# skyhehe123/SA-SSD

Hardware: AMD Instinct MI355X
Metric: KITTI-Car inference frames/sec (whole job) (higher is better)
Workload: dtype f32; 1 GPU; configs/car_cfg.py inference, fp32, synthetic lidar64 K21 frames (21500 pts -> ~16k voxels), batch=1, random-init SA-SSD weights, points resident in HBM; frames_in_flight=3, spconv_cfg=0, rulebook_pyramid=levels, launch=one hipGraph replay per frame, parallelism=frame-sharded x1, no collective

## Files before the change

### include/sassd.h

```cpp
#ifndef SASSD_H
#define SASSD_H

#include <stddef.h>
#include <stdint.h>

#ifdef __cplusplus
extern "C" {
#endif

#define SASSD_OK       0
#define SASSD_EINVAL  -1
#define SASSD_ENOSPC  -2
#define SASSD_EHIP    -3

#define SASSD_ST_VOXEL_OVERFLOW   1
#define SASSD_ST_HASH_FULL        2
#define SASSD_ST_BOX_OVERFLOW     4
#define SASSD_ST_GRID_SYNC        8
#define SASSD_ST_POINT_OVERFLOW  16

#define SASSD_MAX_POINTS_PER_VOXEL 64

const char *sassd_version(void);
int sassd_last_hip_error(void);
const char *sassd_last_hip_error_string(void);


int sassd_graph_begin(void *stream);
int sassd_graph_end(void *stream, void **graph_exec);
int sassd_graph_launch(void *graph_exec, void *stream);
int sassd_graph_destroy(void *graph_exec);

size_t sassd_voxelize_workspace_bytes(int n_points, int max_points);
int sassd_voxelize(const float *points, int n_points, int ndim, const float *voxel_size,
                   const float *coors_range, int max_points, int max_voxels, int batch_idx,
                   float *voxels, int32_t *coors, int coors_cols, int32_t *num_points, float *mean,
                   int nfeat, int32_t *row_offset, int32_t *voxel_num, int cap, int32_t *status,
                   void *workspace, size_t workspace_bytes, void *stream);

int sassd_voxelize_dev(const float *points, int points_cap, const int32_t *n_points_dev, int ndim,
                       const float *voxel_size, const float *coors_range, int max_points, int max_voxels,
                       int batch_idx, float *voxels, int32_t *coors, int coors_cols, int32_t *num_points,
                       float *mean, int nfeat, int32_t *row_offset, int32_t *voxel_num, int cap, int32_t *status,
                       void *workspace, size_t workspace_bytes, void *stream);

int sassd_voxel_mean(const float *voxels, const int32_t *num_points, int m, int max_points, int ndim,
                     int nfeat, float *mean, void *stream);

size_t sassd_crop_polytope_workspace_bytes(int cap_in);
int sassd_crop_polytope_dev(const float *points, int cap_in, const int32_t *n_in_dev, int ndim,
                            const double *planes, int f32_math, float *out, int cap_out, int32_t *n_out_dev,
                            int32_t *status, void *workspace, size_t workspace_bytes, void *stream);

size_t sassd_hash_bytes(int cap_rows);
int sassd_hash_build(const int32_t *indices, const int32_t *n_ptr, int cap, int D, int H, int W,
                     int batch_size, void *table, size_t table_bytes, int32_t *status, void *stream);
int sassd_rulebook_subm(const int32_t *indices, const int32_t *n_ptr, int cap, int D, int H, int W,
                        int batch_size, const void *table, size_t table_bytes, int32_t *nbr,
                        void *stream);
size_t sassd_rulebook_conv_workspace_bytes(int D, int H, int W, int batch_size);
int sassd_rulebook_conv(const int32_t *in_indices, const int32_t *n_in_ptr, int cap_in, int D, int H,
                        int W, int batch_size, const void *in_table, size_t in_table_bytes,
                        int32_t *out_indices, int32_t *n_out_ptr, int cap_out, int32_t *nbr,
                        int32_t *status, void *workspace, size_t workspace_bytes, void *stream);
int sassd_rulebook_pairs(const int32_t *nbr, const int32_t *n_out_ptr, int cap_out, int K,
                         int32_t *pairs , int32_t *pair_num , void *stream);

#define SASSD_PYRAMID_PERSISTENT 1
size_t sassd_rulebook_pyramid_workspace_bytes(int levels, const int *caps, int D, int H, int W, int batch_size);
int sassd_rulebook_pyramid(int levels, int32_t *const *indices, int32_t *const *n_ptrs, const int *caps,
                           int D, int H, int W, int batch_size, int32_t *const *nbr_subm,
                           int32_t *const *nbr_down, int level_begin, int level_end, int flags, int32_t *status,
                           void *workspace, size_t workspace_bytes, void *stream);

size_t sassd_spconv_packed_floats(int K, int Cin, int Cout);
int sassd_spconv_pack_weight(const float *w, int K, int Cin, int Cout, float *packed, void *stream);
int sassd_spconv_fwd(const float *x, const int32_t *nbr, const int32_t *n_out_ptr, int cap_out,
                     const float *w_packed, int K, int Cin, int Cout, const float *scale,
                     const float *shift, int relu, float *y, int cfg, void *stream);

int sassd_rulebook_transpose(const int32_t *nbr, const int32_t *n_out_ptr, int cap_out, int32_t *nbrT,
                             int cap_in, void *stream);
int sassd_spconv_pack_weight_t(const float *w, int K, int Cin, int Cout, float *packed, void *stream);
int sassd_spconv_bwd_data(const float *dy, const int32_t *nbrT, const int32_t *n_in_ptr, int cap_in,
                          const float *wT_packed, int K, int Cin, int Cout, float *dx, int cfg, void *stream);
size_t sassd_spconv_bwd_weight_workspace_bytes(int cap_out, int K, int Cin, int Cout);
int sassd_spconv_bwd_weight(const float *x, const float *dy, const int32_t *nbr, const int32_t *n_out_ptr,
                            int cap_out, int K, int Cin, int Cout, float *dw, int accumulate, int cfg,
                            void *workspace, size_t workspace_bytes, void *stream);

int sassd_densify(const float *feats, const int32_t *indices, const int32_t *n_ptr, int cap, int C,
                  int D, int H, int W, int batch_size, int channel_order, float *out, void *stream);
int sassd_densify_bf16_supported(int C, int D, int H, int W);
int sassd_densify_bf16(const float *feats, const int32_t *indices, const int32_t *n_ptr, int cap, int C, int D, int H, int W,
                       int batch_size, int channel_order, void *out, void *stream);

int sassd_spconv_bf16_supported(int K, int Cin, int Cout, int cap);
size_t sassd_spconv_bf16_packed_bytes(int K, int Cin, int Cout);
int sassd_spconv_bf16_pack_weight(const float *w, int K, int Cin, int Cout, void *packed, void *stream);
int sassd_spconv_fwd_bf16(const void *x, int x_is_f32, const int32_t *nbr, const int32_t *n_out_ptr, int cap_out,
                          const void *w_packed, int K, int Cin, int Cout, const float *scale, const float *shift, int relu,
                          void *y_bf16, int cfg, void *stream);
int sassd_densify_from_bf16(const void *feats, const int32_t *indices, const int32_t *n_ptr, int cap, int C, int D, int H, int W,
                            int batch_size, int channel_order, void *out, int out_is_bf16, void *stream);

int sassd_spconv_train_bf16_supported(int K, int Cin, int Cout, int cap);
size_t sassd_spconv_train_bf16_packed_bytes(int K, int Cin, int Cout);
int sassd_spconv_train_bf16_pack_weight(const float *w, int K, int Cin, int Cout, void *packed, void *stream);
int sassd_spconv_fwd_bf16_raw(const void *x_bf16, const int32_t *nbr, const int32_t *n_out_ptr, int cap_out, const void *w_packed,
                              int K, int Cin, int Cout, float *y, int cfg, void *stream);
size_t sassd_spconv_bwd_weight_bf16_workspace_bytes(int cap_out, int K, int Cin, int Cout);
int sassd_spconv_bwd_weight_bf16(const void *x_bf16, const void *dy_bf16, const int32_t *nbr, const int32_t *n_out_ptr, int cap_out,
                                 int K, int Cin, int Cout, float *dw, int accumulate, int cfg, void *workspace,
                                 size_t workspace_bytes, void *stream);
int sassd_bn_relu_fwd_bf16out(const float *x, int n, int C, const float *gamma, const float *beta, float *running_mean,
                              float *running_var, float momentum, float eps, void *y_bf16, float *save_mean, float *save_invstd,
                              void *workspace, size_t workspace_bytes, void *stream);
int sassd_bn_relu_bwd_bf16out(const float *x, const float *dy, int n, int C, const float *gamma, const float *beta,
                              const float *save_mean, const float *save_invstd, void *dx_bf16, float *dgamma, float *dbeta,
                              void *workspace, size_t workspace_bytes, void *stream);

size_t sassd_conv2d_packed_floats(int Cin, int Cout, int ksize);
int sassd_conv2d_pack_weight(const float *w, int Cout, int Cin, int ksize, float *packed, void *stream);
int sassd_conv2d_fwd(const float *x, const float *w_packed, const float *scale, const float *shift,
                     int relu, float *y, int batch, int Cin, int Cout, int H, int W, int ksize,
                     void *stream);
int sassd_conv2d_fwd_cfg(const float *x, const float *w_packed, const float *scale, const float *shift, int relu, float *y,
                         int batch, int Cin, int Cout, int H, int W, int ksize, int cfg, void *stream);

int sassd_conv1x1_narrow_supported(int Cin, int Cout);
int sassd_conv1x1_narrow_pad(int Cout);
int sassd_conv1x1_narrow_fwd(const float *x, const float *wT, const float *scale, const float *shift, int relu,
                             float *y, int batch, int Cin, int Cout, int H, int W, void *stream);

int sassd_conv2d_wino_supported(int Cin, int Cout, int H, int W);
size_t sassd_conv2d_wino_packed_floats(int Cin, int Cout);
int sassd_conv2d_wino_pack_weight(const float *w, int Cout, int Cin, float *packed, void *stream);
int sassd_conv2d_wino_fwd(const float *x, const float *w_packed, const float *scale, const float *shift, int relu,
                          float *y, int batch, int Cin, int Cout, int H, int W, void *stream);

int sassd_conv2d_wino4_supported(int Cin, int Cout, int H, int W);
size_t sassd_conv2d_wino4_packed_floats(int Cin, int Cout);
int sassd_conv2d_wino4_pack_weight(const float *w , int Cout, int Cin, float *packed, void *stream);
size_t sassd_conv2d_wino4_workspace_bytes(int batch, int Cin, int Cout, int H, int W);
int sassd_conv2d_wino4_fwd(const float *x, const float *w_packed, const float *scale, const float *shift, int relu,
                           float *y, int batch, int Cin, int Cout, int H, int W, int cfg, void *workspace,
                           size_t workspace_bytes, void *stream);

int sassd_conv2d_wino4_chain_supported(int Cin, int Cout, int H, int W);
size_t sassd_conv2d_wino4_chain_workspace_bytes(int batch, int cmax, int H, int W);
int sassd_conv2d_wino4_chain(const float *x, int src_products, const float *prev_scale, const float *prev_shift,
                             int prev_relu, const float *w_packed, const float *scale, const float *shift, int relu,
                             float *y, int batch, int Cin, int Cout, int cmax, int H, int W, const int32_t *tile_map,
                             const int32_t *prev_tile_map, int cfg, void *workspace, size_t workspace_bytes,
                             void *stream);
size_t sassd_conv2d_wino4_narrow_packed_floats(int Cin);
int sassd_conv2d_wino4_pack_weight_narrow(const float *w , int Cout, int Cin, float *packed, void *stream);
int sassd_conv2d_wino4_chain_tail(const float *prev_scale, const float *prev_shift, int prev_relu, float *y_prev,
                                  const float *w_packed64, const float *scale, const float *shift, int relu, float *y,
                                  int batch, int Cin, int Cout, int cmax, int H, int W, const int32_t *prev_tile_map, int cfg,
                                  void *workspace, size_t workspace_bytes, void *stream);

size_t sassd_wino4_tile_map_ints(int batch, int H, int W);
int sassd_wino4_tile_map(const int32_t *indices, const int32_t *n_ptr, int cap, int batch, int H, int W,
                         int32_t *tile_map, void *stream);

size_t sassd_wino4_sparse_grid_ints(int batch, int D, int H, int W);
int sassd_wino4_sparse_prepare(const int32_t *indices, const int32_t *n_ptr, int cap, int batch, int D, int H, int W,
                               int32_t *grid, int32_t *tile_map, void *stream);
int sassd_conv2d_wino4_chain_sparse(const float *feats, int C, int D, const int32_t *grid, const float *w_packed,
                                    const float *scale, const float *shift, int relu, float *y, int batch, int Cin, int Cout,
                                    int cmax, int H, int W, const int32_t *tile_map, int cfg, void *workspace,
                                    size_t workspace_bytes, void *stream);

int sassd_conv1x1_gemm_supported(int Cin, int Cout, int H, int W);
int sassd_conv1x1_gemm_pack_weight(const float *w , int Cout, int Cin, float *packed, void *stream);
int sassd_conv1x1_gemm_fwd(const float *x, const float *w_packed, const float *scale, const float *shift, int relu,
                           float *y, int batch, int Cin, int Cout, int H, int W, int cfg, void *stream);

int sassd_conv2d_bf16_supported(int Cin, int Cout, int H, int W);
size_t sassd_conv2d_bf16_packed_elems(int Cin, int Cout);
int sassd_conv2d_bf16_pack_weight(const float *w, int Cout, int Cin, void *packed, void *stream);
int sassd_conv2d_bf16_fwd(const float *x, const void *w_packed, const float *shift, float *y, int batch, int Cin,
                          int Cout, int H, int W, void *stream);
int sassd_conv2d_bf16_fwd_cfg(const float *x, const void *w_packed, const float *shift, float *y, int batch, int Cin,
                              int Cout, int H, int W, int cfg, void *stream);
int sassd_conv2d_bf16_bnrelu_fwd(const float *x, const float *in_affine, const void *w_packed, const float *shift, float *y,
                                 int batch, int Cin, int Cout, int H, int W, void *stream);

int sassd_conv1x1_bf16_supported(int Cin, int Cout, int HW);
size_t sassd_conv1x1_bf16_packed_elems(int Cin, int Cout);
int sassd_conv1x1_bf16_pack_weight(const float *w, int Cout, int Cin, int transposed, void *packed, void *stream);
int sassd_conv1x1_bf16_fwd(const float *x, const void *w_packed, const float *shift, float *y, int batch, int Cin, int Cout,
                           int HW, void *stream);

int sassd_conv2d_bf16_infer_supported(int Cin, int Cout, int H, int W);
size_t sassd_conv2d_bf16_infer_packed_elems(int Cin, int Cout);
int sassd_conv2d_bf16_infer_pack_weight(const float *w, int Cout, int Cin, void *packed, void *stream);
int sassd_conv2d_bf16_infer_fwd(const void *x, const void *w_packed, const float *scale, const float *shift, int relu, void *y,
                                int y_bf16, int batch, int Cin, int Cout, int H, int W, void *stream);
int sassd_conv1x1_bf16_infer_supported(int Cin, int Cout, int HW);
int sassd_conv1x1_bf16_infer_fwd(const void *x, const void *w_packed, const float *scale, const float *shift, int relu, void *y,
                                 int y_bf16, int batch, int Cin, int Cout, int HW, void *stream);

size_t sassd_conv2d_wgrad_workspace_bytes(int batch, int Cin, int Cout, int H, int W, int ksize);
int sassd_conv2d_bwd_weight(const float *x, const float *dy, float *dw, int batch, int Cin, int Cout, int H, int W,
                            int ksize, int accumulate, void *workspace, size_t workspace_bytes, void *stream);
int sassd_conv2d_bwd_weight_bf16(const float *x, const float *dy, float *dw, int batch, int Cin, int Cout, int H, int W,
                                 int ksize, int accumulate, void *workspace, size_t workspace_bytes, void *stream);
int sassd_conv2d_bwd_weight_bf16_bnrelu(const float *x, const float *x_affine, const float *dy, float *dw, int batch, int Cin,
                                        int Cout, int H, int W, int ksize, int accumulate, void *workspace,
                                        size_t workspace_bytes, void *stream);

size_t sassd_assign_targets_workspace_bytes(int batch, int n_anchors, int total_gt);
int sassd_assign_targets(const float *anchors, int anchors_per_sample, const uint8_t *anchor_mask, int n_anchors,
                         int batch, const float *gt_boxes, const int64_t *gt_classes, const uint8_t *gt_ok,
                         const int32_t *gt_offsets, int total_gt, const float *overlaps, const int64_t *overlap_offsets,
                         float matched_threshold, float unmatched_threshold, int64_t *labels, float *targets,
                         float *best_overlap, size_t out_sample_stride, int32_t *num_pos, int zero_num_pos,
                         void *workspace, size_t workspace_bytes, void *stream);
size_t sassd_guided_select_workspace_bytes(int batch, int n_anchors);
int sassd_guided_select(const float *cls_preds, const uint8_t *anchor_mask, int n_anchors, int batch, int num_class,
                        float score_thr, int cap, int64_t *sel, int32_t *counts, int32_t *overflow, void *workspace,
                        size_t workspace_bytes, void *stream);
size_t sassd_rpn_loss_workspace_bytes(int batch, int n_anchors);
int sassd_rpn_loss(const float *box_preds, const float *cls_preds, const float *dir_preds, int num_class,
                   const int64_t *labels, const float *targets, const float *anchors, int anchors_per_sample,
                   const int32_t *num_pos, int n_anchors, int batch, float *grad_box, float *grad_cls, float *grad_dir,
                   float *loss_sums, void *workspace, size_t workspace_bytes, void *stream);

size_t sassd_anchor_mask_workspace_bytes(int H0, int W0);
int sassd_anchor_mask(const int32_t *coors, const int32_t *row_begin_ptr, const int32_t *row_end_ptr,
                      int H0, int W0, const float *anchors_bv, int n_anchors, const float *voxel_size,
                      const float *coors_range, float area_threshold, uint8_t *mask, void *workspace,
                      size_t workspace_bytes, void *stream);
int sassd_anchor_mask_batch(const int32_t *coors, const int32_t *row_offsets, int batch, int H0, int W0,
                            const float *anchors_bv, int n_anchors, const float *voxel_size,
                            const float *coors_range, float area_threshold, uint8_t *mask, void *workspace,
                            size_t workspace_bytes, void *stream);

size_t sassd_decode_filter_workspace_bytes(int batch, int n_anchors_total);
int sassd_decode_filter(const float *box, const float *cls, const float *dir, size_t batch_stride,
                        int batch, int num_class, int anchors_per_loc, int H, int W,
                        const float *anchors, const uint8_t *mask, float thr, float *guided,
                        int32_t *labels, float *scores, int32_t *counts, int capK, int32_t *status,
                        void *workspace, size_t workspace_bytes, void *stream);

int sassd_pswarp_sample(const float *feat, int batch, int H, int W, const float *guided,
                        const int32_t *counts, int capK, float grid_off_x, float grid_off_y,
                        float spatial_scale, float *logits, void *stream);

int sassd_pswarp_sample_bwd(const float *feat, int batch, int H, int W, const float *guided,
                            const int32_t *counts, int capK, float grid_off_x, float grid_off_y,
                            float spatial_scale, const float *dlogits, float *dfeat, float *dguided,
                            void *stream);

size_t sassd_rescore_nms_workspace_bytes(int batch, int capK);
int sassd_rescore_nms(const float *guided, const float *logits, const int32_t *labels,
                      const int32_t *counts, int batch, int capK, float score_thr, float iou_thr,
                      float *out_boxes, float *out_scores, int32_t *out_labels, int32_t *out_counts,
                      int capD, int32_t *status, void *workspace, size_t workspace_bytes, void *stream);

#define SASSD_FRAME_MAGIC 0x53460001
#define SASSD_FRAME_HEADER_WORDS(B) ((5 + (B) + 3) / 4 * 4)
size_t sassd_frame_record_bytes(int batch, int capD);
int sassd_frame_seal(const float *boxes, const float *scores, const int32_t *labels, const int32_t *counts,
                     int batch, int capD, const int32_t *seq, const int32_t *status, void *record,
                     size_t record_bytes, void *stream);

#define SASSD_FRAME_MAGIC_KITTI 0x53460002
size_t sassd_frame_annos_bytes(int batch, int capD);
int sassd_frame_annos(const float *boxes, const int32_t *counts, int batch, int capD, const double *calib,
                      void *annos, size_t annos_bytes, void *stream);
size_t sassd_frame_record_kitti_bytes(int batch, int capD);
int sassd_frame_seal_kitti(const float *boxes, const float *scores, const int32_t *labels, const int32_t *counts,
                           int batch, int capD, const int32_t *seq, const int32_t *status, const double *calib,
                           void *record, size_t record_bytes, void *stream);

int sassd_boxes_overlap_bev(const float *boxes_a, int num_a, const float *boxes_b, int num_b,
                            float *ans_overlap, void *stream);
int sassd_boxes_iou_bev(const float *boxes_a, int num_a, const float *boxes_b, int num_b,
                        float *ans_iou, void *stream);
size_t sassd_nms_workspace_bytes(int n);
int sassd_nms_gpu(const float *boxes, int n, float thresh, int64_t *keep, int32_t *num_keep,
                  void *workspace, size_t workspace_bytes, void *stream);
int sassd_nms_normal_gpu(const float *boxes_sorted, int n, float thresh, int64_t *keep, int32_t *num_keep,
                         void *workspace, size_t workspace_bytes, void *stream);

int sassd_three_nn(int n, int m, const float *unknown, const float *known, float *dist2, int32_t *idx,
                   void *stream);
size_t sassd_three_nn_binned_workspace_bytes(int m, int nx, int ny, int batch_size);
int sassd_three_nn_binned(int n, int m, const float *unknown, const float *known, float x0, float y0, float cell,
                          int nx, int ny, int batch_size, float *dist2, int32_t *idx, void *workspace,
                          size_t workspace_bytes, void *stream);
int sassd_three_interpolate(int c, int m, int n, const float *points, const int32_t *idx, const float *weight,
                            float *out, void *stream);
int sassd_three_interpolate_grad(int c, int n, int m, const float *grad_out, const int32_t *idx,
                                 const float *weight, float *grad_points, void *stream);
int sassd_pts_in_boxes3d(const float *pts, int n, const float *boxes3d, int m, int32_t *pts_flag,
                         float *reg_target, void *stream);

int sassd_rotate_iou_eval(const float *boxes, int n, const float *query_boxes, int k, int criterion, float *iou,
                          void *stream);

int sassd_kitti_eval_statistics(const double *overlaps, int64_t ld, int n_img, const int64_t *gt_nums,
                                const int64_t *dt_nums, const int64_t *dc_nums, const double *gt_datas,
                                const double *dt_datas, const double *dontcares, const int64_t *ignored_gts,
                                const int64_t *ignored_dets, int metric, double min_overlap, const double *thresholds,
                                int n_thr, int compute_aos, double *pr, double *tp_scores, int64_t *n_tp_scores);


int sassd_points_in_polytopes(const float *points, int n, int stride, const double *planes, int m, int f32_math,
                              uint8_t *mask, void *stream);

int sassd_points_transform(float *points, int n, int stride, const uint8_t *mask, int m, const uint8_t *valid,
                           const float *centers, const float *rot_sin, const float *rot_cos, const double *loc,
                           void *stream);

int sassd_points_global_transform(float *points, int n, int stride, int flip, float rot_sin, float rot_cos, float scale,
                                  void *stream);

int sassd_paste_objects(const float *db_points, const int64_t *src_start, const int64_t *out_start, int n_obj,
                        int64_t n_out, const double *shift, const double *lower, float *out, void *stream);

int sassd_box_collision_test(const void *boxes, int n, const void *qboxes, int k, int is_f64, uint8_t *out);
int sassd_noise_per_box(const float *boxes, const uint8_t *valid, const double *loc_noises, const double *rot_noises,
                        int n, int num_try, int64_t *success);

size_t sassd_bn_relu_workspace_bytes(int C);
int sassd_bn_relu_fwd(const float *x, int n, int C, const float *gamma, const float *beta, float *running_mean,
                      float *running_var, float momentum, float eps, float *y, float *save_mean, float *save_invstd,
                      void *workspace, size_t workspace_bytes, void *stream);
int sassd_bn_relu_bwd(const float *x, const float *dy, int n, int C, const float *gamma, const float *beta,
                      const float *save_mean, const float *save_invstd, float *dx, float *dgamma, float *dbeta,
                      void *workspace, size_t workspace_bytes, void *stream);

size_t sassd_bn2d_relu_workspace_bytes(int C);
int sassd_bn2d_relu_fwd(const float *x, int B, int C, int HW, const float *gamma, const float *beta, float *running_mean,
                        float *running_var, float momentum, float eps, float *y, float *save_mean, float *save_invstd,
                        void *workspace, size_t workspace_bytes, void *stream);
int sassd_bn2d_stats(const float *x, int B, int C, int HW, const float *gamma, const float *beta, float *running_mean,
                     float *running_var, float momentum, float eps, float *save_mean, float *save_invstd, float *affine,
                     void *workspace, size_t workspace_bytes, void *stream);
int sassd_bn2d_relu_bwd(const float *x, const float *dy, int B, int C, int HW, const float *gamma, const float *beta,
                        const float *save_mean, const float *save_invstd, float *dx, float *dgamma, float *dbeta,
                        void *workspace, size_t workspace_bytes, void *stream);

int sassd_guided_decode_fwd(const float *box_preds, const float *dir_preds, const float *anchors, int anchors_per_sample,
                            const int64_t *sel, const int32_t *sel_count, const float *gt_boxes, const int32_t *gt_off,
                            int A, int B, int cap, int gmax, float *guided, int32_t *counts, void *stream);
int sassd_guided_decode_bwd(const float *box_preds, const float *anchors, int anchors_per_sample, const int64_t *sel,
                            const int32_t *sel_count, const int32_t *gt_off, int A, int B, int cap, int gmax,
                            const float *dguided, float *dbox, void *stream);
int sassd_boxes_iou3d_batch(const float *boxes, const int32_t *counts, int B, int rows, const float *gt_boxes,
                            const int32_t *gt_off, int gmax, const int64_t *ov_off, float *overlaps, void *stream);
size_t sassd_focal_loss_workspace_bytes(int n);
int sassd_focal_loss(const float *logits, const int64_t *labels, int n, const int32_t *num_pos, int nb, float *loss_sum,
                     float *grad, void *workspace, size_t workspace_bytes, void *stream);

size_t sassd_aux_head_workspace_bytes(int N);
int sassd_aux_prepare(const float *voxel_feats, int vstride, const int32_t *coors, int N, const int32_t *const *indices,
                      const int *M, const float *voxel_size, const float *offset, const float *gt_boxes,
                      const int32_t *gt_off, int B, float *points, float *const *known, uint8_t *label, float *target,
                      int *npos, void *stream);
int sassd_aux_head_fwd(int N, const float *const *feats, const int32_t *const *nn_idx, const float *const *nn_d2,
                       const float *w1, const float *w2, const uint8_t *label, const float *target, const int *npos,
                       float *wgt, float *h, float *out, float *gout, float *loss_sums, void *workspace,
                       size_t workspace_bytes, void *stream);
int sassd_aux_head_bwd(int N, const float *const *feats, const int *M, const int32_t *const *nn_idx, const float *w1,
                       const float *w2, const float *wgt, const float *h, const float *gout, const float *grad_sums,
                       float *const *grad_feats, float *dw1, float *dw2, void *workspace, size_t workspace_bytes,
                       void *stream);

int sassd_gather_pack(const float *src, const int32_t *map, void *dst, long n, int bf16, void *stream);
int sassd_grad_sumsq(const float *grad, long n, float *out, void *stream);
int sassd_adam_step(float *param, const float *grad, float *exp_avg, float *exp_avg_sq, long n,
                    const float *grad_sumsq, float lr, float beta1, float beta2, float eps, float weight_decay,
                    int step, float max_norm, float grad_scale, void *stream);

size_t sassd_three_interpolate_grad_det_workspace_bytes(int n, int m);
int sassd_three_interpolate_grad_det(int c, int n, int m, const float *grad_out, const int32_t *idx,
                                     const float *weight, float *grad_points, void *ws, size_t ws_bytes, void *stream);
size_t sassd_aux_head_bwd_det_workspace_bytes(int N, const int *M);
int sassd_aux_head_bwd_det(int N, const float *const *feats, const int *M, const int32_t *const *nn_idx,
                           const float *w1, const float *w2, const float *wgt, const float *h, const float *gout,
                           const float *grad_sums, float *const *grad_feats, float *dw1, float *dw2, void *workspace,
                           size_t workspace_bytes, void *stream);
size_t sassd_pswarp_sample_bwd_det_workspace_bytes(int batch, int capK);
int sassd_pswarp_sample_bwd_det(const float *feat, int batch, int H, int W, const float *guided,
                                const int32_t *counts, int capK, float grid_off_x, float grid_off_y,
                                float spatial_scale, const float *dlogits, float *dfeat, float *dguided, void *ws,
                                size_t ws_bytes, void *stream);
size_t sassd_grad_sumsq_det_workspace_bytes(long n);
int sassd_grad_sumsq_det(const float *grad, long n, float *out, void *ws, size_t ws_bytes, void *stream);

int sassd_mfma_probe(const float *a32, const float *b32, float *d32, const float *a16, const float *b16,
                     float *d16, int ksteps, void *stream);

#ifdef __cplusplus
}
#endif
#endif
```

### sa-ssd_amd/_C.py

```python
import ctypes as C
import os
import subprocess

_HERE = os.path.dirname(os.path.abspath(__file__))
LIB_PATH = os.path.join(_HERE, "lib", "libsassd.so")
_lib = None

OK, EINVAL, ENOSPC, EHIP = 0, -1, -2, -3
ST_VOXEL_OVERFLOW, ST_HASH_FULL, ST_BOX_OVERFLOW = 1, 2, 4
ST_POINT_OVERFLOW = 16


def build(force=False, verbose=False):
    cmd = ["make", "-C", os.path.join(_HERE, "csrc"), "-j8"]
    if force:
        subprocess.check_call(cmd + ["clean"], stdout=subprocess.DEVNULL)
    out = subprocess.run(cmd, stdout=subprocess.PIPE, stderr=subprocess.STDOUT, text=True)
    if verbose or out.returncode != 0:
        print(out.stdout)
    if out.returncode != 0:
        raise RuntimeError("building libsassd.so failed")
    return LIB_PATH


_SZ = C.c_size_t
_P = C.c_void_p
_I = C.c_int
_F = C.c_float

_SIGS = {
    "sassd_version": (C.c_char_p, []),
    "sassd_last_hip_error": (_I, []),
    "sassd_last_hip_error_string": (C.c_char_p, []),
    "sassd_voxelize_workspace_bytes": (_SZ, [_I, _I]),
    "sassd_voxelize": (_I, [_P, _I, _I, _P, _P, _I, _I, _I, _P, _P, _I, _P, _P, _I, _P, _P, _I, _P, _P, _SZ, _P]),
    "sassd_voxelize_dev": (_I, [_P, _I, _P, _I, _P, _P, _I, _I, _I, _P, _P, _I, _P, _P, _I, _P, _P, _I, _P, _P, _SZ, _P]),
    "sassd_voxel_mean": (_I, [_P, _P, _I, _I, _I, _I, _P, _P]),
    "sassd_crop_polytope_workspace_bytes": (_SZ, [_I]),
    "sassd_crop_polytope_dev": (_I, [_P, _I, _P, _I, _P, _I, _P, _I, _P, _P, _P, _SZ, _P]),
    "sassd_hash_bytes": (_SZ, [_I]),
    "sassd_hash_build": (_I, [_P, _P, _I, _I, _I, _I, _I, _P, _SZ, _P, _P]),
    "sassd_rulebook_subm": (_I, [_P, _P, _I, _I, _I, _I, _I, _P, _SZ, _P, _P]),
    "sassd_rulebook_conv_workspace_bytes": (_SZ, [_I, _I, _I, _I]),
    "sassd_rulebook_conv": (_I, [_P, _P, _I, _I, _I, _I, _I, _P, _SZ, _P, _P, _I, _P, _P, _P, _SZ, _P]),
    "sassd_rulebook_pairs": (_I, [_P, _P, _I, _I, _P, _P, _P]),
    "sassd_rulebook_pyramid_workspace_bytes": (_SZ, [_I, _P, _I, _I, _I, _I]),
    "sassd_rulebook_pyramid": (_I, [_I, _P, _P, _P, _I, _I, _I, _I, _P, _P, _I, _I, _I, _P, _P, _SZ, _P]),
    "sassd_graph_begin": (_I, [_P]),
    "sassd_graph_end": (_I, [_P, _P]),
    "sassd_graph_launch": (_I, [_P, _P]),
    "sassd_graph_destroy": (_I, [_P]),
    "sassd_spconv_packed_floats": (_SZ, [_I, _I, _I]),
    "sassd_spconv_pack_weight": (_I, [_P, _I, _I, _I, _P, _P]),
    "sassd_spconv_fwd": (_I, [_P, _P, _P, _I, _P, _I, _I, _I, _P, _P, _I, _P, _I, _P]),
    "sassd_rulebook_transpose": (_I, [_P, _P, _I, _P, _I, _P]),
    "sassd_spconv_pack_weight_t": (_I, [_P, _I, _I, _I, _P, _P]),
    "sassd_spconv_bwd_data": (_I, [_P, _P, _P, _I, _P, _I, _I, _I, _P, _I, _P]),
    "sassd_spconv_bwd_weight_workspace_bytes": (_SZ, [_I, _I, _I, _I]),
    "sassd_spconv_bwd_weight": (_I, [_P, _P, _P, _P, _I, _I, _I, _I, _P, _I, _I, _P, _SZ, _P]),
    "sassd_densify": (_I, [_P, _P, _P, _I, _I, _I, _I, _I, _I, _I, _P, _P]),
    "sassd_densify_bf16_supported": (_I, [_I, _I, _I, _I]),
    "sassd_densify_bf16": (_I, [_P, _P, _P, _I, _I, _I, _I, _I, _I, _I, _P, _P]),
    "sassd_spconv_bf16_supported": (_I, [_I, _I, _I, _I]),
    "sassd_spconv_bf16_packed_bytes": (_SZ, [_I, _I, _I]),
    "sassd_spconv_bf16_pack_weight": (_I, [_P, _I, _I, _I, _P, _P]),
    "sassd_spconv_fwd_bf16": (_I, [_P, _I, _P, _P, _I, _P, _I, _I, _I, _P, _P, _I, _P, _I, _P]),
    "sassd_densify_from_bf16": (_I, [_P, _P, _P, _I, _I, _I, _I, _I, _I, _I, _P, _I, _P]),
    "sassd_spconv_train_bf16_supported": (_I, [_I, _I, _I, _I]),
    "sassd_spconv_train_bf16_packed_bytes": (_SZ, [_I, _I, _I]),
    "sassd_spconv_train_bf16_pack_weight": (_I, [_P, _I, _I, _I, _P, _P]),
    "sassd_spconv_fwd_bf16_raw": (_I, [_P, _P, _P, _I, _P, _I, _I, _I, _P, _I, _P]),
    "sassd_spconv_bwd_weight_bf16_workspace_bytes": (_SZ, [_I, _I, _I, _I]),
    "sassd_spconv_bwd_weight_bf16": (_I, [_P, _P, _P, _P, _I, _I, _I, _I, _P, _I, _I, _P, _SZ, _P]),
    "sassd_bn_relu_fwd_bf16out": (_I, [_P, _I, _I, _P, _P, _P, _P, _F, _F, _P, _P, _P, _P, _SZ, _P]),
    "sassd_bn_relu_bwd_bf16out": (_I, [_P, _P, _I, _I, _P, _P, _P, _P, _P, _P, _P, _P, _SZ, _P]),
    "sassd_conv2d_packed_floats": (_SZ, [_I, _I, _I]),
    "sassd_conv2d_pack_weight": (_I, [_P, _I, _I, _I, _P, _P]),
    "sassd_conv2d_fwd": (_I, [_P, _P, _P, _P, _I, _P, _I, _I, _I, _I, _I, _I, _P]),
    "sassd_conv2d_fwd_cfg": (_I, [_P, _P, _P, _P, _I, _P, _I, _I, _I, _I, _I, _I, _I, _P]),
    "sassd_anchor_mask_workspace_bytes": (_SZ, [_I, _I]),
    "sassd_anchor_mask": (_I, [_P, _P, _P, _I, _I, _P, _I, _P, _P, _F, _P, _P, _SZ, _P]),
    "sassd_anchor_mask_batch": (_I, [_P, _P, _I, _I, _I, _P, _I, _P, _P, _F, _P, _P, _SZ, _P]),
    "sassd_decode_filter_workspace_bytes": (_SZ, [_I, _I]),
    "sassd_decode_filter": (_I, [_P, _P, _P, _SZ, _I, _I, _I, _I, _I, _P, _P, _F, _P, _P, _P, _P, _I, _P, _P, _SZ, _P]),
    "sassd_pswarp_sample": (_I, [_P, _I, _I, _I, _P, _P, _I, _F, _F, _F, _P, _P]),
    "sassd_pswarp_sample_bwd": (_I, [_P, _I, _I, _I, _P, _P, _I, _F, _F, _F, _P, _P, _P, _P]),
    "sassd_rescore_nms_workspace_bytes": (_SZ, [_I, _I]),
    "sassd_rescore_nms": (_I, [_P, _P, _P, _P, _I, _I, _F, _F, _P, _P, _P, _P, _I, _P, _P, _SZ, _P]),
    "sassd_frame_record_bytes": (_SZ, [_I, _I]),
    "sassd_frame_seal": (_I, [_P, _P, _P, _P, _I, _I, _P, _P, _P, _SZ, _P]),
    "sassd_frame_annos_bytes": (_SZ, [_I, _I]),
    "sassd_frame_annos": (_I, [_P, _P, _I, _I, _P, _P, _SZ, _P]),
    "sassd_frame_record_kitti_bytes": (_SZ, [_I, _I]),
    "sassd_frame_seal_kitti": (_I, [_P, _P, _P, _P, _I, _I, _P, _P, _P, _P, _SZ, _P]),
    "sassd_boxes_overlap_bev": (_I, [_P, _I, _P, _I, _P, _P]),
    "sassd_boxes_iou_bev": (_I, [_P, _I, _P, _I, _P, _P]),
    "sassd_nms_workspace_bytes": (_SZ, [_I]),
    "sassd_nms_gpu": (_I, [_P, _I, _F, _P, _P, _P, _SZ, _P]),
    "sassd_nms_normal_gpu": (_I, [_P, _I, _F, _P, _P, _P, _SZ, _P]),
    "sassd_three_nn": (_I, [_I, _I, _P, _P, _P, _P, _P]),
    "sassd_three_interpolate": (_I, [_I, _I, _I, _P, _P, _P, _P, _P]),
    "sassd_three_interpolate_grad": (_I, [_I, _I, _I, _P, _P, _P, _P, _P]),
    "sassd_pts_in_boxes3d": (_I, [_P, _I, _P, _I, _P, _P, _P]),
    "sassd_three_nn_binned_workspace_bytes": (_SZ, [_I, _I, _I, _I]),
    "sassd_three_nn_binned": (_I, [_I, _I, _P, _P, _F, _F, _F, _I, _I, _I, _P, _P, _P, _SZ, _P]),
    "sassd_conv2d_wino_supported": (_I, [_I, _I, _I, _I]),
    "sassd_conv2d_wino_packed_floats": (_SZ, [_I, _I]),
    "sassd_conv2d_wino_pack_weight": (_I, [_P, _I, _I, _P, _P]),
    "sassd_conv2d_wino_fwd": (_I, [_P, _P, _P, _P, _I, _P, _I, _I, _I, _I, _I, _P]),
    "sassd_conv2d_wino4_supported": (_I, [_I, _I, _I, _I]),
    "sassd_conv2d_wino4_packed_floats": (_SZ, [_I, _I]),
    "sassd_conv2d_wino4_pack_weight": (_I, [_P, _I, _I, _P, _P]),
    "sassd_conv2d_wino4_workspace_bytes": (_SZ, [_I, _I, _I, _I, _I]),
    "sassd_conv2d_wino4_fwd": (_I, [_P, _P, _P, _P, _I, _P, _I, _I, _I, _I, _I, _I, _P, _SZ, _P]),
    "sassd_conv1x1_gemm_supported": (_I, [_I, _I, _I, _I]),
    "sassd_conv1x1_gemm_pack_weight": (_I, [_P, _I, _I, _P, _P]),
    "sassd_conv1x1_narrow_supported": (_I, [_I, _I]),
    "sassd_conv1x1_narrow_pad": (_I, [_I]),
    "sassd_conv1x1_narrow_fwd": (_I, [_P, _P, _P, _P, _I, _P, _I, _I, _I, _I, _I, _P]),
    "sassd_conv1x1_gemm_fwd": (_I, [_P, _P, _P, _P, _I, _P, _I, _I, _I, _I, _I, _I, _P]),
    "sassd_conv2d_bf16_supported": (_I, [_I, _I, _I, _I]),
    "sassd_conv2d_bf16_packed_elems": (_SZ, [_I, _I]),
    "sassd_conv2d_bf16_pack_weight": (_I, [_P, _I, _I, _P, _P]),
    "sassd_conv2d_bf16_fwd": (_I, [_P, _P, _P, _P, _I, _I, _I, _I, _I, _P]),
    "sassd_conv2d_bf16_fwd_cfg": (_I, [_P, _P, _P, _P, _I, _I, _I, _I, _I, _I, _P]),
    "sassd_conv2d_bf16_bnrelu_fwd": (_I, [_P, _P, _P, _P, _P, _I, _I, _I, _I, _I, _P]),
    "sassd_conv1x1_bf16_supported": (_I, [_I, _I, _I]),
    "sassd_conv1x1_bf16_packed_elems": (_SZ, [_I, _I]),
    "sassd_conv1x1_bf16_pack_weight": (_I, [_P, _I, _I, _I, _P, _P]),
    "sassd_conv1x1_bf16_fwd": (_I, [_P, _P, _P, _P, _I, _I, _I, _I, _P]),
    "sassd_conv2d_bf16_infer_supported": (_I, [_I, _I, _I, _I]),
    "sassd_conv2d_bf16_infer_packed_elems": (_SZ, [_I, _I]),
    "sassd_conv2d_bf16_infer_pack_weight": (_I, [_P, _I, _I, _P, _P]),
    "sassd_conv2d_bf16_infer_fwd": (_I, [_P, _P, _P, _P, _I, _P, _I, _I, _I, _I, _I, _I, _P]),
    "sassd_conv1x1_bf16_infer_supported": (_I, [_I, _I, _I]),
    "sassd_conv1x1_bf16_infer_fwd": (_I, [_P, _P, _P, _P, _I, _P, _I, _I, _I, _I, _I, _P]),
    "sassd_conv2d_wgrad_workspace_bytes": (_SZ, [_I, _I, _I, _I, _I, _I]),
    "sassd_conv2d_bwd_weight": (_I, [_P, _P, _P, _I, _I, _I, _I, _I, _I, _I, _P, _SZ, _P]),
    "sassd_assign_targets_workspace_bytes": (_SZ, [_I, _I, _I]),
    "sassd_assign_targets": (_I, [_P, _I, _P, _I, _I, _P, _P, _P, _P, _I, _P, _P, _F, _F, _P, _P, _P, _SZ, _P, _I, _P,
                                  _SZ, _P]),
    "sassd_guided_select_workspace_bytes": (_SZ, [_I, _I]),
    "sassd_guided_select": (_I, [_P, _P, _I, _I, _I, _F, _I, _P, _P, _P, _P, _SZ, _P]),
    "sassd_rpn_loss_workspace_bytes": (_SZ, [_I, _I]),
    "sassd_rpn_loss": (_I, [_P, _P, _P, _I, _P, _P, _P, _I, _P, _I, _I, _P, _P, _P, _P, _P, _SZ, _P]),
    "sassd_conv2d_bwd_weight_bf16": (_I, [_P, _P, _P, _I, _I, _I, _I, _I, _I, _I, _P, _SZ, _P]),
    "sassd_conv2d_bwd_weight_bf16_bnrelu": (_I, [_P, _P, _P, _P, _I, _I, _I, _I, _I, _I, _I, _P, _SZ, _P]),
    "sassd_rotate_iou_eval": (_I, [_P, _I, _P, _I, _I, _P, _P]),
    "sassd_kitti_eval_statistics": (_I, [_P, C.c_int64, _I, _P, _P, _P, _P, _P, _P, _P, _P, _I, C.c_double, _P, _I, _I, _P,
                                         _P, _P]),
    "sassd_points_in_polytopes": (_I, [_P, _I, _I, _P, _I, _I, _P, _P]),
    "sassd_points_transform": (_I, [_P, _I, _I, _P, _I, _P, _P, _P, _P, _P, _P]),
    "sassd_points_global_transform": (_I, [_P, _I, _I, _I, _F, _F, _F, _P]),
    "sassd_paste_objects": (_I, [_P, _P, _P, _I, C.c_int64, _P, _P, _P, _P]),
    "sassd_box_collision_test": (_I, [_P, _I, _P, _I, _I, _P]),
    "sassd_noise_per_box": (_I, [_P, _P, _P, _P, _I, _I, _P]),
    "sassd_bn_relu_workspace_bytes": (_SZ, [_I]),
    "sassd_bn_relu_fwd": (_I, [_P, _I, _I, _P, _P, _P, _P, _F, _F, _P, _P, _P, _P, _SZ, _P]),
    "sassd_bn_relu_bwd": (_I, [_P, _P, _I, _I, _P, _P, _P, _P, _P, _P, _P, _P, _SZ, _P]),
    "sassd_bn2d_relu_workspace_bytes": (_SZ, [_I]),
    "sassd_bn2d_relu_fwd": (_I, [_P, _I, _I, _I, _P, _P, _P, _P, _F, _F, _P, _P, _P, _P, _SZ, _P]),
    "sassd_bn2d_stats": (_I, [_P, _I, _I, _I, _P, _P, _P, _P, _F, _F, _P, _P, _P, _P, _SZ, _P]),
    "sassd_bn2d_relu_bwd": (_I, [_P, _P, _I, _I, _I, _P, _P, _P, _P, _P, _P, _P, _P, _SZ, _P]),
    "sassd_aux_head_workspace_bytes": (_SZ, [_I]),
    "sassd_aux_prepare": (_I, [_P, _I, _P, _I, _P, _P, _P, _P, _P, _P, _I, _P, _P, _P, _P, _P, _P]),
    "sassd_aux_head_fwd": (_I, [_I, _P, _P, _P, _P, _P, _P, _P, _P, _P, _P, _P, _P, _P, _P, _SZ, _P]),
    "sassd_aux_head_bwd": (_I, [_I, _P, _P, _P, _P, _P, _P, _P, _P, _P, _P, _P, _P, _P, _SZ, _P]),
    "sassd_guided_decode_fwd": (_I, [_P, _P, _P, _I, _P, _P, _P, _P, _I, _I, _I, _I, _P, _P, _P]),
    "sassd_guided_decode_bwd": (_I, [_P, _P, _I, _P, _P, _P, _I, _I, _I, _I, _P, _P, _P]),
    "sassd_boxes_iou3d_batch": (_I, [_P, _P, _I, _I, _P, _P, _I, _P, _P, _P]),
    "sassd_focal_loss_workspace_bytes": (_SZ, [_I]),
    "sassd_focal_loss": (_I, [_P, _P, _I, _P, _I, _P, _P, _P, _SZ, _P]),
    "sassd_conv2d_wino4_chain_supported": (_I, [_I, _I, _I, _I]),
    "sassd_conv2d_wino4_chain_workspace_bytes": (_SZ, [_I, _I, _I, _I]),
    "sassd_conv2d_wino4_chain": (_I, [_P, _I, _P, _P, _I, _P, _P, _P, _I, _P, _I, _I, _I, _I, _I, _I, _P, _P, _I, _P, _SZ, _P]),
    "sassd_conv2d_wino4_narrow_packed_floats": (_SZ, [_I]),
    "sassd_conv2d_wino4_pack_weight_narrow": (_I, [_P, _I, _I, _P, _P]),
    "sassd_conv2d_wino4_chain_tail": (_I, [_P, _P, _I, _P, _P, _P, _P, _I, _P, _I, _I, _I, _I, _I, _I, _P, _I, _P, _SZ, _P]),
    "sassd_wino4_tile_map_ints": (_SZ, [_I, _I, _I]),
    "sassd_wino4_tile_map": (_I, [_P, _P, _I, _I, _I, _I, _P, _P]),
    "sassd_wino4_sparse_grid_ints": (_SZ, [_I, _I, _I, _I]),
    "sassd_wino4_sparse_prepare": (_I, [_P, _P, _I, _I, _I, _I, _I, _P, _P, _P]),
    "sassd_conv2d_wino4_chain_sparse": (_I, [_P, _I, _I, _P, _P, _P, _P, _I, _P, _I, _I, _I, _I, _I, _I, _P, _I, _P, _SZ, _P]),
    "sassd_gather_pack": (_I, [_P, _P, _P, C.c_long, _I, _P]),
    "sassd_grad_sumsq": (_I, [_P, C.c_long, _P, _P]),
    "sassd_adam_step": (_I, [_P, _P, _P, _P, C.c_long, _P, _F, _F, _F, _F, _F, _I, _F, _F, _P]),
    "sassd_mfma_probe": (_I, [_P, _P, _P, _P, _P, _P, _I, _P]),
    "sassd_three_interpolate_grad_det_workspace_bytes": (_SZ, [_I, _I]),
    "sassd_three_interpolate_grad_det": (_I, [_I, _I, _I, _P, _P, _P, _P, _P, _SZ, _P]),
    "sassd_aux_head_bwd_det_workspace_bytes": (_SZ, [_I, _P]),
    "sassd_aux_head_bwd_det": (_I, [_I, _P, _P, _P, _P, _P, _P, _P, _P, _P, _P, _P, _P, _P, _SZ, _P]),
    "sassd_pswarp_sample_bwd_det_workspace_bytes": (_SZ, [_I, _I]),
    "sassd_pswarp_sample_bwd_det": (_I, [_P, _I, _I, _I, _P, _P, _I, _F, _F, _F, _P, _P, _P, _P, _SZ, _P]),
    "sassd_grad_sumsq_det_workspace_bytes": (_SZ, [C.c_long]),
    "sassd_grad_sumsq_det": (_I, [_P, C.c_long, _P, _P, _SZ, _P]),
}

EXPORTS = tuple(_SIGS.keys())


def lib():
    global _lib
    if _lib is None:
        if not os.path.exists(LIB_PATH):
            raise RuntimeError("libsassd.so not found at %s -- run `python -c 'import __graft_entry__ as g; "
                               "g.build()'` (there is no CPU fallback)" % LIB_PATH)
        l = C.CDLL(LIB_PATH)
        for name, (res, args) in _SIGS.items():
            fn = getattr(l, name)
            fn.restype = res
            fn.argtypes = args
        _lib = l
    return _lib


def check(rc, what):
    if rc != OK:
        l = lib()
        extra = ""
        if rc == EHIP:
            extra = ": " + l.sassd_last_hip_error_string().decode()
        raise RuntimeError("%s failed with code %d%s" % (what, rc, extra))


def ptr(t):
    return None if t is None else t.data_ptr()


def stream():
    import torch
    return torch._C._cuda_getCurrentRawStream(torch.cuda.current_device())


def csrc_hash():
    import glob
    import hashlib
    h = hashlib.sha1()
    for f in sorted(glob.glob(os.path.join(os.path.dirname(os.path.abspath(__file__)), "csrc", "*"))):
        if os.path.isfile(f):
            h.update(os.path.basename(f).encode())
            h.update(open(f, "rb").read())
    return h.hexdigest()[:12]
```

### sa-ssd_amd/csrc/conv2d.hip

```cpp
#include <type_traits>

#include "common.h"

namespace {

typedef float f32x16 __attribute__((ext_vector_type(16)));
typedef __attribute__((address_space(3))) void *lds_ptr_t;
typedef const __attribute__((address_space(1))) void *glb_ptr_t;

__device__ __attribute__((aligned(16))) float g_zero_page[4] = {0.f, 0.f, 0.f, 0.f};

template <int CT, int TAPS, int VEC>
struct ConvCfg {
    static constexpr bool KSPLIT = (CT == 1);
    static constexpr int NSEG = (CT == 4) ? 9 : 5;
    static constexpr int KC = (TAPS == 9) ? 8 : 16;
    static constexpr int HALO = (TAPS == 9) ? 1 : 0;
    static constexpr int BMC = CT * 32;
    static constexpr int PIX = NSEG * 32;
    static constexpr int WV4 = TAPS * KC * BMC / 4;
    static constexpr int NLW = (WV4 + 255) / 256;
    static constexpr int MAXLP = (VEC == 4) ? 1 : 40;
    static constexpr int WS = TAPS * KC * BMC;
    static constexpr int NWJ = (WS / 256 + 3) / 4;
// ... 174 lines not shown
                    src -= (size_t)over * P.HW;
                }
            }
            __builtin_amdgcn_global_load_lds((glb_ptr_t)src, (lds_ptr_t)(pdst[part] >= 0 ? buf + pdst[part] : smem + dummy),
                                             16, 0, 0);
            pptr[part] += ((pdata >> part) & 1u) ? pinc : 0;
        }
    };
    auto dma = [&](int ch, float *buf) {
#pragma unroll
        for (int part = 0; part < NPARTS; ++part) dma_part(ch, buf, part);
    };
    auto issue = [&](int ch) {
        const float *wsrc_base = P.wp + (size_t)ch * TAPS * KC * P.CoutPad;
#pragma unroll
        for (int i = 0; i < NLW; ++i)
            if (woff_g[i] >= 0) wreg[i] = *(const float4 *)(wsrc_base + woff_g[i]);
#pragma unroll
        for (int i = 0; i < MAXLP; ++i)
            if (goff[i] >= 0) preg[i] = xb[clamp_off(ch, goff[i])];
    };
    auto commit = [&](float *buf) {
#pragma unroll
        for (int i = 0; i < NLW; ++i)
            if (woff_g[i] >= 0) *(float4 *)(buf + woff_l[i]) = wreg[i];
        float *pbuf = buf + WS;
#pragma unroll
        for (int i = 0; i < MAXLP; ++i)
            if (goff[i] >= 0) pbuf[loff[i]] = preg[i];
    };

    if constexpr (DMA) {
        dma(0, smem);
    } else {
        issue(0);
        commit(smem);
    }
    __syncthreads();

    for (int ch = 0; ch < nchunk; ++ch) {
        const float *W_s = smem + (ch & 1) * bufs;
        const float *P_s = W_s + WS;
        const bool more = ch + 1 < nchunk;
        float *nbuf = smem + ((ch + 1) & 1) * bufs;
        if (more) {
            if constexpr (!DMA) issue(ch + 1);
            else if constexpr (TAPS == 1) dma(ch + 1, nbuf);
        }
        constexpr int NSTEP = KSPLIT ? KC / 8 : KC / 2;
        float a_cur[NSTEP], a_nxt[NSTEP], b_cur[NSTEP][NSEG], b_nxt[NSTEP][NSEG];
        auto read_ops = [&](int tap, float (&av)[NSTEP], float (&bv)[NSTEP][NSEG]) {
            const int toff = (TAPS == 9) ? ((tap / 3 - 1) * PW + (tap % 3 - 1)) : 0;
#pragma unroll
            for (int t = 0; t < NSTEP; ++t) {
                const int s = KSPLIT ? wave + 4 * t : t;
                av[t] = W_s[(tap * KC + 2 * s) * BMC + aoff];
                const float *pb = P_s + 2 * s * chs + toff;
#pragma unroll
                for (int j = 0; j < NSEG; ++j) bv[t][j] = pb[laddr[j]];
            }
        };
        read_ops(0, a_cur, b_cur);
#pragma unroll
        for (int tap = 0; tap < TAPS; ++tap) {
            if constexpr (DMA && TAPS == 9) {
                if (more && tap < kDmaTaps && !(P.dbg & 1)) {
#pragma unroll
                    for (int part = tap; part < NPARTS; part += kDmaTaps) dma_part(ch + 1, nbuf, part);
                }
            }
            __builtin_amdgcn_sched_barrier(0);
            if (tap + 1 < TAPS) read_ops(tap + 1, a_nxt, b_nxt);
#pragma unroll
            for (int t = 0; t < NSTEP; ++t)
#pragma unroll
                for (int j = 0; j < NSEG; ++j)
                    acc[j] = __builtin_amdgcn_mfma_f32_32x32x2f32(a_cur[t], b_cur[t][j], acc[j], 0, 0, 0);
#pragma unroll
            for (int i = 0; i < NSTEP * NSEG; ++i) {
                __builtin_amdgcn_sched_group_barrier(0x008, 1, 0);
                __builtin_amdgcn_sched_group_barrier(0x100, 2, 0);
            }
            __builtin_amdgcn_sched_barrier(0);
            if (tap + 1 < TAPS) {
#pragma unroll
                for (int t = 0; t < NSTEP; ++t) {
                    a_cur[t] = a_nxt[t];
#pragma unroll
                    for (int j = 0; j < NSEG; ++j) b_cur[t][j] = b_nxt[t][j];
                }
            }
        }
        if constexpr (!DMA) {
            if (more) commit(smem + ((ch + 1) & 1) * bufs);
        }
        if (!(P.dbg & 2)) __syncthreads();
    }

    float *yb = P.y + (size_t)b * P.Cout * P.HW;
    if constexpr (!KSPLIT) {
        float sc[16], sh[16];
        int co[16];
#pragma unroll
        for (int r = 0; r < 16; ++r) {
            co[r] = cg * BMC + ct * 32 + (r & 3) + 8 * (r >> 2) + 4 * (lane >> 5);
            const bool ok = co[r] < P.Cout;
            sc[r] = (ok && P.scale) ? P.scale[co[r]] : 1.f;
            sh[r] = (ok && P.shift) ? P.shift[co[r]] : 0.f;
        }
#pragma unroll
        for (int j = 0; j < NSEG; ++j) {
            const int p = p0 + j * 32 + (lane & 31);
            if (p < P.HW) {
#pragma unroll
                for (int r = 0; r < 16; ++r) {
                    if (co[r] < P.Cout) {
                        float v = acc[j][r] * sc[r] + sh[r];
                        if (P.relu) v = fmaxf(v, 0.f);
                        yb[(size_t)co[r] * P.HW + p] = v;
                    }
                }
            }
        }
    } else {
        float *red = smem;
#pragma unroll
        for (int j = 0; j < NSEG; ++j)
#pragma unroll
            for (int r = 0; r < 16; ++r) red[((wave * NSEG + j) * 16 + r) * 64 + lane] = acc[j][r];
        __syncthreads();
        for (int j = wave; j < NSEG; j += 4) {
            const int p = p0 + j * 32 + (lane & 31);
#pragma unroll
            for (int r = 0; r < 16; ++r) {
                const int co = cg * BMC + (r & 3) + 8 * (r >> 2) + 4 * (lane >> 5);
                float v = red[((0 * NSEG + j) * 16 + r) * 64 + lane] + red[((1 * NSEG + j) * 16 + r) * 64 + lane] +
                          red[((2 * NSEG + j) * 16 + r) * 64 + lane] + red[((3 * NSEG + j) * 16 + r) * 64 + lane];
                if (p < P.HW && co < P.Cout) {
                    v = v * (P.scale ? P.scale[co] : 1.f) + (P.shift ? P.shift[co] : 0.f);
                    if (P.relu) v = fmaxf(v, 0.f);
                    yb[(size_t)co * P.HW + p] = v;
                }
            }
        }
    }
}

template <int CT, int TAPS, int VEC>
int launch_conv(ConvParams P, hipStream_t stream)
{
    using C = ConvCfg<CT, TAPS, VEC>;
    P.ntp = cdiv(P.HW, C::PIX);
    P.ncg = P.CoutPad / C::BMC;
    P.PW = (P.W + 8 + 3) / 4 * 4;
    P.NPR = (C::PIX - 1 + P.W - 1) / P.W + 1 + 2 * C::HALO;
    const size_t ps = ((size_t)C::KC * P.NPR * P.PW + 255) / 256 * 256;
    const size_t stage = 2 * ((size_t)C::WS + ps) * sizeof(float);
    const size_t red = C::KSPLIT ? (size_t)4 * C::NSEG * 16 * 64 * sizeof(float) : 0;
    const size_t lds = (stage > red ? stage : red) + 1024;
    if (lds > 160 * 1024) return SASSD_EINVAL;
    if (VEC == 4 ? (ps > (size_t)C::MAXPJ * 4 * 256) : ((size_t)C::KC * P.NPR * P.W > (size_t)256 * C::MAXLP))
        return SASSD_EINVAL;
    static bool attr_set = false;
    if (!attr_set) {
        (void)hipFuncSetAttribute((const void *)conv2d_kernel<CT, TAPS, VEC>,
                                  hipFuncAttributeMaxDynamicSharedMemorySize, 160 * 1024);
        attr_set = true;
    }
    const int grid = P.B * P.ntp * P.ncg;
    hipLaunchKernelGGL((conv2d_kernel<CT, TAPS, VEC>), dim3(grid), dim3(256), lds, stream, P);
    return sassd_launch_status();
}

inline int cout_pad(int Cout) { return (Cout > 64) ? cdiv(Cout, 128) * 128 : cdiv(Cout, 32) * 32; }
inline int kc_of(int ksize) { return ksize == 3 ? 8 : 16; }

}

extern "C" size_t sassd_conv2d_packed_floats(int Cin, int Cout, int ksize)
{
    const int KC = kc_of(ksize);
    return (size_t)cdiv(Cin, KC) * KC * ksize * ksize * cout_pad(Cout);
}

extern "C" int sassd_conv2d_pack_weight(const float *w, int Cout, int Cin, int ksize, float *packed, void *stream_)
{
    if (!w || !packed || (ksize != 1 && ksize != 3) || Cin < 1) return SASSD_EINVAL;
    const int cp = cout_pad(Cout);
    const size_t total = sassd_conv2d_packed_floats(Cin, Cout, ksize);
    hipLaunchKernelGGL(conv_pack_kernel, dim3((unsigned)((total + 255) / 256)), dim3(256), 0, (hipStream_t)stream_, w,
                       Cout, Cin, ksize, cp, kc_of(ksize), packed);
    return sassd_launch_status();
}

extern "C" int sassd_conv2d_fwd_cfg(const float *x, const float *w_packed, const float *scale, const float *shift,
                                    int relu, float *y, int batch, int Cin, int Cout, int H, int W, int ksize, int cfg,
                                    void *stream_)
{
    if (!x || !w_packed || !y || batch < 1 || Cin < 1 || (ksize != 1 && ksize != 3)) return SASSD_EINVAL;
    if (H < 1 || W < 2) return SASSD_EINVAL;
    ConvParams P;
    P.x = x; P.wp = w_packed; P.scale = scale; P.shift = shift; P.y = y;
    P.B = batch; P.Cin = Cin; P.Cout = Cout; P.CoutPad = cout_pad(Cout); P.H = H; P.W = W; P.HW = H * W;
    P.relu = relu;
    P.dbg = cfg;
    hipStream_t stream = (hipStream_t)stream_;
    const bool wide = P.CoutPad % 128 == 0;
    const bool vec = (W % 4 == 0) && (((uintptr_t)x & 15) == 0);
#define SASSD_CONV_GO(CT, TAPS) \
    return vec ? launch_conv<CT, TAPS, 4>(P, stream) : launch_conv<CT, TAPS, 1>(P, stream)
    if (wide) {
        if (ksize == 3) { SASSD_CONV_GO(4, 9); } else { SASSD_CONV_GO(4, 1); }
    } else {
        if (ksize == 3) { SASSD_CONV_GO(1, 9); } else { SASSD_CONV_GO(1, 1); }
    }
#undef SASSD_CONV_GO
}

extern "C" int sassd_conv2d_fwd(const float *x, const float *w_packed, const float *scale, const float *shift,
                                int relu, float *y, int batch, int Cin, int Cout, int H, int W, int ksize,
                                void *stream_)
{
    return sassd_conv2d_fwd_cfg(x, w_packed, scale, shift, relu, y, batch, Cin, Cout, H, W, ksize, 0, stream_);
}

namespace {
template <int CO>
__global__ void __launch_bounds__(256) conv1x1_narrow_kernel(const float *__restrict__ x, const float *__restrict__ wT,
                                                             const float *__restrict__ scale, const float *__restrict__ shift,
                                                             int relu, float *__restrict__ y, int Cin, int Cout, int HW)
{
    __shared__ float part[4][CO][64];
    const int lane = threadIdx.x & 63;
    const int wave = __builtin_amdgcn_readfirstlane(threadIdx.x >> 6);
    const int b = blockIdx.y;
    const int p = blockIdx.x * 64 + lane;
    const bool ok = p < HW;
    const int pc = ok ? p : HW - 1;
    const int cq = (Cin + 3) / 4;
    const int c0 = wave * cq, c1 = min(c0 + cq, Cin);
    const float *xp = x + ((size_t)b * Cin + c0) * HW + pc;
    float acc[CO];
#pragma unroll
    for (int j = 0; j < CO; ++j) acc[j] = 0.f;
    int c = c0;
    for (; c + 8 <= c1; c += 8) {
        float v[8];
#pragma unroll
        for (int u = 0; u < 8; ++u) v[u] = xp[(size_t)u * HW];
        xp += (size_t)8 * HW;
#pragma unroll
        for (int u = 0; u < 8; ++u) {
            const float *wr = wT + (size_t)(c + u) * CO;
#pragma unroll
            for (int j = 0; j < CO; ++j) acc[j] = fmaf(v[u], wr[j], acc[j]);
        }
    }
    for (; c < c1; ++c) {
        const float v = *xp;
        xp += HW;
        const float *wr = wT + (size_t)c * CO;
#pragma unroll
        for (int j = 0; j < CO; ++j) acc[j] = fmaf(v, wr[j], acc[j]);
    }
#pragma unroll
    for (int j = 0; j < CO; ++j) part[wave][j][lane] = acc[j];
    __syncthreads();
    for (int j = wave; j < Cout; j += 4) {
        float s = (part[0][j][lane] + part[1][j][lane]) + (part[2][j][lane] + part[3][j][lane]);
        s = s * (scale ? scale[j] : 1.f) + (shift ? shift[j] : 0.f);
        if (relu) s = fmaxf(s, 0.f);
        if (ok) y[((size_t)b * Cout + j) * HW + p] = s;
    }
}
}

extern "C" int sassd_conv1x1_narrow_supported(int Cin, int Cout) { return Cin >= 1 && Cout >= 1 && Cout <= 32 ? 1 : 0; }

extern "C" int sassd_conv1x1_narrow_pad(int Cout)
{
    return Cout <= 8 ? 8 : Cout <= 16 ? 16 : Cout <= 20 ? 20 : Cout <= 24 ? 24 : Cout <= 28 ? 28 : 32;
}

extern "C" int sassd_conv1x1_narrow_fwd(const float *x, const float *wT, const float *scale, const float *shift, int relu,
                                        float *y, int batch, int Cin, int Cout, int H, int W, void *stream_)
{
    if (!x || !wT || !y || batch < 1 || H < 1 || W < 1 || !sassd_conv1x1_narrow_supported(Cin, Cout)) return SASSD_EINVAL;
    const int HW = H * W;
    const dim3 grid((unsigned)cdiv(HW, 64), (unsigned)batch);
    hipStream_t s = (hipStream_t)stream_;
#define SASSD_NARROW(CO) hipLaunchKernelGGL((conv1x1_narrow_kernel<CO>), grid, dim3(256), 0, s, x, wT, scale, shift, relu, y, Cin, Cout, HW)
    if (((uintptr_t)wT) & 15) return SASSD_EINVAL;
    switch (sassd_conv1x1_narrow_pad(Cout)) {
    case 8: SASSD_NARROW(8); break;
    case 16: SASSD_NARROW(16); break;
    case 20: SASSD_NARROW(20); break;
    case 24: SASSD_NARROW(24); break;
    case 28: SASSD_NARROW(28); break;
    default: SASSD_NARROW(32); break;
    }
#undef SASSD_NARROW
    return sassd_launch_status();
}
```

### sa-ssd_amd/csrc/heads.hip

```cpp
#include "common.h"
#include "iou3d_device.h"

namespace {

constexpr float kPi = 3.14159265358979323846f;

__device__ __forceinline__ float sigmoidf(float x) { return 1.0f / (1.0f + expf(-x)); }

struct DfParams {
    const float *box, *cls, *dir, *anchors;
    const uint8_t *mask;
    size_t bs;
    int B, ncls, A, HW, Atot, capK;
    float thr;
};

constexpr int kDfPerThread = 4;
constexpr int kDfPerBlock = 256 * kDfPerThread;

__device__ __forceinline__ bool df_select(const DfParams &P, int b, int r, float *score, int *label)
{
    if (r >= P.Atot) return false;
    if (!P.mask[(size_t)b * P.Atot + r]) return false;
    const int per_cls = P.HW * P.A;
    const int ci = r / per_cls, rem = r - ci * per_cls;
    const int pix = rem / P.A, a = rem - pix * P.A;
    const float *c = P.cls + (size_t)b * P.bs + (size_t)(ci * P.A * P.ncls + a * P.ncls) * P.HW + pix;
    float best = sigmoidf(c[0]);
    int bl = 0;
    for (int j = 1; j < P.ncls; ++j) {
        const float s = sigmoidf(c[(size_t)j * P.HW]);
        if (s > best) { best = s; bl = j; }
    }
    *score = best;
    *label = bl;
    return best > P.thr;
}

__global__ void __launch_bounds__(256) df_count_kernel(DfParams P, int nblk, int *__restrict__ bsum)
{
    __shared__ int wsum[17];
    const int b = blockIdx.y;
    const int base = blockIdx.x * kDfPerBlock + threadIdx.x * kDfPerThread;
    int s = 0;
    float sc; int lb;
#pragma unroll
    for (int k = 0; k < kDfPerThread; ++k) s += df_select(P, b, base + k, &sc, &lb) ? 1 : 0;
    int tot;
    block_exclusive_scan(s, wsum, &tot);
    if (threadIdx.x == 0) bsum[b * nblk + blockIdx.x] = tot;
}

__global__ void __launch_bounds__(256) df_emit_kernel(DfParams P, int nblk, const int *__restrict__ bsum,
                                                      float *__restrict__ guided, int32_t *__restrict__ labels,
                                                      float *__restrict__ scores, int32_t *__restrict__ counts,
                                                      int32_t *status)
{
    __shared__ int wsum[17];
    const int b = blockIdx.y;
    int part = 0;
    for (int j = threadIdx.x; j < (int)blockIdx.x; j += 256) part += bsum[b * nblk + j];
    int before;
    block_exclusive_scan(part, wsum, &before);
    const int base = blockIdx.x * kDfPerBlock + threadIdx.x * kDfPerThread;
    bool sel[kDfPerThread];
    float sc[kDfPerThread];
    int lb[kDfPerThread];
    int s = 0;
#pragma unroll
    for (int k = 0; k < kDfPerThread; ++k) { sel[k] = df_select(P, b, base + k, &sc[k], &lb[k]); s += sel[k] ? 1 : 0; }
    int tot;
    int o = before + block_exclusive_scan(s, wsum, &tot);
    if ((int)blockIdx.x == nblk - 1 && threadIdx.x == 0) {
        int total = before + tot;
        if (total > P.capK) { if (status) atomicOr(status, SASSD_ST_BOX_OVERFLOW); total = P.capK; }
        counts[b] = total;
    }
#pragma unroll
    for (int k = 0; k < kDfPerThread; ++k) {
        if (!sel[k]) continue;
        const int slot = o++;
        if (slot >= P.capK) continue;
        const int r = base + k;
        const int per_cls = P.HW * P.A;
        const int ci = r / per_cls, rem = r - ci * per_cls;
        const int pix = rem / P.A, a = rem - pix * P.A;
        const float *bx = P.box + (size_t)b * P.bs + (size_t)(ci * P.A * 7 + a * 7) * P.HW + pix;
        const float *dr = P.dir + (size_t)b * P.bs + (size_t)(ci * P.A * 2 + a * 2) * P.HW + pix;
        const float *an = P.anchors + (size_t)r * 7;
        const float xt = bx[0], yt = bx[(size_t)P.HW], zt = bx[(size_t)2 * P.HW], wt = bx[(size_t)3 * P.HW],
                    lt = bx[(size_t)4 * P.HW], ht = bx[(size_t)5 * P.HW], rt = bx[(size_t)6 * P.HW];
        const float xa = an[0], ya = an[1], wa = an[3], la = an[4], ha = an[5], ra = an[6];
        const float za = an[2] + ha / 2;
        const float diag = sqrtf(la * la + wa * wa);
        const float xg = xt * diag + xa;
        const float yg = yt * diag + ya;
        float zg = zt * ha + za;
        const float lg = expf(lt) * la;
        const float wg = expf(wt) * wa;
        const float hg = expf(ht) * ha;
        float rg = rt + ra;
        zg = zg - hg / 2;
        const int dl = dr[(size_t)P.HW] > dr[0] ? 1 : 0;
        if ((rg > 0.f) != (dl != 0)) rg += kPi;
        float *g = guided + ((size_t)b * P.capK + slot) * 7;
        g[0] = xg; g[1] = yg; g[2] = zg; g[3] = wg; g[4] = lg; g[5] = hg; g[6] = rg;
        labels[(size_t)b * P.capK + slot] = lb[k];
        if (scores) scores[(size_t)b * P.capK + slot] = sc[k];
    }
}

struct WarpParams {
    const float *feat, *guided;
    const int32_t *counts;
    float *logits;
    int B, H, W, capK;
    float offx, offy, scale;
    float lin4[4], lin7[7];
};

__global__ void __launch_bounds__(256) pswarp_kernel(WarpParams P)
{
    const int b = blockIdx.y;
    const int K = min(P.counts[b], P.capK);
    const int box = blockIdx.x * 8 + (threadIdx.x >> 5);
    const int k = threadIdx.x & 31;
    float val = 0.f;
    if (box < K && k < 28) {
        const float *g = P.guided + ((size_t)b * P.capK + box) * 7;
        const float xg = g[0], yg = g[1], wg = g[3], lg = g[4], rg = g[6];
        const float ct = cosf(rg), st = sinf(rg);
        const int ix = k / 7, iy = k - ix * 7;
        const float xx = P.lin4[ix] * wg, yy = P.lin7[iy] * lg;
        const float x = xx * ct + yy * st + xg;
        const float y = yy * ct - xx * st + yg;
        const float u = (x + P.offx) * P.scale, v = (y + P.offy) * P.scale;
        const float gx = u / (float)(P.W - 1) * 2.f - 1.f, gy = v / (float)(P.H - 1) * 2.f - 1.f;
        float fx = (gx + 1.f) / 2.f * (float)(P.W - 1), fy = (gy + 1.f) / 2.f * (float)(P.H - 1);
        fx = fminf(fmaxf(fx, -2.f), (float)P.W + 1.f);
        fy = fminf(fmaxf(fy, -2.f), (float)P.H + 1.f);
        const float x0f = floorf(fx), y0f = floorf(fy);
        const int x0 = (int)x0f, y0 = (int)y0f, x1 = x0 + 1, y1 = y0 + 1;
        const float wx1 = fx - x0f, wx0 = (x0f + 1.f) - fx, wy1 = fy - y0f, wy0 = (y0f + 1.f) - fy;
        const float *im = P.feat + ((size_t)b * 28 + k) * P.H * P.W;
        const bool xin0 = x0 >= 0 && x0 < P.W, xin1 = x1 >= 0 && x1 < P.W;
        const bool yin0 = y0 >= 0 && y0 < P.H, yin1 = y1 >= 0 && y1 < P.H;
        if (yin0 && xin0) val += im[(size_t)y0 * P.W + x0] * (wx0 * wy0);
        if (yin0 && xin1) val += im[(size_t)y0 * P.W + x1] * (wx1 * wy0);
        if (yin1 && xin0) val += im[(size_t)y1 * P.W + x0] * (wx0 * wy1);
        if (yin1 && xin1) val += im[(size_t)y1 * P.W + x1] * (wx1 * wy1);
    }
#pragma unroll
    for (int o = 16; o >= 1; o >>= 1) val += __shfl_xor(val, o, 32);
    if (box < K && k == 0) P.logits[(size_t)b * P.capK + box] = val / 28.f;
}

template <bool kDfeat>
__global__ void __launch_bounds__(256) pswarp_bwd_kernel(WarpParams P, const float *__restrict__ dlogits,
                                                         float *__restrict__ dfeat, float *__restrict__ dguided)
{
    const int b = blockIdx.y;
    const int K = min(P.counts[b], P.capK);
    const int box = blockIdx.x * 8 + (threadIdx.x >> 5);
    const int k = threadIdx.x & 31;
    float gxg = 0.f, gyg = 0.f, gw = 0.f, gl = 0.f, gr = 0.f;
    if (box < K && k < 28) {
        const float *g = P.guided + ((size_t)b * P.capK + box) * 7;
        const float xg = g[0], yg = g[1], wg = g[3], lg = g[4], rg = g[6];
        const float ct = cosf(rg), st = sinf(rg);
        const int ix = k / 7, iy = k - ix * 7;
        const float xx = P.lin4[ix] * wg, yy = P.lin7[iy] * lg;
        const float x = xx * ct + yy * st + xg;
        const float y = yy * ct - xx * st + yg;
        const float u = (x + P.offx) * P.scale, v = (y + P.offy) * P.scale;
        const float gx = u / (float)(P.W - 1) * 2.f - 1.f, gy = v / (float)(P.H - 1) * 2.f - 1.f;
        float fx = (gx + 1.f) / 2.f * (float)(P.W - 1), fy = (gy + 1.f) / 2.f * (float)(P.H - 1);
        const bool inr = fx > -1.f && fx < (float)P.W && fy > -1.f && fy < (float)P.H;
        fx = fminf(fmaxf(fx, -2.f), (float)P.W + 1.f);
        fy = fminf(fmaxf(fy, -2.f), (float)P.H + 1.f);
        const float x0f = floorf(fx), y0f = floorf(fy);
        const int x0 = (int)x0f, y0 = (int)y0f, x1 = x0 + 1, y1 = y0 + 1;
        const float wx1 = fx - x0f, wx0 = (x0f + 1.f) - fx, wy1 = fy - y0f, wy0 = (y0f + 1.f) - fy;
        const float go = dlogits[(size_t)b * P.capK + box] / 28.f;
        const size_t plane = ((size_t)b * 28 + k) * P.H * P.W;
        const float *im = P.feat + plane;
        float *di = dfeat + plane;
        const bool xin0 = x0 >= 0 && x0 < P.W, xin1 = x1 >= 0 && x1 < P.W;
        const bool yin0 = y0 >= 0 && y0 < P.H, yin1 = y1 >= 0 && y1 < P.H;
        float v00 = 0.f, v01 = 0.f, v10 = 0.f, v11 = 0.f;
        if (inr) {
            if (yin0 && xin0) { v00 = im[(size_t)y0 * P.W + x0]; if (kDfeat) atomicAdd(&di[(size_t)y0 * P.W + x0], go * wx0 * wy0); }
            if (yin0 && xin1) { v01 = im[(size_t)y0 * P.W + x1]; if (kDfeat) atomicAdd(&di[(size_t)y0 * P.W + x1], go * wx1 * wy0); }
            if (yin1 && xin0) { v10 = im[(size_t)y1 * P.W + x0]; if (kDfeat) atomicAdd(&di[(size_t)y1 * P.W + x0], go * wx0 * wy1); }
            if (yin1 && xin1) { v11 = im[(size_t)y1 * P.W + x1]; if (kDfeat) atomicAdd(&di[(size_t)y1 * P.W + x1], go * wx1 * wy1); }
        }
        const float dfx = ((v01 - v00) * wy0 + (v11 - v10) * wy1) * go;
        const float dfy = ((v10 - v00) * wx0 + (v11 - v01) * wx1) * go;
        const float dx = dfx * P.scale, dy = dfy * P.scale;
        gxg = dx; gyg = dy;
        gw = (dx * ct - dy * st) * P.lin4[ix];
        gl = (dx * st + dy * ct) * P.lin7[iy];
        gr = dx * (-xx * st + yy * ct) + dy * (-yy * st - xx * ct);
    }
#pragma unroll
    for (int o = 16; o >= 1; o >>= 1) {
        gxg += __shfl_xor(gxg, o, 32); gyg += __shfl_xor(gyg, o, 32); gw += __shfl_xor(gw, o, 32);
        gl += __shfl_xor(gl, o, 32); gr += __shfl_xor(gr, o, 32);
    }
    if (box < K && k == 0 && dguided) {
        float *d = dguided + ((size_t)b * P.capK + box) * 7;
        d[0] = gxg; d[1] = gyg; d[2] = 0.f; d[3] = gw; d[4] = gl; d[5] = 0.f; d[6] = gr;
    }
}

constexpr int kPwChunk = 512;

__global__ void __launch_bounds__(256) pswarp_dfeat_det_kernel(WarpParams P, const float *__restrict__ dlogits,
                                                               float *__restrict__ dfeat)
{
    __shared__ unsigned long long key[4 * kPwChunk];
    __shared__ float val[4 * kPwChunk];
    const int plane = blockIdx.x;
    const int b = plane / 28, k = plane - b * 28;
    const int K = min(P.counts[b], P.capK);
    const int ix = k / 7, iy = k - ix * 7;
    const size_t HW = (size_t)P.H * P.W;
    float *di = dfeat + (size_t)plane * HW;
    for (int c0 = 0; c0 < K; c0 += kPwChunk) {
        const int nb = min(kPwChunk, K - c0), ne = 4 * nb;
        const int P2 = 1 << (32 - __clz(ne - 1));
        for (int i = threadIdx.x; i < nb; i += 256) {
            const int box = c0 + i;
            unsigned long long kk[4] = {~0ull, ~0ull, ~0ull, ~0ull};
            float vv[4] = {0.f, 0.f, 0.f, 0.f};
            const float *g = P.guided + ((size_t)b * P.capK + box) * 7;
            const float xg = g[0], yg = g[1], wg = g[3], lg = g[4], rg = g[6];
            const float ct = cosf(rg), st = sinf(rg);
            const float xx = P.lin4[ix] * wg, yy = P.lin7[iy] * lg;
            const float x = xx * ct + yy * st + xg;
            const float y = yy * ct - xx * st + yg;
            const float u = (x + P.offx) * P.scale, v = (y + P.offy) * P.scale;
            const float gx = u / (float)(P.W - 1) * 2.f - 1.f, gy = v / (float)(P.H - 1) * 2.f - 1.f;
            float fx = (gx + 1.f) / 2.f * (float)(P.W - 1), fy = (gy + 1.f) / 2.f * (float)(P.H - 1);
            const bool inr = fx > -1.f && fx < (float)P.W && fy > -1.f && fy < (float)P.H;
            fx = fminf(fmaxf(fx, -2.f), (float)P.W + 1.f);
            fy = fminf(fmaxf(fy, -2.f), (float)P.H + 1.f);
            const float x0f = floorf(fx), y0f = floorf(fy);
            const int x0 = (int)x0f, y0 = (int)y0f, x1 = x0 + 1, y1 = y0 + 1;
            const float wx1 = fx - x0f, wx0 = (x0f + 1.f) - fx, wy1 = fy - y0f, wy0 = (y0f + 1.f) - fy;
            const float go = dlogits[(size_t)b * P.capK + box] / 28.f;
            const bool xin0 = x0 >= 0 && x0 < P.W, xin1 = x1 >= 0 && x1 < P.W;
            const bool yin0 = y0 >= 0 && y0 < P.H, yin1 = y1 >= 0 && y1 < P.H;
            const unsigned long long id = (unsigned long long)(i * 4);
            if (inr) {
                if (yin0 && xin0) { kk[0] = ((unsigned long long)((size_t)y0 * P.W + x0) << 32) | id; vv[0] = go * wx0 * wy0; }
                if (yin0 && xin1) { kk[1] = ((unsigned long long)((size_t)y0 * P.W + x1) << 32) | (id + 1); vv[1] = go * wx1 * wy0; }
                if (yin1 && xin0) { kk[2] = ((unsigned long long)((size_t)y1 * P.W + x0) << 32) | (id + 2); vv[2] = go * wx0 * wy1; }
                if (yin1 && xin1) { kk[3] = ((unsigned long long)((size_t)y1 * P.W + x1) << 32) | (id + 3); vv[3] = go * wx1 * wy1; }
            }
#pragma unroll
            for (int q = 0; q < 4; ++q) { key[i * 4 + q] = kk[q]; val[i * 4 + q] = vv[q]; }
        }
        for (int i = ne + threadIdx.x; i < P2; i += 256) key[i] = ~0ull;
        __syncthreads();
        for (int size = 2; size <= P2; size <<= 1) {
            for (int stride = size >> 1; stride > 0; stride >>= 1) {
                for (int i = threadIdx.x; i < P2 / 2; i += 256) {
                    const int lo = 2 * i - (i & (stride - 1)), hi = lo + stride;
                    const bool asc = (lo & size) == 0;
                    const unsigned long long a = key[lo], c = key[hi];
                    if ((a > c) == asc) { key[lo] = c; key[hi] = a; }
                }
                __syncthreads();
            }
        }
        {
#pragma clang fp contract(off)
            for (int i = threadIdx.x; i < P2; i += 256) {
                const unsigned long long kk = key[i];
                if (kk == ~0ull) continue;
                const unsigned pix = (unsigned)(kk >> 32);
                if (i > 0 && (unsigned)(key[i - 1] >> 32) == pix) continue;
                float acc = di[pix];
                for (int j = i; j < P2 && (unsigned)(key[j] >> 32) == pix; ++j) acc = acc + val[(unsigned)key[j]];
                di[pix] = acc;
            }
        }
        __threadfence();
        __syncthreads();
    }
}

__device__ __forceinline__ unsigned long long nms_word(const float *__restrict__ boxes, int n, int row, int cb,
                                                       float thr, int lane)
{
    const int col = cb * 64 + lane;
    bool hit = false;
    if (col < n && col > row) {
        const iou3d::Box a = iou3d::load_box(boxes + (size_t)row * 5);
        const iou3d::Box b = iou3d::load_box(boxes + (size_t)col * 5);
        const float dx = (a.x1 + a.x2) * 0.5f - (b.x1 + b.x2) * 0.5f, dy = (a.y1 + a.y2) * 0.5f - (b.y1 + b.y2) * 0.5f;
        const float wa = a.x2 - a.x1, la = a.y2 - a.y1, wb = b.x2 - b.x1, lb = b.y2 - b.y1;
        const float rr = 0.5f * (sqrtf(wa * wa + la * la) + sqrtf(wb * wb + lb * lb)) + 1e-3f;
        if (thr < 0.f || dx * dx + dy * dy <= rr * rr) hit = iou3d::iou_bev(a, b) > thr;
    }
    return __ballot(hit);
}

template <int WPL>
__device__ __forceinline__ int nms_greedy(const unsigned long long *mask, int n, int ncb, int lane, int64_t *keep64,
                                          int32_t *keep32, int cap_keep)
{
    unsigned long long remv[WPL];
#pragma unroll
    for (int w = 0; w < WPL; ++w) remv[w] = 0ull;
    int nk = 0;
    for (int i = 0; i < n; ++i) {
        const int nb = i >> 6;
        unsigned long long word = 0ull;
#pragma unroll
        for (int w = 0; w < WPL; ++w)
            if ((nb >> 6) == w) word = __shfl(remv[w], nb & 63, 64);
        if (!((word >> (i & 63)) & 1ull)) {
            if (nk < cap_keep && lane == 0) { if (keep64) keep64[nk] = i; if (keep32) keep32[nk] = i; }
            ++nk;
#pragma unroll
            for (int w = 0; w < WPL; ++w) {
                const int cb = w * 64 + lane;
                if (cb >= nb && cb < ncb) remv[w] |= mask[(size_t)i * ncb + cb];
            }
        }
    }
    return nk;
}

__device__ __forceinline__ int nms_greedy_chunked(const unsigned long long *__restrict__ mask, int n, int ncb, int lane,
                                                  int *__restrict__ keep, int cap_keep)
{
    unsigned long long remv = 0ull;
    int nk = 0;
    for (int cb0 = 0; cb0 < ncb; ++cb0) {
        const int r = cb0 * 64 + lane;
        const unsigned long long dw = (r < n) ? mask[(size_t)r * ncb + cb0] : 0ull;
        const unsigned dlo = (unsigned)dw, dhi = (unsigned)(dw >> 32);
        unsigned long long rem = __shfl(remv, cb0, 64);
        rem = ((unsigned long long)(unsigned)__builtin_amdgcn_readfirstlane((int)(rem >> 32)) << 32) |
              (unsigned long long)(unsigned)__builtin_amdgcn_readfirstlane((int)(unsigned)rem);
        const int rows = min(64, n - cb0 * 64);
        unsigned long long kept = 0ull;
        for (int i = 0; i < rows; ++i) {
            if (!((rem >> i) & 1ull)) {
                kept |= 1ull << i;
                rem |= ((unsigned long long)(unsigned)__builtin_amdgcn_readlane((int)dhi, i) << 32) |
                       (unsigned long long)(unsigned)__builtin_amdgcn_readlane((int)dlo, i);
            }
        }
        if ((kept >> lane) & 1ull) {
            const int pos = nk + __popcll(kept & ((1ull << lane) - 1ull));
            if (pos < cap_keep) keep[pos] = r;
        }
        nk += __popcll(kept);
        unsigned long long acc = 0ull;
        unsigned long long km = kept;
        while (km) {
            const int i = __ffsll((long long)km) - 1;
            km &= km - 1ull;
            if (lane > cb0 && lane < ncb) acc |= mask[(size_t)(cb0 * 64 + i) * ncb + lane];
        }
        remv |= acc;
    }
    return nk;
}

__device__ __forceinline__ unsigned long long nms_word_normal(const float *__restrict__ boxes, int n, int row, int cb,
                                                              float thr, int lane)
{
    const int col = cb * 64 + lane;
    bool hit = false;
    if (col < n && col > row) {
        const float *a = boxes + (size_t)row * 5, *b = boxes + (size_t)col * 5;
        const float left = fmaxf(a[0], b[0]), right = fminf(a[2], b[2]);
        const float top = fmaxf(a[1], b[1]), bottom = fminf(a[3], b[3]);
        const float width = fmaxf(right - left, 0.f), height = fmaxf(bottom - top, 0.f);
        const float inter = width * height;
        const float sa = (a[2] - a[0]) * (a[3] - a[1]), sb = (b[2] - b[0]) * (b[3] - b[1]);
        hit = inter / fmaxf(sa + sb - inter, iou3d::kEps) > thr;
    }
    return __ballot(hit);
}

__global__ void __launch_bounds__(256) nms_mask_kernel(const float *__restrict__ boxes, int n, int ncb, float thr,
                                                       unsigned long long *__restrict__ mask, int normal)
{
    const int lane = threadIdx.x & 63;
    const int item = blockIdx.x * 4 + (threadIdx.x >> 6);
    if (item >= n * ncb) return;
    const int row = item / ncb, cb = item - row * ncb;
    unsigned long long w = 0ull;
    if (cb >= (row >> 6)) w = normal ? nms_word_normal(boxes, n, row, cb, thr, lane) : nms_word(boxes, n, row, cb, thr, lane);
    if (lane == 0) mask[item] = w;
}

__global__ void __launch_bounds__(64) nms_greedy_kernel(const unsigned long long *__restrict__ mask, int n, int ncb,
                                                        int64_t *__restrict__ keep, int32_t *__restrict__ num_keep)
{
    const int lane = threadIdx.x;
    int nk;
    if (ncb <= 64) nk = nms_greedy<1>(mask, n, ncb, lane, keep, nullptr, n);
    else nk = nms_greedy<4>(mask, n, ncb, lane, keep, nullptr, n);
    if (lane == 0) *num_keep = nk;
}

struct RnParams {
    const float *guided, *logits;
    const int32_t *labels, *counts;
    float *out_boxes, *out_scores;
    int32_t *out_labels, *out_counts, *status;
    int capK, capD;
    float score_thr, iou_thr;
    int *cand;
    float *cscore;
    int *order;
    float *sboxes;
    unsigned long long *mask;
    int *keep;
    int ncb_cap;
};

constexpr int kRnLdsScores = 4096;

__global__ void __launch_bounds__(1024) rescore_prep_kernel(RnParams P, int *__restrict__ mcount)
{
    __shared__ int wsum[17];
    __shared__ float s_score[kRnLdsScores];
    const int b = blockIdx.x, tid = threadIdx.x;
    const int K = min(P.counts[b], P.capK);
    int *cand = P.cand + (size_t)b * P.capK;
    float *cscore = P.cscore + (size_t)b * P.capK;
    int *order = P.order + (size_t)b * P.capK;
    float *sb = P.sboxes + (size_t)b * P.capK * 5;
    const float *guided = P.guided + (size_t)b * P.capK * 7;
    int running = 0;
    for (int i0 = 0; i0 < K; i0 += 1024) {
        const int i = i0 + tid;
        float s = 0.f;
        bool sel = false;
        if (i < K) { s = sigmoidf(P.logits[(size_t)b * P.capK + i]); sel = s > P.score_thr; }
        int tot;
        const int ex = block_exclusive_scan(sel ? 1 : 0, wsum, &tot);
        if (sel) { cand[running + ex] = i; cscore[running + ex] = s; if (running + ex < kRnLdsScores) s_score[running + ex] = s; }
        running += tot;
    }
    const int M = running;
    if (tid == 0) mcount[b] = M;
    __syncthreads();
    if (M == 0) return;
    for (int i = tid; i < M; i += 1024) {
        const float si = cscore[i];
        int rank = 0;
        if (M <= kRnLdsScores) {
#pragma unroll 8
            for (int j = 0; j < M; ++j) {
                const float sj = s_score[j];
                rank += (sj > si || (sj == si && j < i)) ? 1 : 0;
            }
        } else {
            for (int j = 0; j < M; ++j) {
                const float sj = cscore[j];
                rank += (sj > si || (sj == si && j < i)) ? 1 : 0;
            }
        }
        order[rank] = i;
    }
    __syncthreads();
    for (int r = tid; r < M; r += 1024) {
        const float *g = guided + (size_t)cand[order[r]] * 7;
        const float hx = g[3] / 2, hy = g[4] / 2;
        sb[r * 5 + 0] = g[0] - hx; sb[r * 5 + 1] = g[1] - hy;
        sb[r * 5 + 2] = g[0] + hx; sb[r * 5 + 3] = g[1] + hy;
        sb[r * 5 + 4] = g[6];
    }
}

__global__ void __launch_bounds__(256) rescore_mask_kernel(RnParams P, const int *__restrict__ mcount)
{
    const int b = blockIdx.y, lane = threadIdx.x & 63;
    const int M = mcount[b];
    const int ncb = (M + 63) >> 6;
    const float *sb = P.sboxes + (size_t)b * P.capK * 5;
    unsigned long long *mask = P.mask + (size_t)b * P.capK * P.ncb_cap;
    const int nwaves = gridDim.x * 4;
    for (int item = blockIdx.x * 4 + (threadIdx.x >> 6); item < M * ncb; item += nwaves) {
        const int row = item / ncb, cb = item - row * ncb;
        if (cb < (row >> 6)) continue;
        const unsigned long long w = nms_word(sb, M, row, cb, P.iou_thr, lane);
        if (lane == 0) mask[(size_t)row * ncb + cb] = w;
    }
}

__global__ void __launch_bounds__(256) rescore_final_kernel(RnParams P, const int *__restrict__ mcount)
{
    __shared__ int s_nk;
    const int b = blockIdx.x, tid = threadIdx.x, lane = tid & 63, wave = tid >> 6;
    const int M = mcount[b];
    if (M == 0) { if (tid == 0) P.out_counts[b] = 0; return; }
    const int ncb = (M + 63) >> 6;
    const int *cand = P.cand + (size_t)b * P.capK;
    const float *cscore = P.cscore + (size_t)b * P.capK;
    const int *order = P.order + (size_t)b * P.capK;
    const unsigned long long *mask = P.mask + (size_t)b * P.capK * P.ncb_cap;
    int *keep = P.keep + (size_t)b * P.capK;
    const float *guided = P.guided + (size_t)b * P.capK * 7;
    if (wave == 0) {
        const int nk = nms_greedy_chunked(mask, M, ncb, lane, keep, P.capK);
        if (lane == 0) s_nk = nk;
    }
    __syncthreads();
    int nk = s_nk;
    if (nk > P.capD) { if (tid == 0 && P.status) atomicOr(P.status, SASSD_ST_BOX_OVERFLOW); nk = P.capD; }
    for (int t = tid; t < nk; t += 256) {
        const int c = order[keep[t]];
        const int src = cand[c];
        float *ob = P.out_boxes + ((size_t)b * P.capD + t) * 7;
#pragma unroll
        for (int q = 0; q < 7; ++q) ob[q] = guided[(size_t)src * 7 + q];
        P.out_scores[(size_t)b * P.capD + t] = cscore[c];
        P.out_labels[(size_t)b * P.capD + t] = P.labels[(size_t)b * P.capK + src];
    }
    if (tid == 0) P.out_counts[b] = nk;
}

template <bool IOU>
__global__ void __launch_bounds__(256) pair_kernel(const float *__restrict__ a, int na, const float *__restrict__ b,
                                                   int nb, float *__restrict__ out)
{
    const size_t t = (size_t)blockIdx.x * blockDim.x + threadIdx.x;
    if (t >= (size_t)na * nb) return;
    const int i = t / nb, j = t - (size_t)i * nb;
    const iou3d::Box A = iou3d::load_box(a + (size_t)i * 5), Bx = iou3d::load_box(b + (size_t)j * 5);
    out[t] = IOU ? iou3d::iou_bev(A, Bx) : iou3d::box_overlap(A, Bx);
}

struct RnLayout { size_t cand, cscore, order, sboxes, mask, keep, mcount, total; int ncb_cap; };
RnLayout rn_layout(int B, int capK)
{
    RnLayout L;
    L.ncb_cap = (capK + 63) / 64;
    size_t o = 0;
    L.cand = o;   o += align_up((size_t)B * capK * 4, 256);
    L.cscore = o; o += align_up((size_t)B * capK * 4, 256);
    L.order = o;  o += align_up((size_t)B * capK * 4, 256);
    L.sboxes = o; o += align_up((size_t)B * capK * 5 * 4, 256);
    L.mask = o;   o += align_up((size_t)B * capK * L.ncb_cap * 8, 256);
    L.keep = o;   o += align_up((size_t)B * capK * 4, 256);
    L.mcount = o; o += align_up((size_t)B * 4, 256);
    L.total = o;
    return L;
}

void linspace_f32(float start, float end, int steps, float *out)
{
    const float step = (end - start) / (float)(steps - 1);
    const int half = steps / 2;
    for (int i = 0; i < steps; ++i) out[i] = (i < half) ? start + step * (float)i : end - step * (float)(steps - i - 1);
}

}

extern "C" size_t sassd_decode_filter_workspace_bytes(int batch, int n_anchors_total)
{
    const int nblk = cdiv(n_anchors_total, kDfPerBlock);
    return 2 * align_up((size_t)batch * nblk * 4, 256);
}

extern "C" int sassd_decode_filter(const float *box, const float *cls, const float *dir, size_t batch_stride,
                                   int batch, int num_class, int anchors_per_loc, int H, int W,
                                   const float *anchors, const uint8_t *mask, float thr, float *guided,
                                   int32_t *labels, float *scores, int32_t *counts, int capK, int32_t *status,
                                   void *workspace, size_t workspace_bytes, void *stream_)
{
    if (!box || !cls || !dir || !anchors || !mask || !guided || !labels || !counts || !workspace) return SASSD_EINVAL;
    if (batch < 1 || num_class < 1 || anchors_per_loc < 1 || capK < 1) return SASSD_EINVAL;
    DfParams P;
    P.box = box; P.cls = cls; P.dir = dir; P.anchors = anchors; P.mask = mask; P.bs = batch_stride;
    P.B = batch; P.ncls = num_class; P.A = anchors_per_loc; P.HW = H * W; P.Atot = num_class * H * W * anchors_per_loc;
    P.capK = capK; P.thr = thr;
    const int nblk = cdiv(P.Atot, kDfPerBlock);
    if (workspace_bytes < sassd_decode_filter_workspace_bytes(batch, P.Atot)) return SASSD_ENOSPC;
    int *bsum = (int *)workspace;
    hipStream_t stream = (hipStream_t)stream_;
    hipLaunchKernelGGL(df_count_kernel, dim3(nblk, batch), dim3(256), 0, stream, P, nblk, bsum);
    hipLaunchKernelGGL(df_emit_kernel, dim3(nblk, batch), dim3(256), 0, stream, P, nblk, (const int *)bsum, guided,
                       labels, scores, counts, status);
    return sassd_launch_status();
}

extern "C" int sassd_pswarp_sample(const float *feat, int batch, int H, int W, const float *guided,
                                   const int32_t *counts, int capK, float grid_off_x, float grid_off_y,
                                   float spatial_scale, float *logits, void *stream_)
{
    if (!feat || !guided || !counts || !logits || batch < 1 || capK < 1) return SASSD_EINVAL;
    WarpParams P;
    P.feat = feat; P.guided = guided; P.counts = counts; P.logits = logits;
    P.B = batch; P.H = H; P.W = W; P.capK = capK;
    P.offx = grid_off_x; P.offy = grid_off_y; P.scale = spatial_scale;
    linspace_f32(-0.5f, 0.5f, 4, P.lin4);
    linspace_f32(-0.5f, 0.5f, 7, P.lin7);
    hipLaunchKernelGGL(pswarp_kernel, dim3(cdiv(capK, 8), batch), dim3(256), 0, (hipStream_t)stream_, P);
    return sassd_launch_status();
}

extern "C" int sassd_pswarp_sample_bwd(const float *feat, int batch, int H, int W, const float *guided,
                                       const int32_t *counts, int capK, float grid_off_x, float grid_off_y,
                                       float spatial_scale, const float *dlogits, float *dfeat, float *dguided,
                                       void *stream_)
{
    if (!feat || !guided || !counts || !dlogits || !dfeat || batch < 1 || capK < 1) return SASSD_EINVAL;
    WarpParams P;
    P.feat = feat; P.guided = guided; P.counts = counts; P.logits = nullptr;
    P.B = batch; P.H = H; P.W = W; P.capK = capK;
    P.offx = grid_off_x; P.offy = grid_off_y; P.scale = spatial_scale;
    linspace_f32(-0.5f, 0.5f, 4, P.lin4);
    linspace_f32(-0.5f, 0.5f, 7, P.lin7);
    hipLaunchKernelGGL(pswarp_bwd_kernel<true>, dim3(cdiv(capK, 8), batch), dim3(256), 0, (hipStream_t)stream_, P, dlogits,
                       dfeat, dguided);
    return sassd_launch_status();
}

extern "C" size_t sassd_pswarp_sample_bwd_det_workspace_bytes(int batch, int capK)
{
    (void)batch; (void)capK;
    return 0;
}

extern "C" int sassd_pswarp_sample_bwd_det(const float *feat, int batch, int H, int W, const float *guided,
                                           const int32_t *counts, int capK, float grid_off_x, float grid_off_y,
                                           float spatial_scale, const float *dlogits, float *dfeat, float *dguided,
                                           void *ws, size_t ws_bytes, void *stream_)
{
    if (!feat || !guided || !counts || !dlogits || !dfeat || batch < 1 || capK < 1 || H < 1 || W < 1) return SASSD_EINVAL;
    if ((long)H * W >= (1L << 32) - 1 || (long)batch * 28 >= (1L << 31)) return SASSD_EINVAL;
    if (ws_bytes < sassd_pswarp_sample_bwd_det_workspace_bytes(batch, capK)) return SASSD_ENOSPC;
    (void)ws;
    WarpParams P;
    P.feat = feat; P.guided = guided; P.counts = counts; P.logits = nullptr;
    P.B = batch; P.H = H; P.W = W; P.capK = capK;
    P.offx = grid_off_x; P.offy = grid_off_y; P.scale = spatial_scale;
    linspace_f32(-0.5f, 0.5f, 4, P.lin4);
    linspace_f32(-0.5f, 0.5f, 7, P.lin7);
    hipStream_t s = (hipStream_t)stream_;
    hipLaunchKernelGGL(pswarp_dfeat_det_kernel, dim3(batch * 28), dim3(256), 0, s, P, dlogits, dfeat);
    if (dguided)
        hipLaunchKernelGGL(pswarp_bwd_kernel<false>, dim3(cdiv(capK, 8), batch), dim3(256), 0, s, P, dlogits, dfeat,
                           dguided);
    return sassd_launch_status();
}

extern "C" size_t sassd_rescore_nms_workspace_bytes(int batch, int capK) { return rn_layout(batch, capK).total; }

extern "C" int sassd_rescore_nms(const float *guided, const float *logits, const int32_t *labels,
                                 const int32_t *counts, int batch, int capK, float score_thr, float iou_thr,
                                 float *out_boxes, float *out_scores, int32_t *out_labels, int32_t *out_counts,
                                 int capD, int32_t *status, void *workspace, size_t workspace_bytes, void *stream_)
{
    if (!guided || !logits || !labels || !counts || !out_boxes || !out_scores || !out_labels || !out_counts ||
        !workspace)
        return SASSD_EINVAL;
    if (batch < 1 || capK < 1 || capK > 4096 || capD < 1) return SASSD_EINVAL;
    const RnLayout L = rn_layout(batch, capK);
    if (workspace_bytes < L.total) return SASSD_ENOSPC;
    char *w = (char *)workspace;
    RnParams P;
    P.guided = guided; P.logits = logits; P.labels = labels; P.counts = counts;
    P.out_boxes = out_boxes; P.out_scores = out_scores; P.out_labels = out_labels; P.out_counts = out_counts;
    P.status = status; P.capK = capK; P.capD = capD; P.score_thr = score_thr; P.iou_thr = iou_thr;
    P.cand = (int *)(w + L.cand); P.cscore = (float *)(w + L.cscore); P.order = (int *)(w + L.order);
    P.sboxes = (float *)(w + L.sboxes); P.mask = (unsigned long long *)(w + L.mask); P.keep = (int *)(w + L.keep);
    P.ncb_cap = L.ncb_cap;
    int *mcount = (int *)(w + L.mcount);
    hipStream_t stream = (hipStream_t)stream_;
    hipLaunchKernelGGL(rescore_prep_kernel, dim3(batch), dim3(1024), 0, stream, P, mcount);
    hipLaunchKernelGGL(rescore_mask_kernel, dim3(512, batch), dim3(256), 0, stream, P, (const int *)mcount);
    hipLaunchKernelGGL(rescore_final_kernel, dim3(batch), dim3(256), 0, stream, P, (const int *)mcount);
    return sassd_launch_status();
}

struct SealParams {
    const float *boxes; const float *scores; const int32_t *labels; const int32_t *counts;
    const int32_t *seq; const int32_t *status;
    int32_t *rec;
    int B, capD, hdr;
    int magic, pad;
};

__device__ __forceinline__ int seal_count(const SealParams &P, int b)
{
    const int c = P.counts[b];
    return c < 0 ? 0 : (c > P.capD ? P.capD : c);
}

__global__ void __launch_bounds__(256) frame_seal_kernel(SealParams P)
{
    const int N = P.B * P.capD;
    const int i = blockIdx.x * blockDim.x + threadIdx.x;
    if (i < P.hdr) {
        int v = 0;
        if (i == 0) v = P.magic;
        else if (i == 1) v = P.seq[0];
        else if (i == 2) v = P.status[0];
        else if (i == 3) v = P.B;
        else if (i == 4) v = P.capD;
        else if (i < 5 + P.B) v = seal_count(P, i - 5);
        P.rec[i] = v;
    }
    if (i >= N) return;
    float *rb = (float *)(P.rec + P.hdr);
    float *rs = rb + (size_t)7 * N;
    int32_t *rl = (int32_t *)(rs + N);
    if (i < P.pad) rl[N + i] = 0;
#pragma unroll
    for (int k = 0; k < 7; ++k) {
        const int e = i + k * N, row = e / 7, b = row / P.capD;
        rb[e] = (row - b * P.capD) < seal_count(P, b) ? P.boxes[e] : 0.f;
    }
    const int b = i / P.capD;
    const bool live = (i - b * P.capD) < seal_count(P, b);
    rs[i] = live ? P.scores[i] : 0.f;
    rl[i] = live ? P.labels[i] : 0;
}

extern "C" size_t sassd_frame_record_bytes(int batch, int capD)
{
    if (batch < 1 || capD < 1 || (long)batch * capD > (1L << 24)) return 0;
    return 4 * ((size_t)SASSD_FRAME_HEADER_WORDS(batch) + (size_t)9 * batch * capD);
}

extern "C" int sassd_frame_seal(const float *boxes, const float *scores, const int32_t *labels, const int32_t *counts,
                                int batch, int capD, const int32_t *seq, const int32_t *status, void *record,
                                size_t record_bytes, void *stream_)
{
    if (!boxes || !scores || !labels || !counts || !seq || !status || !record) return SASSD_EINVAL;
    const size_t need = sassd_frame_record_bytes(batch, capD);
    if (need == 0 || ((uintptr_t)record & 3)) return SASSD_EINVAL;
    if (record_bytes < need) return SASSD_ENOSPC;
    SealParams P;
    P.boxes = boxes; P.scores = scores; P.labels = labels; P.counts = counts; P.seq = seq; P.status = status;
    P.rec = (int32_t *)record; P.B = batch; P.capD = capD; P.hdr = SASSD_FRAME_HEADER_WORDS(batch);
    P.magic = SASSD_FRAME_MAGIC; P.pad = 0;
    const int threads = batch * capD > P.hdr ? batch * capD : P.hdr;
    hipLaunchKernelGGL(frame_seal_kernel, dim3(cdiv(threads, 256)), dim3(256), 0, (hipStream_t)stream_, P);
    return sassd_launch_status();
}

extern "C" size_t sassd_frame_record_kitti_bytes(int batch, int capD)
{
    const size_t v1 = sassd_frame_record_bytes(batch, capD), an = sassd_frame_annos_bytes(batch, capD);
    return v1 && an ? align_up(v1, 8) + an : 0;
}

extern "C" int sassd_frame_seal_kitti(const float *boxes, const float *scores, const int32_t *labels, const int32_t *counts,
                                      int batch, int capD, const int32_t *seq, const int32_t *status, const double *calib,
                                      void *record, size_t record_bytes, void *stream_)
{
    if (!boxes || !scores || !labels || !counts || !seq || !status || !calib || !record) return SASSD_EINVAL;
    const size_t need = sassd_frame_record_kitti_bytes(batch, capD);
    if (need == 0 || ((uintptr_t)record & 7) || ((uintptr_t)calib & 7)) return SASSD_EINVAL;
    if (record_bytes < need) return SASSD_ENOSPC;
    const size_t v1 = sassd_frame_record_bytes(batch, capD), at = align_up(v1, 8);
    SealParams P;
    P.boxes = boxes; P.scores = scores; P.labels = labels; P.counts = counts; P.seq = seq; P.status = status;
    P.rec = (int32_t *)record; P.B = batch; P.capD = capD; P.hdr = SASSD_FRAME_HEADER_WORDS(batch);
    P.magic = SASSD_FRAME_MAGIC_KITTI; P.pad = (int)((at - v1) / 4);
    const int threads = batch * capD > P.hdr ? batch * capD : P.hdr;
    hipLaunchKernelGGL(frame_seal_kernel, dim3(cdiv(threads, 256)), dim3(256), 0, (hipStream_t)stream_, P);
    const int rc = sassd_launch_status();
    if (rc != SASSD_OK) return rc;
    return sassd_frame_annos(boxes, counts, batch, capD, calib, (char *)record + at, record_bytes - at, stream_);
}

extern "C" int sassd_boxes_overlap_bev(const float *boxes_a, int num_a, const float *boxes_b, int num_b,
                                       float *ans_overlap, void *stream_)
{
    if (!boxes_a || !boxes_b || !ans_overlap || num_a < 0 || num_b < 0) return SASSD_EINVAL;
    const size_t tot = (size_t)num_a * num_b;
    if (tot == 0) return SASSD_OK;
    hipLaunchKernelGGL(pair_kernel<false>, dim3((unsigned)((tot + 255) / 256)), dim3(256), 0, (hipStream_t)stream_,
                       boxes_a, num_a, boxes_b, num_b, ans_overlap);
    return sassd_launch_status();
}

extern "C" int sassd_boxes_iou_bev(const float *boxes_a, int num_a, const float *boxes_b, int num_b, float *ans_iou,
                                   void *stream_)
{
    if (!boxes_a || !boxes_b || !ans_iou || num_a < 0 || num_b < 0) return SASSD_EINVAL;
    const size_t tot = (size_t)num_a * num_b;
    if (tot == 0) return SASSD_OK;
    hipLaunchKernelGGL(pair_kernel<true>, dim3((unsigned)((tot + 255) / 256)), dim3(256), 0, (hipStream_t)stream_,
                       boxes_a, num_a, boxes_b, num_b, ans_iou);
    return sassd_launch_status();
}

extern "C" size_t sassd_nms_workspace_bytes(int n)
{
    const size_t ncb = (size_t)(n + 63) / 64;
    return align_up((size_t)(n > 0 ? n : 1) * (ncb ? ncb : 1) * 8, 256);
}

static int nms_impl(const float *boxes, int n, float thresh, int64_t *keep, int32_t *num_keep, void *workspace,
                    size_t workspace_bytes, void *stream_, int normal)
{
    if (!keep || !num_keep || n < 0 || n > 16384) return SASSD_EINVAL;
    hipStream_t stream = (hipStream_t)stream_;
    if (n == 0) return sassd_hip(hipMemsetAsync(num_keep, 0, 4, stream));
    if (!boxes || !workspace) return SASSD_EINVAL;
    if (workspace_bytes < sassd_nms_workspace_bytes(n)) return SASSD_ENOSPC;
    const int ncb = (n + 63) / 64;
    unsigned long long *mask = (unsigned long long *)workspace;
    hipLaunchKernelGGL(nms_mask_kernel, dim3(cdiv(n * ncb, 4)), dim3(256), 0, stream, boxes, n, ncb, thresh, mask, normal);
    hipLaunchKernelGGL(nms_greedy_kernel, dim3(1), dim3(64), 0, stream, (const unsigned long long *)mask, n, ncb, keep,
                       num_keep);
    return sassd_launch_status();
}

extern "C" int sassd_nms_gpu(const float *boxes, int n, float thresh, int64_t *keep, int32_t *num_keep,
                             void *workspace, size_t workspace_bytes, void *stream)
{
    return nms_impl(boxes, n, thresh, keep, num_keep, workspace, workspace_bytes, stream, 0);
}

extern "C" int sassd_nms_normal_gpu(const float *boxes, int n, float thresh, int64_t *keep, int32_t *num_keep,
                                    void *workspace, size_t workspace_bytes, void *stream)
{
    return nms_impl(boxes, n, thresh, keep, num_keep, workspace, workspace_bytes, stream, 1);
}
```

### sa-ssd_amd/kernels.py

```python
import numpy as np
import torch

from . import _C

_ws_cache = {}

_weights_gen = [0]


def weights_generation():
    return _weights_gen[0]


def bump_weights_generation():
    _weights_gen[0] += 1


def weight_key(w):
    return (w._version, w.data_ptr(), str(w.device), _weights_gen[0])


_ws_scope = [None]


# ... 551 lines not shown
def conv2d_wino4_chain_workspace(b, cmax, h, w, device):
    n = _C.lib().sassd_conv2d_wino4_chain_workspace_bytes(b, cmax, h, w)
    if n == 0:
        raise ValueError("wino4 chain: unsupported shape")
    return torch.empty(n, dtype=torch.uint8, device=device)


def wino4_tile_map(indices, n_ptr, cap, batch, h, w, out=None):
    n = _C.lib().sassd_wino4_tile_map_ints(int(batch), int(h), int(w))
    if n == 0:
        return None
    if out is None:
        out = torch.zeros(n, dtype=torch.int32, device=indices.device)
    _C.check(_C.lib().sassd_wino4_tile_map(_C.ptr(indices), _C.ptr(n_ptr), int(cap), int(batch), int(h), int(w), _C.ptr(out),
                                           _C.stream()), "sassd_wino4_tile_map")
    return out


def conv2d_wino4_chain(x, prev, w_packed, cin, cout, cmax, batch, h, w, scale, shift, relu, y, ws, cfg=None, tile_map=None,
                       prev_tile_map=None):
    _chk_cuda(x, w_packed, scale, shift, y, ws)
    ps, pb, pr = prev if prev is not None else (None, None, False)
    _C.check(_C.lib().sassd_conv2d_wino4_chain(_C.ptr(x), 0 if x is not None else 1, _C.ptr(ps), _C.ptr(pb), 1 if pr else 0,
                                               _C.ptr(w_packed), _C.ptr(scale), _C.ptr(shift), 1 if relu else 0,
                                               _C.ptr(y), batch, cin, cout, cmax, h, w, _C.ptr(tile_map), _C.ptr(prev_tile_map),
                                               DEFAULT_CFG["wino4"] if cfg is None else int(cfg), _C.ptr(ws), ws.numel(),
                                               _C.stream()), "sassd_conv2d_wino4_chain")
    return y


def wino4_sparse_grid(batch, d, h, w, device):
    n = _C.lib().sassd_wino4_sparse_grid_ints(int(batch), int(d), int(h), int(w))
    return torch.full((n,), -1, dtype=torch.int32, device=device) if n else None


def wino4_sparse_prepare(indices, n_ptr, cap, batch, d, h, w, grid, tile_map):
    _chk_cuda(indices, n_ptr, grid, tile_map)
    _C.check(_C.lib().sassd_wino4_sparse_prepare(_C.ptr(indices), _C.ptr(n_ptr), int(cap), int(batch), int(d), int(h), int(w),
                                                 _C.ptr(grid), _C.ptr(tile_map), _C.stream()), "sassd_wino4_sparse_prepare")
    return grid, tile_map


def conv2d_wino4_chain_sparse(feats, d, grid, w_packed, cin, cout, cmax, batch, h, w, scale, shift, relu, y, ws, tile_map,
                              cfg=None):
    _chk_cuda(feats, grid, w_packed, scale, shift, y, ws, tile_map)
    _C.check(_C.lib().sassd_conv2d_wino4_chain_sparse(_C.ptr(feats), int(feats.shape[1]), int(d), _C.ptr(grid), _C.ptr(w_packed),
                                                      _C.ptr(scale), _C.ptr(shift), 1 if relu else 0, _C.ptr(y), batch, cin,
                                                      cout, cmax, h, w, _C.ptr(tile_map),
                                                      DEFAULT_CFG["wino4"] if cfg is None else int(cfg), _C.ptr(ws), ws.numel(),
                                                      _C.stream()), "sassd_conv2d_wino4_chain_sparse")
    return y


def conv2d_wino4_pack_weight_narrow(w):
    _chk_cuda(w)
    cout, cin = w.shape[0], w.shape[1]
    L = _C.lib()
    packed = torch.empty(L.sassd_conv2d_wino4_narrow_packed_floats(cin), dtype=torch.float32, device=w.device)
    _C.check(L.sassd_conv2d_wino4_pack_weight_narrow(_C.ptr(w.contiguous()), cout, cin, _C.ptr(packed), _C.stream()),
             "sassd_conv2d_wino4_pack_weight_narrow")
    return packed


def conv2d_wino4_chain_tail(prev, y_prev, w_packed64, cin, cout, cmax, batch, h, w, scale, shift, relu, y, ws, cfg=None,
                            prev_tile_map=None):
    _chk_cuda(w_packed64, scale, shift, y, ws, y_prev)
    ps, pb, pr = prev
    _C.check(_C.lib().sassd_conv2d_wino4_chain_tail(_C.ptr(ps), _C.ptr(pb), 1 if pr else 0, _C.ptr(y_prev), _C.ptr(w_packed64),
                                                    _C.ptr(scale), _C.ptr(shift), 1 if relu else 0, _C.ptr(y), batch, cin, cout,
                                                    cmax, h, w, _C.ptr(prev_tile_map),
                                                    DEFAULT_CFG["wino4"] if cfg is None else int(cfg), _C.ptr(ws), ws.numel(),
                                                    _C.stream()), "sassd_conv2d_wino4_chain_tail")
    return y


def conv1x1_gemm_supported(cin, cout, h, w):
    return bool(_C.lib().sassd_conv1x1_gemm_supported(int(cin), int(cout), int(h), int(w)))


def conv1x1_gemm_pack_weight(w):
    _chk_cuda(w)
    cout, cin = w.shape[0], w.shape[1]
    packed = torch.empty(cin * cout, dtype=torch.float32, device=w.device)
    _C.check(_C.lib().sassd_conv1x1_gemm_pack_weight(_C.ptr(w.contiguous()), cout, cin, _C.ptr(packed), _C.stream()),
             "sassd_conv1x1_gemm_pack_weight")
    return packed


def conv1x1_gemm_fwd(x, w_packed, cout, scale=None, shift=None, relu=False, y=None, cfg=None):
    _chk_cuda(x, w_packed, scale, shift)
    b, cin, h, w = x.shape
    if y is None:
        y = torch.empty(b, cout, h, w, dtype=torch.float32, device=x.device)
    _C.check(_C.lib().sassd_conv1x1_gemm_fwd(_C.ptr(x), _C.ptr(w_packed), _C.ptr(scale), _C.ptr(shift), 1 if relu else 0,
                                             _C.ptr(y), b, cin, cout, h, w,
                                             DEFAULT_CFG["wino4"] if cfg is None else int(cfg), _C.stream()),
             "sassd_conv1x1_gemm_fwd")
    return y


def conv2d_bf16_supported(cin, cout, h, w):
    return bool(_C.lib().sassd_conv2d_bf16_supported(cin, cout, h, w))


def conv2d_bf16_pack_weight(w):
    _chk_cuda(w)
    cout, cin, kh, kw = w.shape
    assert kh == 3 and kw == 3
    L = _C.lib()
    packed = torch.empty(L.sassd_conv2d_bf16_packed_elems(cin, cout), dtype=torch.int16, device=w.device)
    _C.check(L.sassd_conv2d_bf16_pack_weight(_C.ptr(w.contiguous()), cout, cin, _C.ptr(packed), _C.stream()),
             "sassd_conv2d_bf16_pack_weight")
    return packed


def conv2d_bf16_fwd(x, w_packed, cout, shift=None, y=None, in_affine=None, cfg=0):
    _chk_cuda(x, w_packed, in_affine)
    b, cin, h, w = x.shape
    if y is None:
        y = torch.empty(b, cout, h, w, dtype=torch.float32, device=x.device)
    if cfg:
        assert in_affine is None
        _C.check(_C.lib().sassd_conv2d_bf16_fwd_cfg(_C.ptr(x), _C.ptr(w_packed), _C.ptr(shift) if shift is not None else None,
                                                    _C.ptr(y), b, cin, cout, h, w, int(cfg), _C.stream()), "sassd_conv2d_bf16_fwd_cfg")
        return y
    if in_affine is not None:
        _C.check(_C.lib().sassd_conv2d_bf16_bnrelu_fwd(_C.ptr(x), _C.ptr(in_affine), _C.ptr(w_packed), _C.ptr(shift), _C.ptr(y),
                                                       b, cin, cout, h, w, _C.stream()), "sassd_conv2d_bf16_bnrelu_fwd")
        return y
    _C.check(_C.lib().sassd_conv2d_bf16_fwd(_C.ptr(x), _C.ptr(w_packed), _C.ptr(shift) if shift is not None else None,
                                            _C.ptr(y), b, cin, cout, h, w, _C.stream()), "sassd_conv2d_bf16_fwd")
    return y


def conv1x1_bf16_supported(cin, cout, hw):
    return bool(_C.lib().sassd_conv1x1_bf16_supported(cin, cout, hw))


def conv1x1_bf16_pack_weight(w, transposed=False):
    _chk_cuda(w)
    w2 = w.reshape(w.shape[0], w.shape[1]).contiguous()
    cout, cin = (w2.shape[1], w2.shape[0]) if transposed else (w2.shape[0], w2.shape[1])
    L = _C.lib()
    packed = torch.empty(L.sassd_conv1x1_bf16_packed_elems(cin, cout), dtype=torch.int16, device=w.device)
    _C.check(L.sassd_conv1x1_bf16_pack_weight(_C.ptr(w2), cout, cin, 1 if transposed else 0, _C.ptr(packed), _C.stream()),
             "sassd_conv1x1_bf16_pack_weight")
    return packed


def conv1x1_bf16_fwd(x, w_packed, cout, shift=None, y=None):
    _chk_cuda(x, w_packed)
    b, cin, h, w = x.shape
    if y is None:
        y = torch.empty(b, cout, h, w, dtype=torch.float32, device=x.device)
    _C.check(_C.lib().sassd_conv1x1_bf16_fwd(_C.ptr(x), _C.ptr(w_packed), _C.ptr(shift) if shift is not None else None,
                                             _C.ptr(y), b, cin, cout, h * w, _C.stream()), "sassd_conv1x1_bf16_fwd")
    return y


def conv2d_bf16_infer_supported(cin, cout, h, w):
    return bool(_C.lib().sassd_conv2d_bf16_infer_supported(cin, cout, h, w))


def conv2d_bf16_infer_pack_weight(w):
    _chk_cuda(w)
    cout, cin, kh, kw = w.shape
    assert kh == 3 and kw == 3
    L = _C.lib()
    packed = torch.empty(L.sassd_conv2d_bf16_infer_packed_elems(cin, cout), dtype=torch.int16, device=w.device)
    _C.check(L.sassd_conv2d_bf16_infer_pack_weight(_C.ptr(w.contiguous()), cout, cin, _C.ptr(packed), _C.stream()),
             "sassd_conv2d_bf16_infer_pack_weight")
    return packed


def _infer_out(x, cout, y, out_bf16):
    b, _, h, w = x.shape
    if y is None:
        y = torch.empty(b, cout, h, w, dtype=torch.bfloat16 if out_bf16 else torch.float32, device=x.device)
    assert y.dtype == (torch.bfloat16 if out_bf16 else torch.float32) and y.is_contiguous() and y.shape == (b, cout, h, w)
    return y


def conv2d_bf16_infer_fwd(x, w_packed, cout, scale, shift, relu, y=None, out_bf16=True):
    _chk_cuda(x, w_packed)
    assert x.dtype == torch.bfloat16 and x.is_contiguous()
    b, cin, h, w = x.shape
    y = _infer_out(x, cout, y, out_bf16)
    _C.check(_C.lib().sassd_conv2d_bf16_infer_fwd(_C.ptr(x), _C.ptr(w_packed), _C.ptr(scale), _C.ptr(shift), 1 if relu else 0,
                                                  _C.ptr(y), 1 if out_bf16 else 0, b, cin, cout, h, w, _C.stream()),
             "sassd_conv2d_bf16_infer_fwd")
    return y


def conv1x1_bf16_infer_supported(cin, cout, hw):
    return bool(_C.lib().sassd_conv1x1_bf16_infer_supported(cin, cout, hw))


def conv1x1_bf16_infer_fwd(x, w_packed, cout, scale, shift, relu, y=None, out_bf16=True):
    _chk_cuda(x, w_packed)
    assert x.dtype == torch.bfloat16 and x.is_contiguous()
    b, cin, h, w = x.shape
    y = _infer_out(x, cout, y, out_bf16)
    _C.check(_C.lib().sassd_conv1x1_bf16_infer_fwd(_C.ptr(x), _C.ptr(w_packed), _C.ptr(scale), _C.ptr(shift), 1 if relu else 0,
                                                   _C.ptr(y), 1 if out_bf16 else 0, b, cin, cout, h * w, _C.stream()),
             "sassd_conv1x1_bf16_infer_fwd")
    return y


def conv2d_bwd_weight(x, dy, ksize, dw=None, accumulate=False, bf16=False, x_affine=None):
    _chk_cuda(x, dy, x_affine)
    b, cin, h, w = x.shape
    cout = dy.shape[1]
    L = _C.lib()
    if dw is None:
        dw = torch.empty(cout, cin, ksize, ksize, dtype=torch.float32, device=x.device)
    wsb = L.sassd_conv2d_wgrad_workspace_bytes(b, cin, cout, h, w, ksize)
    ws = workspace("conv2d_wgrad", wsb, x.device)
    if x_affine is not None:
        assert bf16 and w % 2 == 0 and ksize == 3
        _C.check(L.sassd_conv2d_bwd_weight_bf16_bnrelu(_C.ptr(x), _C.ptr(x_affine), _C.ptr(dy), _C.ptr(dw), b, cin, cout, h, w,
                                                       ksize, 1 if accumulate else 0, _C.ptr(ws), wsb, _C.stream()),
                 "sassd_conv2d_bwd_weight_bf16_bnrelu")
        return dw
    fn = L.sassd_conv2d_bwd_weight_bf16 if bf16 and w % 2 == 0 else L.sassd_conv2d_bwd_weight
    _C.check(fn(_C.ptr(x), _C.ptr(dy), _C.ptr(dw), b, cin, cout, h, w, ksize, 1 if accumulate else 0, _C.ptr(ws), wsb,
                _C.stream()), "sassd_conv2d_bwd_weight")
    return dw


def anchor_mask(coors, row_begin_ptr, row_end_ptr, h0, w0, anchors_bv, voxel_size, coors_range, area_threshold,
                mask=None):
    _chk_cuda(coors, row_begin_ptr, row_end_ptr, anchors_bv, mask)
    assert anchors_bv.dtype == torch.float32 and anchors_bv.shape[1] == 4 and coors.dtype == torch.int32
    dev = coors.device
    L = _C.lib()
    n = anchors_bv.shape[0]
    if mask is None:
        mask = torch.empty(n, dtype=torch.uint8, device=dev)
    vs, cr = _f32(voxel_size), _f32(coors_range)
    wsb = L.sassd_anchor_mask_workspace_bytes(h0, w0)
    ws = workspace("anchor_mask", wsb, dev)
    rc = L.sassd_anchor_mask(_C.ptr(coors), _C.ptr(row_begin_ptr), _C.ptr(row_end_ptr), h0, w0, _C.ptr(anchors_bv),
                             n, vs.ctypes.data, cr.ctypes.data, float(area_threshold), _C.ptr(mask), _C.ptr(ws), wsb,
                             _C.stream())
    _C.check(rc, "sassd_anchor_mask")
    return mask


def anchor_mask_batch(coors, row_offsets, batch, h0, w0, anchors_bv, voxel_size, coors_range, area_threshold, mask):
    _chk_cuda(coors, row_offsets, anchors_bv, mask)
    assert anchors_bv.dtype == torch.float32 and anchors_bv.shape[1] == 4 and coors.dtype == torch.int32
    L = _C.lib()
    n = anchors_bv.shape[0]
    vs, cr = _f32(voxel_size), _f32(coors_range)
    wsb = L.sassd_anchor_mask_workspace_bytes(h0, w0) * batch
    ws = workspace("anchor_mask_batch", wsb, coors.device)
    rc = L.sassd_anchor_mask_batch(_C.ptr(coors), _C.ptr(row_offsets), batch, h0, w0, _C.ptr(anchors_bv), n,
                                   vs.ctypes.data, cr.ctypes.data, float(area_threshold), _C.ptr(mask), _C.ptr(ws), wsb,
                                   _C.stream())
    _C.check(rc, "sassd_anchor_mask_batch")
    return mask


def decode_filter(box, cls, dirp, batch_stride, batch, num_class, anchors_per_loc, h, w, anchors, mask, thr, cap_k,
                  out=None, status=None):
    dev = box.device
    L = _C.lib()
    out = out or {}
    guided = out.get("guided")
    if guided is None:
        guided = torch.empty(batch, cap_k, 7, dtype=torch.float32, device=dev)
    labels = out.get("labels")
    if labels is None:
        labels = torch.empty(batch, cap_k, dtype=torch.int32, device=dev)
    scores = out.get("scores")
    if scores is None:
        scores = torch.empty(batch, cap_k, dtype=torch.float32, device=dev)
    counts = out.get("counts")
    if counts is None:
        counts = torch.zeros(batch, dtype=torch.int32, device=dev)
    atot = num_class * h * w * anchors_per_loc
    wsb = L.sassd_decode_filter_workspace_bytes(batch, atot)
    ws = workspace("decode_filter", wsb, dev)
    rc = L.sassd_decode_filter(_C.ptr(box), _C.ptr(cls), _C.ptr(dirp), int(batch_stride), batch, num_class,
                               anchors_per_loc, h, w, _C.ptr(anchors), _C.ptr(mask), float(thr), _C.ptr(guided),
                               _C.ptr(labels), _C.ptr(scores), _C.ptr(counts), cap_k, _C.ptr(status), _C.ptr(ws), wsb,
                               _C.stream())
    _C.check(rc, "sassd_decode_filter")
    return dict(guided=guided, labels=labels, scores=scores, counts=counts)


def pswarp_sample(feat, guided, counts, cap_k, grid_offsets, spatial_scale, logits=None):
    b, parts, h, w = feat.shape
    assert parts == 28, "PSWarp window is 4x7 (ssd_rotate_head.py:374)"
    if logits is None:
        logits = torch.zeros(b, cap_k, dtype=torch.float32, device=feat.device)
    rc = _C.lib().sassd_pswarp_sample(_C.ptr(feat), b, h, w, _C.ptr(guided), _C.ptr(counts), cap_k,
                                      float(grid_offsets[0]), float(grid_offsets[1]), float(spatial_scale),
                                      _C.ptr(logits), _C.stream())
    _C.check(rc, "sassd_pswarp_sample")
    return logits


def pswarp_sample_bwd(feat, guided, counts, cap_k, grid_offsets, spatial_scale, dlogits, deterministic=False):
    b, parts, h, w = feat.shape
    dfeat = torch.zeros_like(feat)
    dg = torch.zeros(b, cap_k, 7, dtype=torch.float32, device=feat.device)
    if deterministic:
        L = _C.lib()
        wsb = L.sassd_pswarp_sample_bwd_det_workspace_bytes(b, cap_k)
        ws = workspace("pswarp_det", wsb, feat.device)
        rc = L.sassd_pswarp_sample_bwd_det(_C.ptr(feat), b, h, w, _C.ptr(guided), _C.ptr(counts), cap_k,
                                           float(grid_offsets[0]), float(grid_offsets[1]), float(spatial_scale),
                                           _C.ptr(dlogits), _C.ptr(dfeat), _C.ptr(dg), _C.ptr(ws), wsb, _C.stream())
        _C.check(rc, "sassd_pswarp_sample_bwd_det")
        return dfeat, dg
    rc = _C.lib().sassd_pswarp_sample_bwd(_C.ptr(feat), b, h, w, _C.ptr(guided), _C.ptr(counts), cap_k,
                                          float(grid_offsets[0]), float(grid_offsets[1]), float(spatial_scale),
                                          _C.ptr(dlogits), _C.ptr(dfeat), _C.ptr(dg), _C.stream())
    _C.check(rc, "sassd_pswarp_sample_bwd")
    return dfeat, dg


def rescore_nms(guided, logits, labels, counts, score_thr, iou_thr, cap_d, out=None, status=None):
    dev = guided.device
    L = _C.lib()
    b, cap_k, _ = guided.shape
    out = out or {}
    boxes = out.get("boxes")
    if boxes is None:
        boxes = torch.empty(b, cap_d, 7, dtype=torch.float32, device=dev)
    scores = out.get("scores")
    if scores is None:
        scores = torch.empty(b, cap_d, dtype=torch.float32, device=dev)
    olabels = out.get("labels")
    if olabels is None:
        olabels = torch.empty(b, cap_d, dtype=torch.int32, device=dev)
    ocounts = out.get("counts")
    if ocounts is None:
        ocounts = torch.zeros(b, dtype=torch.int32, device=dev)
    wsb = L.sassd_rescore_nms_workspace_bytes(b, cap_k)
    ws = workspace("rescore_nms", wsb, dev)
    rc = L.sassd_rescore_nms(_C.ptr(guided), _C.ptr(logits), _C.ptr(labels), _C.ptr(counts), b, cap_k,
                             float(score_thr), float(iou_thr), _C.ptr(boxes), _C.ptr(scores), _C.ptr(olabels),
                             _C.ptr(ocounts), cap_d, _C.ptr(status), _C.ptr(ws), wsb, _C.stream())
    _C.check(rc, "sassd_rescore_nms")
    return dict(boxes=boxes, scores=scores, labels=olabels, counts=ocounts)


def frame_record_bytes(batch, cap_d):
    n = int(_C.lib().sassd_frame_record_bytes(int(batch), int(cap_d)))
    if n == 0:
        raise ValueError("no frame record for batch %d x capD %d" % (batch, cap_d))
    return n


def frame_seal(det, seq, status, record=None):
    boxes, scores, labels, counts = det["boxes"], det["scores"], det["labels"], det["counts"]
    _chk_cuda(boxes, scores, labels, counts, seq, status, record)
    b, cap_d = int(boxes.shape[0]), int(boxes.shape[1])
    nbytes = frame_record_bytes(b, cap_d)
    if record is None:
        record = torch.empty(nbytes, dtype=torch.uint8, device=boxes.device)
    rc = _C.lib().sassd_frame_seal(_C.ptr(boxes), _C.ptr(scores), _C.ptr(labels), _C.ptr(counts), b, cap_d, _C.ptr(seq),
                                   _C.ptr(status), _C.ptr(record), record.numel() * record.element_size(), _C.stream())
    _C.check(rc, "sassd_frame_seal")
    return record


def frame_annos_bytes(batch, cap_d):
    n = int(_C.lib().sassd_frame_annos_bytes(int(batch), int(cap_d)))
    if n == 0:
        raise ValueError("no annotation block for batch %d x capD %d" % (batch, cap_d))
    return n


def frame_record_kitti_bytes(batch, cap_d):
    n = int(_C.lib().sassd_frame_record_kitti_bytes(int(batch), int(cap_d)))
    if n == 0:
        raise ValueError("no frame record for batch %d x capD %d" % (batch, cap_d))
    return n


def _chk_calib(calib, b):
    from .stream import CALIB_DOUBLES
    if calib.dtype != torch.float64 or calib.numel() != b * CALIB_DOUBLES or not calib.is_contiguous():
        raise ValueError("calib must be a contiguous float64 tensor of [%d, %d]" % (b, CALIB_DOUBLES))


def frame_annos(det, calib, annos=None):
    boxes, counts = det["boxes"], det["counts"]
    _chk_cuda(boxes, counts, calib, annos)
    b, cap_d = int(boxes.shape[0]), int(boxes.shape[1])
    _chk_calib(calib, b)
    nbytes = frame_annos_bytes(b, cap_d)
    if annos is None:
        annos = torch.empty(nbytes, dtype=torch.uint8, device=boxes.device)
    rc = _C.lib().sassd_frame_annos(_C.ptr(boxes), _C.ptr(counts), b, cap_d, _C.ptr(calib), _C.ptr(annos),
                                    annos.numel() * annos.element_size(), _C.stream())
    _C.check(rc, "sassd_frame_annos")
    return annos


def frame_seal_kitti(det, seq, status, calib, record=None):
    boxes, scores, labels, counts = det["boxes"], det["scores"], det["labels"], det["counts"]
    _chk_cuda(boxes, scores, labels, counts, seq, status, calib, record)
    b, cap_d = int(boxes.shape[0]), int(boxes.shape[1])
    _chk_calib(calib, b)
    nbytes = frame_record_kitti_bytes(b, cap_d)
    if record is None:
        record = torch.empty(nbytes, dtype=torch.uint8, device=boxes.device)
    rc = _C.lib().sassd_frame_seal_kitti(_C.ptr(boxes), _C.ptr(scores), _C.ptr(labels), _C.ptr(counts), b, cap_d,
                                         _C.ptr(seq), _C.ptr(status), _C.ptr(calib), _C.ptr(record),
                                         record.numel() * record.element_size(), _C.stream())
    _C.check(rc, "sassd_frame_seal_kitti")
    return record


def boxes_overlap_bev(a, b, out=None):
    _chk_cuda(a, b)
    if out is None:
        out = torch.zeros(a.shape[0], b.shape[0], dtype=torch.float32, device=a.device)
    rc = _C.lib().sassd_boxes_overlap_bev(_C.ptr(a), a.shape[0], _C.ptr(b), b.shape[0], _C.ptr(out), _C.stream())
    _C.check(rc, "sassd_boxes_overlap_bev")
    return out


def boxes_iou_bev(a, b, out=None):
    _chk_cuda(a, b)
    if out is None:
        out = torch.zeros(a.shape[0], b.shape[0], dtype=torch.float32, device=a.device)
    rc = _C.lib().sassd_boxes_iou_bev(_C.ptr(a), a.shape[0], _C.ptr(b), b.shape[0], _C.ptr(out), _C.stream())
    _C.check(rc, "sassd_boxes_iou_bev")
    return out


def nms_gpu(boxes_sorted, thresh, normal=False):
    _chk_cuda(boxes_sorted)
    n = boxes_sorted.shape[0]
    dev = boxes_sorted.device
    keep = torch.empty(max(n, 1), dtype=torch.int64, device=dev)
    num = torch.zeros(1, dtype=torch.int32, device=dev)
    L = _C.lib()
    wsb = L.sassd_nms_workspace_bytes(n)
    ws = workspace("nms", wsb, dev)
    fn = L.sassd_nms_normal_gpu if normal else L.sassd_nms_gpu
    rc = fn(_C.ptr(boxes_sorted), n, float(thresh), _C.ptr(keep), _C.ptr(num), _C.ptr(ws), wsb, _C.stream())
    _C.check(rc, "sassd_nms_normal_gpu" if normal else "sassd_nms_gpu")
    return keep, num


def three_nn(unknown, known):
    _chk_cuda(unknown, known)
    n, m = unknown.shape[0], known.shape[0]
    d = torch.empty(n, 3, dtype=torch.float32, device=unknown.device)
    i = torch.empty(n, 3, dtype=torch.int32, device=unknown.device)
    _C.check(_C.lib().sassd_three_nn(n, m, _C.ptr(unknown), _C.ptr(known), _C.ptr(d), _C.ptr(i), _C.stream()),
             "sassd_three_nn")
    return d, i


def three_nn_binned(unknown, known, xy_range, cell, batch_size):
    _chk_cuda(unknown, known)
    n, m = unknown.shape[0], known.shape[0]
    dev = unknown.device
    d2 = torch.empty(n, 3, dtype=torch.float32, device=dev)
    idx = torch.empty(n, 3, dtype=torch.int32, device=dev)
    x0, y0, x1, y1 = [float(v) for v in xy_range]
    nx, ny = max(1, int(np.ceil((x1 - x0) / cell))), max(1, int(np.ceil((y1 - y0) / cell)))
    L = _C.lib()
    wsb = L.sassd_three_nn_binned_workspace_bytes(m, nx, ny, int(batch_size))
    if wsb == 0:
        raise ValueError("three_nn_binned: grid %dx%dx%d too large" % (nx, ny, batch_size))
    ws = workspace("three_nn_binned", wsb, dev)
    _C.check(L.sassd_three_nn_binned(n, m, _C.ptr(unknown), _C.ptr(known), x0, y0, float(cell), nx, ny,
                                     int(batch_size), _C.ptr(d2), _C.ptr(idx), _C.ptr(ws), wsb, _C.stream()),
             "sassd_three_nn_binned")
    return d2, idx


def three_interpolate(points, idx, weight):
    _chk_cuda(points, idx, weight)
    m, c = points.shape
    n = idx.shape[0]
    out = torch.empty(n, c, dtype=torch.float32, device=points.device)
    _C.check(_C.lib().sassd_three_interpolate(c, m, n, _C.ptr(points), _C.ptr(idx), _C.ptr(weight), _C.ptr(out),
                                              _C.stream()), "sassd_three_interpolate")
    return out


def three_interpolate_grad(grad_out, idx, weight, m, deterministic=False, grad_points=None):
    _chk_cuda(grad_out, idx, weight, grad_points)
    n, c = grad_out.shape
    gp = torch.zeros(m, c, dtype=torch.float32, device=grad_out.device) if grad_points is None else grad_points
    if deterministic:
        L = _C.lib()
        wsb = L.sassd_three_interpolate_grad_det_workspace_bytes(n, m)
        ws = workspace("three_interpolate_grad_det", wsb, grad_out.device)
        _C.check(L.sassd_three_interpolate_grad_det(c, n, m, _C.ptr(grad_out), _C.ptr(idx), _C.ptr(weight), _C.ptr(gp),
                                                    _C.ptr(ws), wsb, _C.stream()), "sassd_three_interpolate_grad_det")
        return gp
    _C.check(_C.lib().sassd_three_interpolate_grad(c, n, m, _C.ptr(grad_out), _C.ptr(idx), _C.ptr(weight), _C.ptr(gp),
                                                   _C.stream()), "sassd_three_interpolate_grad")
    return gp


def pts_in_boxes3d(pts, boxes3d):
    _chk_cuda(pts, boxes3d)
    n, m = pts.shape[0], boxes3d.shape[0]
    flag = torch.zeros(m, n, dtype=torch.int32, device=pts.device)
    reg = torch.zeros(n, 3, dtype=torch.float32, device=pts.device)
    _C.check(_C.lib().sassd_pts_in_boxes3d(_C.ptr(pts), n, _C.ptr(boxes3d), m, _C.ptr(flag), _C.ptr(reg),
                                           _C.stream()), "sassd_pts_in_boxes3d")
    return flag, reg


def mfma_probe(a32, b32, a16, b16, ksteps):
    dev = a32.device
    d32 = torch.zeros(32, 32, dtype=torch.float32, device=dev)
    d16 = torch.zeros(16, 16, dtype=torch.float32, device=dev)
    rc = _C.lib().sassd_mfma_probe(_C.ptr(a32), _C.ptr(b32), _C.ptr(d32), _C.ptr(a16), _C.ptr(b16), _C.ptr(d16),
                                   ksteps, _C.stream())
    _C.check(rc, "sassd_mfma_probe")
    return d32, d16


def grad_sumsq(grad_flat, out=None, deterministic=False):
    _chk_cuda(grad_flat)
    out = torch.empty(1, dtype=torch.float32, device=grad_flat.device) if out is None else out
    if deterministic:
        L = _C.lib()
        wsb = L.sassd_grad_sumsq_det_workspace_bytes(grad_flat.numel())
        ws = workspace("grad_sumsq_det", wsb, grad_flat.device)
        _C.check(L.sassd_grad_sumsq_det(_C.ptr(grad_flat), grad_flat.numel(), _C.ptr(out), _C.ptr(ws), wsb, _C.stream()),
                 "sassd_grad_sumsq_det")
        return out
    _C.check(_C.lib().sassd_grad_sumsq(_C.ptr(grad_flat), grad_flat.numel(), _C.ptr(out), _C.stream()),
             "sassd_grad_sumsq")
    return out


def adam_step(param, grad, exp_avg, exp_avg_sq, sumsq, lr, beta1, beta2, eps, weight_decay, step, max_norm=0.0,
              grad_scale=1.0):
    _chk_cuda(param, grad, exp_avg, exp_avg_sq)
    _C.check(_C.lib().sassd_adam_step(_C.ptr(param), _C.ptr(grad), _C.ptr(exp_avg), _C.ptr(exp_avg_sq),
                                      param.numel(), _C.ptr(sumsq), lr, beta1, beta2, eps, weight_decay, int(step),
                                      max_norm, grad_scale, _C.stream()), "sassd_adam_step")


def rotate_iou_eval(boxes, query_boxes, criterion=-1):
    _chk_cuda(boxes, query_boxes)
    n, k = boxes.shape[0], query_boxes.shape[0]
    out = torch.zeros(n, k, dtype=torch.float32, device=boxes.device)
    _C.check(_C.lib().sassd_rotate_iou_eval(_C.ptr(boxes), n, _C.ptr(query_boxes), k, int(criterion), _C.ptr(out),
                                            _C.stream()), "sassd_rotate_iou_eval")
    return out


_gt_offset_cache = {}


def gt_offsets(counts, device):
    key = (tuple(int(c) for c in counts), str(device))
    t = _gt_offset_cache.get(key)
    if t is None:
        if len(_gt_offset_cache) > 4096:
            _gt_offset_cache.clear()
        off = np.zeros(len(key[0]) + 1, np.int32)
        off[1:] = np.cumsum(key[0])
        t = torch.from_numpy(off).to(device)
        _gt_offset_cache[key] = t
    return t


def assign_targets(anchors, anchor_mask, gt_boxes, gt_classes, gt_ok, gt_off, matched, unmatched, labels, targets,
                   num_pos, zero_num_pos=True, out_stride=None, best=None, overlaps=None, overlap_offsets=None):
    per_sample = anchors.dim() == 3
    a = anchors.shape[-2]
    b = gt_off.shape[0] - 1
    t = int(gt_boxes.shape[0]) if gt_boxes is not None else 0
    _chk_cuda(anchors, anchor_mask, gt_boxes, gt_classes, gt_ok, gt_off, overlaps, overlap_offsets)
    L = _C.lib()
    wsb = L.sassd_assign_targets_workspace_bytes(b, a, t)
    ws = workspace("assign_targets", wsb, anchors.device)
    _C.check(L.sassd_assign_targets(_C.ptr(anchors), 1 if per_sample else 0, _C.ptr(anchor_mask), a, b,
                                    _C.ptr(gt_boxes) if t else None, _C.ptr(gt_classes), _C.ptr(gt_ok),
                                    _C.ptr(gt_off), t, _C.ptr(overlaps), _C.ptr(overlap_offsets), float(matched),
                                    float(unmatched), _C.ptr(labels), _C.ptr(targets), _C.ptr(best),
                                    int(out_stride if out_stride is not None else a), _C.ptr(num_pos),
                                    1 if zero_num_pos else 0, _C.ptr(ws), wsb, _C.stream()), "sassd_assign_targets")


def rpn_loss(box_preds, cls_preds, dir_preds, labels, targets, anchors, num_pos):
    _chk_cuda(box_preds, cls_preds, dir_preds, labels, targets, anchors, num_pos)
    b, a = labels.shape
    nc = cls_preds.shape[-1]
    dev = box_preds.device
    gbox, gcls = torch.empty_like(box_preds), torch.empty_like(cls_preds)
    gdir = torch.empty_like(dir_preds) if dir_preds is not None else None
    sums = torch.empty(3, dtype=torch.float32, device=dev)
    L = _C.lib()
    wsb = L.sassd_rpn_loss_workspace_bytes(b, a)
    ws = workspace("rpn_loss", wsb, dev)
    _C.check(L.sassd_rpn_loss(_C.ptr(box_preds), _C.ptr(cls_preds), _C.ptr(dir_preds), nc, _C.ptr(labels),
                              _C.ptr(targets), _C.ptr(anchors), 1 if anchors.dim() == 3 else 0, _C.ptr(num_pos), a, b,
                              _C.ptr(gbox), _C.ptr(gcls), _C.ptr(gdir), _C.ptr(sums), _C.ptr(ws), wsb, _C.stream()),
# ... 228 lines not shown
```

### sa-ssd_amd/pipeline.py

```python
import numpy as np

import torch

from . import kernels as K
from . import anchors as A
from .stream import CALIB_DOUBLES, stage_layout

BN_EPS = 1e-3

VXNET = [
    ("conv0.0", "conv0.1", "subm", 4, 16, "subm0"), ("conv0.3", "conv0.4", "subm", 16, 16, "subm0"),
    ("down0.0", "down0.1", "down", 16, 32, "down0"),
    ("conv1.0", "conv1.1", "subm", 32, 32, "subm1"), ("conv1.3", "conv1.4", "subm", 32, 32, "subm1"),
    ("down1.0", "down1.1", "down", 32, 64, "down1"),
    ("conv2.0", "conv2.1", "subm", 64, 64, "subm2"), ("conv2.3", "conv2.4", "subm", 64, 64, "subm2"),
    ("conv2.6", "conv2.7", "subm", 64, 64, "subm2"),
    ("down2.0", "down2.1", "down", 64, 64, "down2"),
    ("conv3.0", "conv3.1", "subm", 64, 64, "subm3"), ("conv3.3", "conv3.4", "subm", 64, 64, "subm3"),
    ("conv3.6", "conv3.7", "subm", 64, 64, "subm3"),
    ("extra_conv.0", "extra_conv.1", "1x1", 64, 64, None),
]


def fold_bn(sd, prefix, eps=BN_EPS):
    g, b = sd[prefix + ".weight"].float(), sd[prefix + ".bias"].float()
    m, v = sd[prefix + ".running_mean"].float(), sd[prefix + ".running_var"].float()
    scale = g / torch.sqrt(v + eps)
    return scale.contiguous(), (b - m * scale).contiguous()


def _bev_weight(sd, i, D3):
    w = sd["neck.fcn.conv%d.weight" % i].float()
    if i == 0:
        cout, cin = w.shape[:2]
        c = cin // D3
        w = w.view(cout, c, D3, 3, 3).permute(0, 2, 1, 3, 4).reshape(cout, cin, 3, 3)
    return w.contiguous()


class InferencePlan:

    def __init__(self, state_dict, *, batch_size=1, num_class=1, voxel_size=(0.05, 0.05, 0.1),
                 point_cloud_range=(0, -40., -3., 70.4, 40., 1.), max_num_points=5, max_voxels=20000,
                 sparse_shape=(40, 1600, 1408), anchors=None, anchors_bv=None, anchor_area_threshold=1,
                 anchors_per_loc=2, grid_offsets=(0., 40.), featmap_stride=0.4, rpn_thr=0.1, score_thr=0.3,
                 iou_thr=0.1, cap_k=4096, cap_d=512, device=None, level_cap_factor=2, overlap=True, winograd=True,
                 fused_rulebooks=True, chain_bev=True, pyramid_persistent=False, spconv_cfg=None, wino4_cfg=None,
                 skip_inactive_tiles=True, rb_sync_levels=(0, 1, 2, 3), ps_tail=False, precision="fp32",
                 sparse_precision="fp32", dense_entry=False):
        if precision not in ("fp32", "bf16"):
            raise ValueError("precision must be 'fp32' or 'bf16', got %r" % (precision,))
        if sparse_precision not in ("fp32", "bf16"):
            raise ValueError("sparse_precision must be 'fp32' or 'bf16', got %r" % (sparse_precision,))
        self.precision, self.bf16 = precision, precision == "bf16"
        self.sparse_precision, self.sparse_bf16 = sparse_precision, sparse_precision == "bf16"
        dev = torch.device(device if device is not None else "cuda:0")
        self.dev, self.B, self.ncls, self.A = dev, int(batch_size), int(num_class), int(anchors_per_loc)
        self.voxel_size = np.asarray(voxel_size, np.float32)
        self.pc_range = np.asarray(point_cloud_range, np.float32)
        self.T, self.max_voxels = int(max_num_points), int(max_voxels)
        self.shape0 = tuple(int(s) for s in sparse_shape)
        self.rpn_thr, self.score_thr, self.iou_thr = float(rpn_thr), float(score_thr), float(iou_thr)
        self.grid_offsets, self.spatial_scale = grid_offsets, 1.0 / featmap_stride
        self.area_thr = anchor_area_threshold
        self.capK, self.capD = int(cap_k), int(cap_d)
        sd = {k: v.detach().to(dev) for k, v in state_dict.items()}

        self.shapes = [self.shape0]
        for _ in range(3):
            self.shapes.append(K.conv_out_shape(self.shapes[-1]))
        cap0 = self.B * self.max_voxels
        self.caps = [cap0] + [cap0 * level_cap_factor] * 3
        D3, self.H, self.W = self.shapes[3]
        self.D3 = D3

        self.sp = []
        lvl = 0
        for wname, bnname, kind, cin, cout, key in VXNET:
            w = sd["neck.backbone.%s.weight" % wname].float()
            k = 1 if kind == "1x1" else 27
            lvl += kind == "down"
            if self.sparse_bf16:
                if not K.spconv_bf16_supported(k, cin, cout, self.caps[lvl]):
                    raise ValueError("sparse_precision='bf16': %s (%s, %d -> %d) at a capacity of %d rows is not supported by "
                                     "the bf16 sparse-conv kernels" % (wname, kind, cin, cout, self.caps[lvl]))
                wp = K.spconv_bf16_pack_weight(w.reshape(k, cin, cout).contiguous())
            else:
                wp = K.spconv_pack_weight(w.reshape(k, cin, cout).contiguous())
            scale, shift = fold_bn(sd, "neck.backbone.%s" % bnname)
            self.sp.append((kind, cin, cout, key, wp, scale, shift))
        if self.sparse_bf16 and not K.densify_bf16_supported(64, self.shapes[3]):
            raise ValueError("sparse_precision='bf16': the dense map (64 x %d channels) on a %dx%d BEV map is not supported by "
                             "the bf16 densify" % (D3, self.H, self.W))

        hw = torch.cat([sd["rpn_head.conv_box.weight"], sd["rpn_head.conv_cls.weight"],
                        sd["rpn_head.conv_dir_cls.weight"]], 0).float().contiguous()
        hb = torch.cat([sd["rpn_head.conv_box.bias"], sd["rpn_head.conv_cls.bias"],
                        sd["rpn_head.conv_dir_cls.bias"]], 0).float().contiguous()
        self.n_box = sd["rpn_head.conv_box.weight"].shape[0]
        self.n_cls = sd["rpn_head.conv_cls.weight"].shape[0]
        self.n_dir = sd["rpn_head.conv_dir_cls.weight"].shape[0]
        self.head_c = hw.shape[0]
        self.head_b = hb
        w0 = sd["extra_head.convs.0.weight"].float().contiguous()
        self.ps_parts = w0.shape[0]
        self.ps_s0, self.ps_b0 = fold_bn(sd, "extra_head.convs.1")
        w1 = sd["extra_head.convs.3.weight"].float().contiguous()
        if self.bf16:
            self._dense_weights_bf16(sd, hw, w0, w1)
        else:
            self._dense_weights_fp32(sd, hw, w0, w1, winograd, chain_bev, wino4_cfg, ps_tail)

        self.Atot = self.ncls * self.H * self.W * self.A
        if anchors is not None:
            an = np.asarray(anchors, np.float32).reshape(-1, 7)
            assert an.shape[0] == self.Atot, (an.shape, self.Atot)
            self.anchors = torch.from_numpy(np.ascontiguousarray(an)).to(dev)
            bv = anchors_bv if anchors_bv is not None else A.rbbox2d_to_near_bbox(an[:, [0, 1, 3, 4, 6]])
            self.anchors_bv = torch.from_numpy(np.ascontiguousarray(bv, np.float32)).to(dev)
        else:
            self.anchors = self.anchors_bv = None

        B, H, W = self.B, self.H, self.W
        i32, f32 = torch.int32, torch.float32
        z = lambda *s, dt=f32: torch.zeros(*s, dtype=dt, device=dev)
        self.status = z(1, dt=i32)
        self.row_off = z(B + 1, dt=i32)
        self.vnum = z(B, dt=i32)
        self.n = [self.row_off[B:B + 1]] + [z(1, dt=i32) for _ in range(3)]
        self.idx = [z(c, 4, dt=i32) for c in self.caps]
        self.tables = [K.HashTable(c, dev) for c in self.caps]
        self.nbr = {key: z(self.caps[lvl], 27, dt=i32)
                    for key, lvl in (("subm0", 0), ("down0", 1), ("subm1", 1), ("down1", 2), ("subm2", 2),
                                     ("down2", 3), ("subm3", 3))}
        fdt = torch.bfloat16 if self.sparse_bf16 else f32
        self.feat = [z(max(self.caps), 64, dt=fdt), z(max(self.caps), 64, dt=fdt)]
        self.mean = z(self.caps[0], 4)
        mdt = torch.bfloat16 if self.bf16 else f32
        self._dense_shape, self._dense_dt = (B, 64 * D3, H, W), mdt
        self._dense = None
        self.act = [z(B, 256, H, W, dt=mdt) for _ in range(3)]
        self.head_out = z(B, self.head_c, H, W)
        self.ps_t = [z(B, self.ps_parts, H, W, dt=mdt), z(B, self.ps_parts, H, W)]
        self.mask = z(B, self.Atot, dt=torch.uint8)
        self.df = dict(guided=z(B, self.capK, 7), labels=z(B, self.capK, dt=i32), scores=z(B, self.capK),
                       counts=z(B, dt=i32))
        self.logits = z(B, self.capK)
        self.det = dict(boxes=z(B, self.capD, 7), scores=z(B, self.capD), labels=z(B, self.capD, dt=i32),
                        counts=z(B, dt=i32))
        self.middle = {}
        self.pyr = None
        if fused_rulebooks:
            self.pyr = K.RulebookPyramid(self.idx, self.n, self.caps, self.shape0, B,
                                         [self.nbr["subm%d" % l] for l in range(4)],
                                         [None] + [self.nbr["down%d" % l] for l in range(3)], self.status)
        self.pyramid_persistent = bool(pyramid_persistent)
        self.spconv_cfg, self.wino4_cfg = spconv_cfg, wino4_cfg
        self.graph = None
        self.record = None
        self.raw_cap = None
        self._stage_block = None
        self._wsid = id(self)
        self.overlap = bool(overlap)
        self.side = torch.cuda.Stream(device=dev) if self.overlap else None
        self.rb_ev = {k: torch.cuda.Event() for k in self.nbr}
        self.mask_ev = torch.cuda.Event()
        self.tile_map = None
        if skip_inactive_tiles and not self.bf16 and self.bev[0][5] == 4:
            n_ints = K._C.lib().sassd_wino4_tile_map_ints(B, H, W)
            if n_ints:
                self.tile_map = z(n_ints, dt=i32)
        self.tmap_ev = torch.cuda.Event()
        self.sparse_grid = None
        if not dense_entry and self.tile_map is not None and not self.sparse_bf16 and not self.chain[0]:
            self.sparse_grid = K.wino4_sparse_grid(B, D3, H, W, dev)
        self.sparse_entry = self.sparse_grid is not None
        self._sparse_frame = False
        self._tmap_joined = False
        if not self.sparse_entry:
            self._dense_map()
        self.rb_sync_levels = tuple(sorted(int(l) for l in rb_sync_levels))
        assert self.rb_sync_levels and self.rb_sync_levels[-1] == 3
        self.prof = None
        self.prof_sparse_layers = False

    def _dense_weights_fp32(self, sd, hw, w0, w1, winograd, chain_bev, wino4_cfg, ps_tail):
        D3, dev = self.D3, self.dev
        self.bev = []
        for i in range(8):
            w = _bev_weight(sd, i, D3)
            scale, shift = fold_bn(sd, "neck.fcn.bn%d" % i)
            wino = 0
            if winograd and w.shape[2] == 3:
                if winograd != 2 and K.conv2d_wino4_supported(w.shape[1], w.shape[0], self.H, self.W):
                    wino = 4
                elif K.conv2d_wino_supported(w.shape[1], w.shape[0], self.H, self.W):
                    wino = 2
            if w.shape[2] == 1 and winograd and K.conv1x1_gemm_supported(w.shape[1], w.shape[0], self.H, self.W):
                wino = 1
            wp = (K.conv2d_wino4_pack_weight(w.contiguous()) if wino == 4 else
                  K.conv2d_wino_pack_weight(w.contiguous()) if wino == 2 else
                  K.conv1x1_gemm_pack_weight(w.contiguous()) if wino == 1 else K.conv2d_pack_weight(w.contiguous()))
            self.bev.append((wp, w.shape[0], w.shape[2], scale, shift, wino))
        self.wino4_ws = None
        self.bev_cin = [int(sd["neck.fcn.conv%d.weight" % i].shape[1]) for i in range(8)]
        self.chain = [False] * 8
        if any(l[5] == 4 for l in self.bev):
            self.cmax = max(max(self.bev_cin[i], self.bev[i][1]) for i in range(8) if self.bev[i][5] == 4)
            self.wino4_ws = K.conv2d_wino4_chain_workspace(self.B, self.cmax, self.H, self.W, dev)
            for i in range(1, 8):
                self.chain[i] = bool(chain_bev and self.bev[i][5] == 4 and self.bev[i - 1][5] == 4 and i - 1 != 6 and
                                     self.bev[i - 1][1] == self.bev_cin[i] and self.bev[i - 1][1] == self.bev[i][1] and
                                     K.conv2d_wino4_chain_supported(self.bev_cin[i], self.bev[i][1], self.H, self.W))
        self.head_narrow = K.conv1x1_narrow_supported(hw.shape[1], hw.shape[0])
        self.head_w = K.conv1x1_narrow_pack_weight(hw) if self.head_narrow else K.conv2d_pack_weight(hw)
        self.ps_w0 = K.conv2d_pack_weight(w0)
        self.ps_tail = bool(ps_tail and chain_bev and self.bev[6][5] == 4 and self.chain[6] and self.ps_parts <= 64 and
                            w0.shape[2] == 3 and w0.shape[1] == self.bev[6][1] and not ((wino4_cfg or 0) & 0xff))
        self.ps_w0t = K.conv2d_wino4_pack_weight_narrow(w0) if self.ps_tail else None
        self.ps_narrow = K.conv1x1_narrow_supported(w1.shape[1], w1.shape[0])
        self.ps_w1 = K.conv1x1_narrow_pack_weight(w1) if self.ps_narrow else K.conv2d_pack_weight(w1)

    def _dense_weights_bf16(self, sd, hw, w0, w1):
        H, W = self.H, self.W

        def need(ok, what):
            if not ok:
                raise ValueError("precision='bf16': %s on a %dx%d BEV map is not supported by the bf16 inference kernels"
                                 % (what, H, W))
        need(K.densify_bf16_supported(64, self.shapes[3]), "the dense map (64 x %d channels)" % self.D3)
        self.bev, self.chain, self.wino4_ws, self.ps_tail, self.ps_w0t = [], [False] * 8, None, False, None
        self.head_narrow = self.ps_narrow = False
        self.bev_cin = [int(sd["neck.fcn.conv%d.weight" % i].shape[1]) for i in range(8)]
        self.bev16 = []
        for i in range(8):
            w = _bev_weight(sd, i, self.D3)
            cout, cin, k = int(w.shape[0]), int(w.shape[1]), int(w.shape[2])
            if k == 3:
                need(K.conv2d_bf16_infer_supported(cin, cout, H, W), "BEV conv%d (3x3, %d -> %d)" % (i, cin, cout))
                wp = K.conv2d_bf16_infer_pack_weight(w)
            else:
                need(k == 1 and K.conv1x1_bf16_infer_supported(cin, cout, H * W),
                     "BEV conv%d (%dx%d, %d -> %d)" % (i, k, k, cin, cout))
                wp = K.conv1x1_bf16_pack_weight(w)
            scale, shift = fold_bn(sd, "neck.fcn.bn%d" % i)
            self.bev16.append((wp, cout, k, scale, shift))
        need(K.conv1x1_bf16_infer_supported(hw.shape[1], hw.shape[0], H * W), "the fused SSD head (%d -> %d)" % (hw.shape[1], hw.shape[0]))
        self.head_w = K.conv1x1_bf16_pack_weight(hw)
        need(w0.shape[2] == 3 and K.conv2d_bf16_infer_supported(w0.shape[1], w0.shape[0], H, W),
             "the part-sensitive conv (%d -> %d)" % (w0.shape[1], w0.shape[0]))
        self.ps_w0 = K.conv2d_bf16_infer_pack_weight(w0)
        need(K.conv1x1_bf16_infer_supported(w1.shape[1], w1.shape[0], H * W), "the part-sensitive 1x1 (%d -> %d)" % (w1.shape[1], w1.shape[0]))
        self.ps_w1 = K.conv1x1_bf16_pack_weight(w1)

    def _dense_map(self):
        if self._dense is None:
            self._dense = torch.zeros(*self._dense_shape, dtype=self._dense_dt, device=self.dev)
        return self._dense

    @property
    def dense(self):
        if self._sparse_frame:
            K.densify(self.sp_out, self.idx[3], self.n[3], self.caps[3], self.shapes[3], self.B, 1, self._dense_map())
        return self._dense_map()

    def _ev(self):
        e = torch.cuda.Event(enable_timing=True)
        e.record()
        return e

    def _seg(self, name, e0):
        if self.prof is not None:
            self.prof.setdefault(name, []).append((e0, self._ev()))

    def voxelize(self, clouds, n_dev=None):
        assert len(clouds) == self.B
        e0 = self._ev() if self.prof is not None else None
        self.row_off.fill_(0)
        for b, pts in enumerate(clouds):
            K.voxelize(pts, self.voxel_size, self.pc_range, self.T, self.max_voxels, batch_idx=b, coors_cols=4,
                       want_voxels=False, want_mean=True, nfeat=4,
                       out=dict(coors=self.idx[0], mean=self.mean, voxel_num=self.vnum[b:b + 1],
                                num_points=self._numpts()),
                       row_offset=self.row_off[b:b + 2], status=self.status, cap=self.caps[0],
                       n_dev=None if n_dev is None else n_dev[b:b + 1])
        self._seg("voxelize", e0)

    def _numpts(self):
        if not hasattr(self, "_np"):
            self._np = torch.zeros(self.caps[0], dtype=torch.int32, device=self.dev)
        return self._np

    def load_voxels(self, voxel_feats, coors4):
        m = voxel_feats.shape[0]
        assert m <= self.caps[0]
        self.mean[:m].copy_(voxel_feats)
        self.idx[0][:m].copy_(coors4.int())
        self.row_off.fill_(0)
        bc = torch.bincount(coors4[:, 0].long(), minlength=self.B).cumsum(0).int()
        self.row_off[1:].copy_(bc)

    def rulebooks(self):
        B = self.B
        if self.pyr is not None:
            if self.pyramid_persistent:
                self.pyr.build(persistent=True)
                for ev in self.rb_ev.values():
                    ev.record()
                return
            for lvl in range(4):
                self._rulebook_level(lvl)
            return
        self.tables[0].build(self.idx[0], self.n[0], self.shapes[0], B, self.status)
        for lvl in range(4):
            K.rulebook_subm(self.idx[lvl], self.n[lvl], self.caps[lvl], self.shapes[lvl], B, self.tables[lvl],
                            self.nbr["subm%d" % lvl])
            self.rb_ev["subm%d" % lvl].record()
            if lvl < 3:
                K.rulebook_conv(self.idx[lvl], self.n[lvl], self.caps[lvl], self.shapes[lvl], B, self.tables[lvl],
                                self.caps[lvl + 1], self.idx[lvl + 1], self.n[lvl + 1], self.nbr["down%d" % lvl],
                                self.status)
                self.rb_ev["down%d" % lvl].record()
                self.tables[lvl + 1].build(self.idx[lvl + 1], self.n[lvl + 1], self.shapes[lvl + 1], B, self.status)

    def _rulebook_level(self, lvl):
        self.pyr.build(lvl, lvl + 1)
        self.rb_ev["subm%d" % lvl].record()
        if lvl > 0:
            self.rb_ev["down%d" % (lvl - 1)].record()

    def backbone(self, keep_middle=False, anchors_mask=None, densify=True, masks=True, rulebooks=True, convs=True):
        main = torch.cuda.current_stream(self.dev)
        e0 = self._ev() if self.prof is not None else None
        sparse = self.sparse_entry and densify and not keep_middle
        self._sparse_frame, self._tmap_joined = sparse, False
        if self.overlap:
            self.side.wait_stream(main)
            with torch.cuda.stream(self.side):
                if rulebooks:
                    self.rulebooks()
                if self.tile_map is not None and densify:
                    self._tile_map(sparse)
                    self.tmap_ev.record()
                if masks:
                    self.anchor_masks(anchors_mask)
                self.mask_ev.record()
        else:
            if rulebooks:
                self.rulebooks()
            if self.tile_map is not None and densify and not sparse:
                self._tile_map(False)
        if not convs:
            return
        x = self.mean
        lvl = 0
        cur = 0
        covered = -1
        for li, (kind, cin, cout, key, wp, scale, shift) in enumerate(self.sp):
            y = self.feat[cur]
            if kind == "down":
                lvl += 1
            if key is not None and self.overlap and rulebooks and lvl > covered:
                upto = min([l for l in self.rb_sync_levels if l >= lvl] or [3])
                main.wait_event(self.rb_ev["subm%d" % upto])
                covered = upto
            el = self._ev() if self.prof is not None and self.prof_sparse_layers else None
            if self.sparse_bf16:
                K.spconv_fwd_bf16(x, None if key is None else self.nbr[key], self.n[lvl], self.caps[lvl], wp,
                                  1 if key is None else 27, cin, cout, scale, shift, True, y)
            elif kind == "subm" or kind == "down":
                K.spconv_fwd(x, self.nbr[key], self.n[lvl], self.caps[lvl], wp, 27, cin, cout, scale, shift, True, y,
                             cfg=self.spconv_cfg)
            else:
                K.spconv_fwd(x, None, self.n[lvl], self.caps[lvl], wp, 1, cin, cout, scale, shift, True, y, cfg=self.spconv_cfg)
            if el is not None:
                self._seg("sparse_conv%d" % li, el)
            if keep_middle:
                self.middle[li] = (y.clone(), lvl, cout)
            x = y
            cur ^= 1
        self.sp_out = x
        self._seg("sparse", e0)
        if not densify:
            return
        e1 = self._ev() if self.prof is not None else None
        if sparse:
            if self.overlap:
                main.wait_event(self.tmap_ev)
                self._tmap_joined = True
            else:
                self._tile_map(True)
        elif self.sparse_bf16:
            K.densify_from_bf16(x, self.idx[3], self.n[3], self.caps[3], self.shapes[3], self.B, 1, self._dense_map(),
                                  out_bf16=self.bf16)
        elif self.bf16:
            K.densify_bf16(x, self.idx[3], self.n[3], self.caps[3], self.shapes[3], self.B, 1, self._dense_map())
        else:
            K.densify(x, self.idx[3], self.n[3], self.caps[3], self.shapes[3], self.B, 1, self._dense_map())
        self._seg("densify", e1)

    def _tile_map(self, sparse):
        if sparse:
            K.wino4_sparse_prepare(self.idx[3], self.n[3], self.caps[3], self.B, self.D3, self.H, self.W, self.sparse_grid,
                                   self.tile_map)
        else:
            K.wino4_tile_map(self.idx[3], self.n[3], self.caps[3], self.B, self.H, self.W, out=self.tile_map)

    def bev_and_heads(self):
        if self.bf16:
            return self._bev_and_heads_bf16()
        x = None if self._sparse_frame else self._dense_map()
        for i, (wp, cout, ks, scale, shift, wino) in enumerate(self.bev):
            y = self.act[i % 2] if i < 7 else self.act[2]
            e0 = self._ev() if self.prof is not None else None
            if wino == 4:
                keep = (i + 1 < 8 and self.chain[i + 1]) or (i == 6 and self.ps_tail)
                prev = self.bev[i - 1][3:5] + (True,) if self.chain[i] else None
                tmap = self.tile_map if i == 0 else None
                ptmap = self.tile_map if (i == 1 and self.chain[1]) else None
                if tmap is not None and self.overlap and not self._tmap_joined:
                    torch.cuda.current_stream(self.dev).wait_event(self.tmap_ev)
                if i == 0 and self._sparse_frame:
                    K.conv2d_wino4_chain_sparse(self.sp_out, self.D3, self.sparse_grid, wp, self.bev_cin[0], cout, self.cmax,
                                                self.B, self.H, self.W, scale, shift, True, None if keep else y, self.wino4_ws,
                                                tmap, cfg=self.wino4_cfg)
                else:
                    K.conv2d_wino4_chain(None if self.chain[i] else x, prev, wp, self.bev_cin[i], cout, self.cmax, self.B,
                                         self.H, self.W, scale, shift, True, None if keep else y, self.wino4_ws,
                                         cfg=self.wino4_cfg, tile_map=tmap, prev_tile_map=ptmap)
            elif wino == 2:
                K.conv2d_wino_fwd(x, wp, cout, scale, shift, True, y)
            elif wino == 1:
                K.conv1x1_gemm_fwd(x, wp, cout, scale, shift, True, y, cfg=self.wino4_cfg)
            else:
                K.conv2d_fwd(x, wp, cout, ks, scale, shift, True, y)
            if i == 6 and self.ps_tail:
                K.conv2d_wino4_chain_tail(self.bev[6][3:5] + (True,), y, self.ps_w0t, cout, self.ps_parts, self.cmax, self.B,
                                          self.H, self.W, self.ps_s0, self.ps_b0, True, self.ps_t[0], self.wino4_ws,
                                          cfg=self.wino4_cfg)
            self._seg("bev_conv%d" % i, e0)
            x = y
            if i == 6:
                self.conv6 = y
        self.x = x
        e0 = self._ev() if self.prof is not None else None
        if self.head_narrow:
            K.conv1x1_narrow_fwd(x, self.head_w, self.head_c, None, self.head_b, False, self.head_out)
        else:
            K.conv2d_fwd(x, self.head_w, self.head_c, 1, None, self.head_b, False, self.head_out)
        if not self.ps_tail:
            K.conv2d_fwd(self.conv6, self.ps_w0, self.ps_parts, 3, self.ps_s0, self.ps_b0, True, self.ps_t[0])
        if self.ps_narrow:
            K.conv1x1_narrow_fwd(self.ps_t[0], self.ps_w1, self.ps_parts, None, None, False, self.ps_t[1])
        else:
            K.conv2d_fwd(self.ps_t[0], self.ps_w1, self.ps_parts, 1, None, None, False, self.ps_t[1])
        self._seg("heads", e0)

    def _bev_and_heads_bf16(self):
        x = self._dense_map()
        for i, (wp, cout, ks, scale, shift) in enumerate(self.bev16):
            y = self.act[i % 2] if i < 7 else self.act[2]
            e0 = self._ev() if self.prof is not None else None
            if ks == 3:
                K.conv2d_bf16_infer_fwd(x, wp, cout, scale, shift, True, y)
            else:
                K.conv1x1_bf16_infer_fwd(x, wp, cout, scale, shift, True, y)
            self._seg("bev_conv%d" % i, e0)
            x = y
            if i == 6:
                self.conv6 = y
        self.x = x
        e0 = self._ev() if self.prof is not None else None
        K.conv1x1_bf16_infer_fwd(x, self.head_w, self.head_c, None, self.head_b, False, self.head_out, out_bf16=False)
        K.conv2d_bf16_infer_fwd(self.conv6, self.ps_w0, self.ps_parts, self.ps_s0, self.ps_b0, True, self.ps_t[0])
        K.conv1x1_bf16_infer_fwd(self.ps_t[0], self.ps_w1, self.ps_parts, None, None, False, self.ps_t[1], out_bf16=False)
        self._seg("heads", e0)

    def anchor_masks(self, masks=None):
        if masks is not None:
            self.mask.copy_(masks.view(self.B, -1).to(torch.uint8))
            return
        H0, W0 = self.shape0[1], self.shape0[2]
        K.anchor_mask_batch(self.idx[0], self.row_off, self.B, H0, W0, self.anchors_bv, self.voxel_size, self.pc_range,
                            self.area_thr, self.mask)

    def post(self):
        e0 = self._ev() if self.prof is not None else None
        HW = self.H * self.W
        ho = self.head_out
        base = ho.view(-1)
        box = base
        cls = base[self.n_box * HW:]
        dirp = base[(self.n_box + self.n_cls) * HW:]
        K.decode_filter(box, cls, dirp, self.head_c * HW, self.B, self.ncls, self.A, self.H, self.W, self.anchors,
                        self.mask, self.rpn_thr, self.capK, self.df, self.status)
        K.pswarp_sample(self.ps_t[1], self.df["guided"], self.df["counts"], self.capK, self.grid_offsets,
                        self.spatial_scale, self.logits)
        K.rescore_nms(self.df["guided"], self.logits, self.df["labels"], self.df["counts"], self.score_thr,
                      self.iou_thr, self.capD, self.det, self.status)
        self._seg("post", e0)

    def sparse_work(self):
        n = [int(t.item()) for t in self.n]
        pairs = {}
        lvl_of = dict(subm0=0, down0=1, subm1=1, down1=2, subm2=2, down2=3, subm3=3)
        for key, t in self.nbr.items():
            pairs[key] = int((t[:n[lvl_of[key]]] >= 0).sum().item())
        bgs = bmin = flops = rb = 0
        lvl = 0
        seen = set()
        for kind, cin, cout, key, *_ in self.sp:
            if kind == "down":
                nin, lvl = n[lvl], lvl + 1
            else:
                nin = n[lvl]
            nout = n[lvl]
            p = pairs[key] if key else nout
            k = 27 if key else 1
            bgs += 4 * p * (cin + cout) + 8 * p + 4 * k * cin * cout + 4 * nout * cout
            bmin += 4 * nin * cin + 4 * nout * cout + 4 * k * cin * cout + 8 * p
            flops += 2 * p * cin * cout
            if key and key not in seen:
                seen.add(key)
                rb += (16 * nin + 8 * p) if kind == "subm" else (16 * nin + 16 * nout + 8 * p)
        return dict(n=n, pairs=pairs, bytes_gs=bgs, bytes_min=bmin, flops=flops, rulebook_bytes=rb)

    def _tail(self, anchors_mask):
        self.bev_and_heads()
        if self.overlap:
            torch.cuda.current_stream(self.dev).wait_event(self.mask_ev)
        else:
            self.anchor_masks(anchors_mask)
        self.post()
        return self.det

    def run_from_points(self, clouds, anchors_mask=None):
        with K.ws_scope(self._wsid):
            self.voxelize(clouds)
            self.backbone(anchors_mask=anchors_mask)
            return self._tail(anchors_mask)

    def run_from_voxels(self, voxel_feats, coors4, anchors_mask=None):
        with K.ws_scope(self._wsid):
            self.load_voxels(voxel_feats, coors4)
            self.backbone(anchors_mask=anchors_mask)
            return self._tail(anchors_mask)

    def capture(self, points_cap, ndim=4, stages=("voxelize", "backbone", "tail"), seal=False, raw_cap=None, annos=False):
        dev = self.dev
        if annos and not seal:
            raise ValueError("annos=True writes the annotation block into the frame record: it needs seal=True")
        self.pts_cap = int(points_cap)
        self.raw_cap = None if raw_cap is None else int(raw_cap)
        if self.raw_cap is not None and (self.raw_cap < 1 or "voxelize" not in stages):
            raise ValueError("raw_cap must be >= 1 and needs the voxelize stage")
        self.pts_in = [torch.zeros(self.pts_cap, ndim, dtype=torch.float32, device=dev) for _ in range(self.B)]
        L = stage_layout(self.B, self.raw_cap is not None, annos, seal)
        block = self._stage_block = torch.zeros(L["total"], dtype=torch.uint8, device=dev)
        counts = block[L["counts"]:L["total"]].view(torch.int32)
        if seal:
            self._seq = block[L["seq"]:L["counts"]].view(torch.int32)
        if annos:
            self.calib = block[L["calib"]:L["words"]].view(torch.float64).view(self.B, CALIB_DOUBLES)
        if self.raw_cap is not None:
            self.raw_in = [torch.zeros(self.raw_cap, ndim, dtype=torch.float32, device=dev) for _ in range(self.B)]
            self.crop_planes = block[L["planes"]:L["calib"]].view(torch.float64).view(self.B, 6, 4)
            self.crop_f32_math = False
            self.nraw = counts
            self.npts = torch.zeros(self.B, dtype=torch.int32, device=dev)
        else:
            self.npts = counts
        if annos:
            self.record = torch.zeros(K.frame_record_kitti_bytes(self.B, self.capD), dtype=torch.uint8, device=dev)
        elif seal:
            self.record = torch.zeros(K.frame_record_bytes(self.B, self.capD), dtype=torch.uint8, device=dev)
        assert self.prof is None, "per-stage event timing and graph capture exclude each other"

        def frame():
            with K.ws_scope(self._wsid):
                if self.raw_cap is not None:
                    for b in range(self.B):
                        K.crop_polytope(self.raw_in[b], self.nraw[b:b + 1], self.crop_planes[b], self.crop_f32_math,
                                        self.pts_in[b], self.npts[b:b + 1], self.status)
                if "voxelize" in stages:
                    self.voxelize(self.pts_in, n_dev=self.npts)
                if "backbone" in stages:
                    self.backbone()
                elif "sparse" in stages:
                    self.backbone(densify=False, masks=False)
                elif "sparse_convs" in stages:
                    self.backbone(densify=False, masks=False, rulebooks=False)
                elif "pyramid" in stages:
                    self.backbone(densify=False, masks=False, convs=False)
                if "tail" in stages:
                    self._tail(None)
                elif self.overlap:
                    torch.cuda.current_stream(self.dev).wait_event(self.mask_ev)
                if annos:
                    K.frame_seal_kitti(self.det, self._seq, self.status, self.calib, self.record)
                elif seal:
                    K.frame_seal(self.det, self._seq, self.status, self.record)

        cap = torch.cuda.Stream(device=dev)
        cap.wait_stream(torch.cuda.current_stream(dev))
        with torch.cuda.stream(cap):
            frame()
            cap.synchronize()
            self.graph = K.Graph().capture(frame)
        self._frame_fn = frame
        self._graph_ws = K.scoped_workspaces(self._wsid)
        torch.cuda.current_stream(dev).wait_stream(cap)
        return self.graph

    def stage_inputs(self, clouds):
        if self.raw_cap is not None:
            raise RuntimeError("a plan captured with raw_cap is fed through raw_in / nraw / crop_planes (sassd.stream.FrameStream)")
        for b, pts in enumerate(clouds or ()):
            n = pts.shape[0]
            if n > self.pts_cap:
                raise ValueError("cloud %d has %d points, the captured graph was sized for %d (plan.capture(points_cap))"
                                 % (b, n, self.pts_cap))
            self.pts_in[b][:n].copy_(pts, non_blocking=True)
            self.npts[b:b + 1].fill_(n)

    def run_graph(self, clouds=None):
        if clouds is not None:
            self.stage_inputs(clouds)
        self.graph.launch()
        return self.det

    def results(self):
        counts = self.det["counts"].cpu().numpy()
        st = int(self.status.item())
        if st:
            raise RuntimeError("sassd pipeline status flags 0x%x (capacity overflow / hash full)" % st)
        out = []
        for b in range(self.B):
            k = int(counts[b])
            if k == 0:
                out.append((None, None, None))
                continue
            out.append((self.det["boxes"][b, :k].cpu().numpy(), self.det["scores"][b, :k].cpu().numpy(),
                        self.det["labels"][b, :k].cpu().numpy().astype(np.int64)))
        return out
```

Before: 1017 frames/s.

## Compute PS-warp head only at pixels sampled by proposal boxes

Instead of running the dense 3x3 conv plus 1x1 conv for the part-sensitive head over the whole BEV map, the pipeline now marks the bilinear sample pixels touched by decoded proposals, compacts them into a pixel list, and runs a fused sparse 3x3+1x1 MFMA kernel only at those pixels. The aim is to cut the dense part-head compute and memory traffic down to the touched pixels. It adds mark/compact kernels to the post-processing path and moves the part-head onto the critical path after decode_filter. The kernel grid is sized for the full map and relies on early exit, and the output buffer stays zero at untouched pixels, which pswarp never reads.

```diff
diff --git a/include/sassd.h b/include/sassd.h
--- a/include/sassd.h
+++ b/include/sassd.h
@@ -250,6 +250,14 @@
                         const int32_t *counts, int capK, float grid_off_x, float grid_off_y,
                         float spatial_scale, float *logits, void *stream);
 
+size_t sassd_ps_pixel_list_ints(int batch, int H, int W);
+int sassd_ps_pixel_list(const float *guided, const int32_t *counts, int capK, int batch, int H, int W,
+                        float grid_off_x, float grid_off_y, float spatial_scale, int32_t *list, void *stream);
+int sassd_ps_head_sampled_supported(int Cin, int parts);
+int sassd_ps_head_sampled(const float *x, const float *w_packed, const float *scale0, const float *shift0, int relu0,
+                          const float *wT, const float *scale1, const float *shift1, int relu1, const int32_t *list,
+                          float *y, int batch, int Cin, int parts, int H, int W, void *stream);
+
 int sassd_pswarp_sample_bwd(const float *feat, int batch, int H, int W, const float *guided,
                             const int32_t *counts, int capK, float grid_off_x, float grid_off_y,
                             float spatial_scale, const float *dlogits, float *dfeat, float *dguided,
diff --git a/sa-ssd_amd/_C.py b/sa-ssd_amd/_C.py
--- a/sa-ssd_amd/_C.py
+++ b/sa-ssd_amd/_C.py
@@ -85,6 +85,10 @@
     "sassd_decode_filter": (_I, [_P, _P, _P, _SZ, _I, _I, _I, _I, _I, _P, _P, _F, _P, _P, _P, _P, _I, _P, _P, _SZ, _P]),
     "sassd_pswarp_sample": (_I, [_P, _I, _I, _I, _P, _P, _I, _F, _F, _F, _P, _P]),
     "sassd_pswarp_sample_bwd": (_I, [_P, _I, _I, _I, _P, _P, _I, _F, _F, _F, _P, _P, _P, _P]),
+    "sassd_ps_pixel_list_ints": (_SZ, [_I, _I, _I]),
+    "sassd_ps_pixel_list": (_I, [_P, _P, _I, _I, _I, _I, _F, _F, _F, _P, _P]),
+    "sassd_ps_head_sampled_supported": (_I, [_I, _I]),
+    "sassd_ps_head_sampled": (_I, [_P, _P, _P, _P, _I, _P, _P, _P, _I, _P, _P, _I, _I, _I, _I, _I, _P]),
     "sassd_rescore_nms_workspace_bytes": (_SZ, [_I, _I]),
     "sassd_rescore_nms": (_I, [_P, _P, _P, _P, _I, _I, _F, _F, _P, _P, _P, _P, _I, _P, _P, _SZ, _P]),
     "sassd_frame_record_bytes": (_SZ, [_I, _I]),
diff --git a/sa-ssd_amd/csrc/conv2d.hip b/sa-ssd_amd/csrc/conv2d.hip
--- a/sa-ssd_amd/csrc/conv2d.hip
+++ b/sa-ssd_amd/csrc/conv2d.hip
@@ -500,3 +500,146 @@
 #undef SASSD_NARROW
     return sassd_launch_status();
 }
+
+namespace {
+struct PsSampledParams {
+    const float *x, *wp, *scale0, *shift0, *wT, *scale1, *shift1;
+    const int32_t *counts, *pix;
+    float *y;
+    int Cin, parts, CO, H, W, HW, relu0, relu1;
+};
+
+constexpr int kPsRing = 4;
+
+__global__ void __launch_bounds__(256) ps_sampled_kernel(PsSampledParams P)
+{
+    constexpr int KC = 8, BMC = 32;
+    __shared__ float red[4][16][64];
+    __shared__ float hbuf[32][33];
+    const int b = blockIdx.y;
+    const int n = min(max(P.counts[b], 0), P.HW);
+    const int i0 = blockIdx.x * 32;
+    if (i0 >= n) return;
+    const int tid = threadIdx.x, lane = tid & 63;
+    const int wave = __builtin_amdgcn_readfirstlane(tid >> 6);
+    const int32_t *pl = P.pix + (size_t)b * P.HW;
+
+    int off[9];
+    unsigned vmask = 0;
+    {
+        const int i = i0 + (lane & 31);
+        int p = i < n ? pl[i] : -1;
+        const bool ok = p >= 0 && p < P.HW;
+        p = ok ? p : 0;
+        const int py = p / P.W, px = p - py * P.W;
+#pragma unroll
+        for (int tap = 0; tap < 9; ++tap) {
+            const int yy = py + tap / 3 - 1, xx = px + tap % 3 - 1;
+            const bool in = ok && yy >= 0 && yy < P.H && xx >= 0 && xx < P.W;
+            off[tap] = (in ? yy * P.W + xx : p) + (lane >> 5) * P.HW;
+            vmask |= in ? 1u << tap : 0u;
+        }
+    }
+    const __amdgpu_buffer_rsrc_t xr = __builtin_amdgcn_make_buffer_rsrc((void *)(P.x + (size_t)b * P.Cin * P.HW), 0,
+                                                                         P.Cin * P.HW * 4, 0x00020000);
+    const __amdgpu_buffer_rsrc_t wr = __builtin_amdgcn_make_buffer_rsrc((void *)P.wp, 0, P.Cin * 9 * BMC * 4, 0x00020000);
+#pragma unroll
+    for (int tap = 0; tap < 9; ++tap) off[tap] *= 4;
+    const int xso = 2 * wave * P.HW * 4, wso = 2 * wave * BMC * 4;
+    const int nchunk = P.Cin / KC;
+
+    f32x16 acc;
+#pragma unroll
+    for (int r = 0; r < 16; ++r) acc[r] = 0.f;
+
+    float av[kPsRing][9], bv[kPsRing][9];
+    auto gather = [&](int ch, float (&a)[9], float (&v)[9]) {
+        const int xo = xso + ch * KC * P.HW * 4, wo = wso + ch * 9 * KC * BMC * 4;
+#pragma unroll
+        for (int tap = 0; tap < 9; ++tap) {
+            v[tap] = __builtin_bit_cast(float, __builtin_amdgcn_raw_buffer_load_b32(xr, off[tap], xo, 0));
+            a[tap] = __builtin_bit_cast(float, __builtin_amdgcn_raw_buffer_load_b32(wr, lane * 4 + tap * KC * BMC * 4, wo, 0));
+        }
+    };
+    auto mma = [&](const float (&a)[9], const float (&v)[9]) {
+        __builtin_amdgcn_sched_barrier(0);
+#pragma unroll
+        for (int tap = 0; tap < 9; ++tap)
+            acc = __builtin_amdgcn_mfma_f32_32x32x2f32(a[tap], ((vmask >> tap) & 1u) ? v[tap] : 0.f, acc, 0, 0, 0);
+        __builtin_amdgcn_sched_barrier(0);
+    };
+#pragma unroll
+    for (int u = 0; u < kPsRing - 1; ++u) gather(u, av[u], bv[u]);
+    int ch = 0;
+    for (; ch < nchunk - kPsRing; ch += kPsRing) {
+#pragma unroll
+        for (int u = 0; u < kPsRing; ++u) {
+            gather(ch + u + kPsRing - 1, av[(u + kPsRing - 1) % kPsRing], bv[(u + kPsRing - 1) % kPsRing]);
+            mma(av[u], bv[u]);
+        }
+    }
+    gather(ch + kPsRing - 1, av[kPsRing - 1], bv[kPsRing - 1]);
+#pragma unroll
+    for (int u = 0; u < kPsRing; ++u) mma(av[u], bv[u]);
+
+#pragma unroll
+    for (int r = 0; r < 16; ++r) red[wave][r][lane] = acc[r];
+    __syncthreads();
+#pragma unroll
+    for (int q = 0; q < 4; ++q) {
+        const int r = wave + 4 * q;
+        const int co = (r & 3) + 8 * (r >> 2) + 4 * (lane >> 5);
+        float v = red[0][r][lane] + red[1][r][lane] + red[2][r][lane] + red[3][r][lane];
+        if (co < P.parts) {
+            v = v * (P.scale0 ? P.scale0[co] : 1.f) + (P.shift0 ? P.shift0[co] : 0.f);
+            if (P.relu0) v = fmaxf(v, 0.f);
+        }
+        hbuf[co][lane & 31] = v;
+    }
+    __syncthreads();
+
+    const int pi = tid & 31;
+    const int i = i0 + pi;
+    const int p = i < n ? pl[i] : -1;
+    const bool ok = p >= 0 && p < P.HW;
+    const int cq = (P.parts + 3) / 4;
+    for (int j = tid >> 5; j < P.parts; j += 8) {
+        float part[4];
+#pragma unroll
+        for (int w = 0; w < 4; ++w) {
+            float a = 0.f;
+            const int c1 = min(w * cq + cq, P.parts);
+            for (int c = w * cq; c < c1; ++c) a = fmaf(hbuf[c][pi], P.wT[(size_t)c * P.CO + j], a);
+            part[w] = a;
+        }
+        float s = (part[0] + part[1]) + (part[2] + part[3]);
+        s = s * (P.scale1 ? P.scale1[j] : 1.f) + (P.shift1 ? P.shift1[j] : 0.f);
+        if (P.relu1) s = fmaxf(s, 0.f);
+        if (ok) P.y[((size_t)b * P.parts + j) * P.HW + p] = s;
+    }
+}
+}
+
+extern "C" int sassd_ps_head_sampled_supported(int Cin, int parts)
+{
+    return Cin >= 32 && Cin % 32 == 0 && parts >= 1 && parts <= 32 ? 1 : 0;
+}
+
+extern "C" int sassd_ps_head_sampled(const float *x, const float *w_packed, const float *scale0, const float *shift0,
+                                     int relu0, const float *wT, const float *scale1, const float *shift1, int relu1,
+                                     const int32_t *list, float *y, int batch, int Cin, int parts, int H, int W,
+                                     void *stream_)
+{
+    if (!x || !w_packed || !wT || !list || !y || batch < 1 || H < 1 || W < 2) return SASSD_EINVAL;
+    if (!sassd_ps_head_sampled_supported(Cin, parts) || ((uintptr_t)list & 15)) return SASSD_EINVAL;
+    if ((size_t)batch * H * W > ((size_t)1 << 30) || (size_t)Cin * H * W >= ((size_t)1 << 29)) return SASSD_EINVAL;
+    PsSampledParams P;
+    P.x = x; P.wp = w_packed; P.scale0 = scale0; P.shift0 = shift0; P.wT = wT; P.scale1 = scale1; P.shift1 = shift1;
+    P.counts = list; P.pix = list + (batch + 3) / 4 * 4;
+    P.y = y;
+    P.Cin = Cin; P.parts = parts; P.CO = sassd_conv1x1_narrow_pad(parts); P.H = H; P.W = W; P.HW = H * W;
+    P.relu0 = relu0; P.relu1 = relu1;
+    hipLaunchKernelGGL(ps_sampled_kernel, dim3((unsigned)cdiv(P.HW, 32), (unsigned)batch), dim3(256), 0,
+                       (hipStream_t)stream_, P);
+    return sassd_launch_status();
+}
diff --git a/sa-ssd_amd/csrc/heads.hip b/sa-ssd_amd/csrc/heads.hip
--- a/sa-ssd_amd/csrc/heads.hip
+++ b/sa-ssd_amd/csrc/heads.hip
@@ -119,6 +119,38 @@
     float lin4[4], lin7[7];
 };
 
+struct PsTap {
+    float ct, st, xx, yy;
+    int x0, y0, x1, y1;
+    float wx0, wx1, wy0, wy1;
+    bool inr;
+    bool xin0, xin1, yin0, yin1;
+};
+
+__device__ __forceinline__ PsTap ps_tap(const WarpParams &P, int b, int box, int ix, int iy)
+{
+    PsTap t;
+    const float *g = P.guided + ((size_t)b * P.capK + box) * 7;
+    const float xg = g[0], yg = g[1], wg = g[3], lg = g[4], rg = g[6];
+    const float ct = cosf(rg), st = sinf(rg);
+    const float xx = P.lin4[ix] * wg, yy = P.lin7[iy] * lg;
+    const float x = xx * ct + yy * st + xg;
+    const float y = yy * ct - xx * st + yg;
+    const float u = (x + P.offx) * P.scale, v = (y + P.offy) * P.scale;
+    const float gx = u / (float)(P.W - 1) * 2.f - 1.f, gy = v / (float)(P.H - 1) * 2.f - 1.f;
+    float fx = (gx + 1.f) / 2.f * (float)(P.W - 1), fy = (gy + 1.f) / 2.f * (float)(P.H - 1);
+    t.inr = fx > -1.f && fx < (float)P.W && fy > -1.f && fy < (float)P.H;
+    fx = fminf(fmaxf(fx, -2.f), (float)P.W + 1.f);
+    fy = fminf(fmaxf(fy, -2.f), (float)P.H + 1.f);
+    const float x0f = floorf(fx), y0f = floorf(fy);
+    t.x0 = (int)x0f; t.y0 = (int)y0f; t.x1 = t.x0 + 1; t.y1 = t.y0 + 1;
+    t.wx1 = fx - x0f; t.wx0 = (x0f + 1.f) - fx; t.wy1 = fy - y0f; t.wy0 = (y0f + 1.f) - fy;
+    t.xin0 = t.x0 >= 0 && t.x0 < P.W; t.xin1 = t.x1 >= 0 && t.x1 < P.W;
+    t.yin0 = t.y0 >= 0 && t.y0 < P.H; t.yin1 = t.y1 >= 0 && t.y1 < P.H;
+    t.ct = ct; t.st = st; t.xx = xx; t.yy = yy;
+    return t;
+}
+
 __global__ void __launch_bounds__(256) pswarp_kernel(WarpParams P)
 {
     const int b = blockIdx.y;
@@ -127,24 +159,12 @@
     const int k = threadIdx.x & 31;
     float val = 0.f;
     if (box < K && k < 28) {
-        const float *g = P.guided + ((size_t)b * P.capK + box) * 7;
-        const float xg = g[0], yg = g[1], wg = g[3], lg = g[4], rg = g[6];
-        const float ct = cosf(rg), st = sinf(rg);
         const int ix = k / 7, iy = k - ix * 7;
-        const float xx = P.lin4[ix] * wg, yy = P.lin7[iy] * lg;
-        const float x = xx * ct + yy * st + xg;
-        const float y = yy * ct - xx * st + yg;
-        const float u = (x + P.offx) * P.scale, v = (y + P.offy) * P.scale;
-        const float gx = u / (float)(P.W - 1) * 2.f - 1.f, gy = v / (float)(P.H - 1) * 2.f - 1.f;
-        float fx = (gx + 1.f) / 2.f * (float)(P.W - 1), fy = (gy + 1.f) / 2.f * (float)(P.H - 1);
-        fx = fminf(fmaxf(fx, -2.f), (float)P.W + 1.f);
-        fy = fminf(fmaxf(fy, -2.f), (float)P.H + 1.f);
-        const float x0f = floorf(fx), y0f = floorf(fy);
-        const int x0 = (int)x0f, y0 = (int)y0f, x1 = x0 + 1, y1 = y0 + 1;
-        const float wx1 = fx - x0f, wx0 = (x0f + 1.f) - fx, wy1 = fy - y0f, wy0 = (y0f + 1.f) - fy;
+        const PsTap t = ps_tap(P, b, box, ix, iy);
+        const int x0 = t.x0, y0 = t.y0, x1 = t.x1, y1 = t.y1;
+        const float wx0 = t.wx0, wx1 = t.wx1, wy0 = t.wy0, wy1 = t.wy1;
+        const bool xin0 = t.xin0, xin1 = t.xin1, yin0 = t.yin0, yin1 = t.yin1;
         const float *im = P.feat + ((size_t)b * 28 + k) * P.H * P.W;
-        const bool xin0 = x0 >= 0 && x0 < P.W, xin1 = x1 >= 0 && x1 < P.W;
-        const bool yin0 = y0 >= 0 && y0 < P.H, yin1 = y1 >= 0 && y1 < P.H;
         if (yin0 && xin0) val += im[(size_t)y0 * P.W + x0] * (wx0 * wy0);
         if (yin0 && xin1) val += im[(size_t)y0 * P.W + x1] * (wx1 * wy0);
         if (yin1 && xin0) val += im[(size_t)y1 * P.W + x0] * (wx0 * wy1);
@@ -153,6 +173,50 @@
 #pragma unroll
     for (int o = 16; o >= 1; o >>= 1) val += __shfl_xor(val, o, 32);
     if (box < K && k == 0) P.logits[(size_t)b * P.capK + box] = val / 28.f;
+}
+
+constexpr int kPsBlock = 1024;
+inline size_t ps_list_head(int B) { return align_up((size_t)B, 4); }
+inline size_t ps_flag_stride(size_t HW) { return align_up(HW, 16); }
+inline size_t ps_flag_off(int B, size_t HW) { return ps_list_head(B) + align_up((size_t)B * HW, 4); }
+
+__global__ void __launch_bounds__(256) ps_mark_kernel(WarpParams P, unsigned char *__restrict__ flags, int fstride)
+{
+    const int b = blockIdx.y;
+    const int K = min(P.counts[b], P.capK);
+    const int box = blockIdx.x * 8 + (threadIdx.x >> 5);
+    const int k = threadIdx.x & 31;
+    if (box < K && k < 28) {
+        const int ix = k / 7, iy = k - ix * 7;
+        const PsTap t = ps_tap(P, b, box, ix, iy);
+        unsigned char *f = flags + (size_t)b * fstride;
+        if (t.yin0 && t.xin0) f[(size_t)t.y0 * P.W + t.x0] = 1;
+        if (t.yin0 && t.xin1) f[(size_t)t.y0 * P.W + t.x1] = 1;
+        if (t.yin1 && t.xin0) f[(size_t)t.y1 * P.W + t.x0] = 1;
+        if (t.yin1 && t.xin1) f[(size_t)t.y1 * P.W + t.x1] = 1;
+    }
+}
+
+__global__ void __launch_bounds__(kPsBlock) ps_compact_kernel(const unsigned char *__restrict__ flags, int fstride, int HW,
+                                                              int32_t *__restrict__ counts, int32_t *__restrict__ pix)
+{
+    __shared__ int wsum[17];
+    const int b = blockIdx.y;
+    const unsigned char *f = flags + (size_t)b * fstride;
+    const int t0 = blockIdx.x * kPsBlock;
+    int before = 0;
+    for (int i = threadIdx.x; i < t0 / 16; i += kPsBlock) {
+        const uint4 w = ((const uint4 *)f)[i];
+        before += __popc(w.x) + __popc(w.y) + __popc(w.z) + __popc(w.w);
+    }
+    int base;
+    block_exclusive_scan(before, wsum, &base);
+    const int t = t0 + threadIdx.x;
+    const int on = t < HW ? (int)f[t] : 0;
+    int total;
+    const int j = base + block_exclusive_scan(on, wsum, &total);
+    if (on) pix[(size_t)b * HW + j] = t;
+    if (blockIdx.x == gridDim.x - 1 && threadIdx.x == 0) counts[b] = base + total;
 }
 
 template <bool kDfeat>
@@ -165,28 +229,17 @@
     const int k = threadIdx.x & 31;
     float gxg = 0.f, gyg = 0.f, gw = 0.f, gl = 0.f, gr = 0.f;
     if (box < K && k < 28) {
-        const float *g = P.guided + ((size_t)b * P.capK + box) * 7;
-        const float xg = g[0], yg = g[1], wg = g[3], lg = g[4], rg = g[6];
-        const float ct = cosf(rg), st = sinf(rg);
         const int ix = k / 7, iy = k - ix * 7;
-        const float xx = P.lin4[ix] * wg, yy = P.lin7[iy] * lg;
-        const float x = xx * ct + yy * st + xg;
-        const float y = yy * ct - xx * st + yg;
-        const float u = (x + P.offx) * P.scale, v = (y + P.offy) * P.scale;
-        const float gx = u / (float)(P.W - 1) * 2.f - 1.f, gy = v / (float)(P.H - 1) * 2.f - 1.f;
-        float fx = (gx + 1.f) / 2.f * (float)(P.W - 1), fy = (gy + 1.f) / 2.f * (float)(P.H - 1);
-        const bool inr = fx > -1.f && fx < (float)P.W && fy > -1.f && fy < (float)P.H;
-        fx = fminf(fmaxf(fx, -2.f), (float)P.W + 1.f);
-        fy = fminf(fmaxf(fy, -2.f), (float)P.H + 1.f);
-        const float x0f = floorf(fx), y0f = floorf(fy);
-        const int x0 = (int)x0f, y0 = (int)y0f, x1 = x0 + 1, y1 = y0 + 1;
-        const float wx1 = fx - x0f, wx0 = (x0f + 1.f) - fx, wy1 = fy - y0f, wy0 = (y0f + 1.f) - fy;
+        const PsTap t = ps_tap(P, b, box, ix, iy);
+        const float ct = t.ct, st = t.st, xx = t.xx, yy = t.yy;
+        const bool inr = t.inr;
+        const int x0 = t.x0, y0 = t.y0, x1 = t.x1, y1 = t.y1;
+        const float wx0 = t.wx0, wx1 = t.wx1, wy0 = t.wy0, wy1 = t.wy1;
+        const bool xin0 = t.xin0, xin1 = t.xin1, yin0 = t.yin0, yin1 = t.yin1;
         const float go = dlogits[(size_t)b * P.capK + box] / 28.f;
         const size_t plane = ((size_t)b * 28 + k) * P.H * P.W;
         const float *im = P.feat + plane;
         float *di = dfeat + plane;
-        const bool xin0 = x0 >= 0 && x0 < P.W, xin1 = x1 >= 0 && x1 < P.W;
-        const bool yin0 = y0 >= 0 && y0 < P.H, yin1 = y1 >= 0 && y1 < P.H;
         float v00 = 0.f, v01 = 0.f, v10 = 0.f, v11 = 0.f;
         if (inr) {
             if (yin0 && xin0) { v00 = im[(size_t)y0 * P.W + x0]; if (kDfeat) atomicAdd(&di[(size_t)y0 * P.W + x0], go * wx0 * wy0); }
@@ -233,24 +286,12 @@
             const int box = c0 + i;
             unsigned long long kk[4] = {~0ull, ~0ull, ~0ull, ~0ull};
             float vv[4] = {0.f, 0.f, 0.f, 0.f};
-            const float *g = P.guided + ((size_t)b * P.capK + box) * 7;
-            const float xg = g[0], yg = g[1], wg = g[3], lg = g[4], rg = g[6];
-            const float ct = cosf(rg), st = sinf(rg);
-            const float xx = P.lin4[ix] * wg, yy = P.lin7[iy] * lg;
-            const float x = xx * ct + yy * st + xg;
-            const float y = yy * ct - xx * st + yg;
-            const float u = (x + P.offx) * P.scale, v = (y + P.offy) * P.scale;
-            const float gx = u / (float)(P.W - 1) * 2.f - 1.f, gy = v / (float)(P.H - 1) * 2.f - 1.f;
-            float fx = (gx + 1.f) / 2.f * (float)(P.W - 1), fy = (gy + 1.f) / 2.f * (float)(P.H - 1);
-            const bool inr = fx > -1.f && fx < (float)P.W && fy > -1.f && fy < (float)P.H;
-            fx = fminf(fmaxf(fx, -2.f), (float)P.W + 1.f);
-            fy = fminf(fmaxf(fy, -2.f), (float)P.H + 1.f);
-            const float x0f = floorf(fx), y0f = floorf(fy);
-            const int x0 = (int)x0f, y0 = (int)y0f, x1 = x0 + 1, y1 = y0 + 1;
-            const float wx1 = fx - x0f, wx0 = (x0f + 1.f) - fx, wy1 = fy - y0f, wy0 = (y0f + 1.f) - fy;
+            const PsTap t = ps_tap(P, b, box, ix, iy);
+            const bool inr = t.inr;
+            const int x0 = t.x0, y0 = t.y0, x1 = t.x1, y1 = t.y1;
+            const float wx0 = t.wx0, wx1 = t.wx1, wy0 = t.wy0, wy1 = t.wy1;
+            const bool xin0 = t.xin0, xin1 = t.xin1, yin0 = t.yin0, yin1 = t.yin1;
             const float go = dlogits[(size_t)b * P.capK + box] / 28.f;
-            const bool xin0 = x0 >= 0 && x0 < P.W, xin1 = x1 >= 0 && x1 < P.W;
-            const bool yin0 = y0 >= 0 && y0 < P.H, yin1 = y1 >= 0 && y1 < P.H;
             const unsigned long long id = (unsigned long long)(i * 4);
             if (inr) {
                 if (yin0 && xin0) { kk[0] = ((unsigned long long)((size_t)y0 * P.W + x0) << 32) | id; vv[0] = go * wx0 * wy0; }
@@ -610,6 +651,36 @@
     return sassd_launch_status();
 }
 
+extern "C" size_t sassd_ps_pixel_list_ints(int batch, int H, int W)
+{
+    if (batch < 1 || H < 1 || W < 1 || (size_t)batch * H * W > ((size_t)1 << 30)) return 0;
+    const size_t HW = (size_t)H * W;
+    return ps_flag_off(batch, HW) + (size_t)batch * ps_flag_stride(HW) / 4;
+}
+
+extern "C" int sassd_ps_pixel_list(const float *guided, const int32_t *counts, int capK, int batch, int H, int W,
+                                   float grid_off_x, float grid_off_y, float spatial_scale, int32_t *list, void *stream_)
+{
+    if (!guided || !counts || !list || capK < 1 || sassd_ps_pixel_list_ints(batch, H, W) == 0) return SASSD_EINVAL;
+    if ((uintptr_t)list & 15) return SASSD_EINVAL;
+    WarpParams P;
+    P.feat = nullptr; P.guided = guided; P.counts = counts; P.logits = nullptr;
+    P.B = batch; P.H = H; P.W = W; P.capK = capK;
+    P.offx = grid_off_x; P.offy = grid_off_y; P.scale = spatial_scale;
+    linspace_f32(-0.5f, 0.5f, 4, P.lin4);
+    linspace_f32(-0.5f, 0.5f, 7, P.lin7);
+    const int HW = H * W;
+    const int fstride = (int)ps_flag_stride(HW);
+    unsigned char *flags = (unsigned char *)(list + ps_flag_off(batch, HW));
+    hipStream_t s = (hipStream_t)stream_;
+    const int rc = sassd_fill2(flags, (size_t)batch * fstride, 0, flags, 0, 0, s);
+    if (rc) return rc;
+    hipLaunchKernelGGL(ps_mark_kernel, dim3(cdiv(capK, 8), batch), dim3(256), 0, s, P, flags, fstride);
+    hipLaunchKernelGGL(ps_compact_kernel, dim3(cdiv(HW, kPsBlock), batch), dim3(kPsBlock), 0, s, (const unsigned char *)flags,
+                       fstride, HW, list, list + ps_list_head(batch));
+    return sassd_launch_status();
+}
+
 extern "C" int sassd_pswarp_sample_bwd(const float *feat, int batch, int H, int W, const float *guided,
                                        const int32_t *counts, int capK, float grid_off_x, float grid_off_y,
                                        float spatial_scale, const float *dlogits, float *dfeat, float *dguided,
diff --git a/sa-ssd_amd/kernels.py b/sa-ssd_amd/kernels.py
--- a/sa-ssd_amd/kernels.py
+++ b/sa-ssd_amd/kernels.py
@@ -877,6 +877,45 @@
     return logits
 
 
+def ps_pixel_list_buffer(batch, h, w, device):
+    n = _C.lib().sassd_ps_pixel_list_ints(int(batch), int(h), int(w))
+    if n == 0:
+        raise ValueError("ps_pixel_list: unsupported shape")
+    return torch.zeros(n, dtype=torch.int32, device=device)
+
+
+def ps_pixel_list_views(buf, batch, h, w):
+    hw, head = h * w, (batch + 3) // 4 * 4
+    fs = (hw + 15) // 16 * 16
+    fo = head + (batch * hw + 3) // 4 * 4
+    flags = buf[fo:fo + batch * fs // 4].view(torch.uint8).view(batch, fs)[:, :hw]
+    return buf[:batch], buf[head:head + batch * hw].view(batch, hw), flags
+
+
+def ps_pixel_list(guided, counts, cap_k, batch, h, w, grid_offsets, spatial_scale, out=None):
+    _chk_cuda(guided, counts)
+    if out is None:
+        out = ps_pixel_list_buffer(batch, h, w, guided.device)
+    _C.check(_C.lib().sassd_ps_pixel_list(_C.ptr(guided), _C.ptr(counts), int(cap_k), int(batch), int(h), int(w),
+                                          float(grid_offsets[0]), float(grid_offsets[1]), float(spatial_scale), _C.ptr(out),
+                                          _C.stream()), "sassd_ps_pixel_list")
+    return out
+
+
+def ps_head_sampled_supported(cin, parts):
+    return bool(_C.lib().sassd_ps_head_sampled_supported(int(cin), int(parts)))
+
+
+def ps_head_sampled(x, w0_packed, scale0, shift0, relu0, w1t, scale1, shift1, relu1, pixel_list, y):
+    _chk_cuda(x, w0_packed, scale0, shift0, w1t, scale1, shift1, pixel_list, y)
+    b, cin, h, w = x.shape
+    _C.check(_C.lib().sassd_ps_head_sampled(_C.ptr(x), _C.ptr(w0_packed), _C.ptr(scale0), _C.ptr(shift0), 1 if relu0 else 0,
+                                            _C.ptr(w1t), _C.ptr(scale1), _C.ptr(shift1), 1 if relu1 else 0,
+                                            _C.ptr(pixel_list), _C.ptr(y), b, cin, y.shape[1], h, w, _C.stream()),
+             "sassd_ps_head_sampled")
+    return y
+
+
 def pswarp_sample_bwd(feat, guided, counts, cap_k, grid_offsets, spatial_scale, dlogits, deterministic=False):
     b, parts, h, w = feat.shape
     dfeat = torch.zeros_like(feat)
diff --git a/sa-ssd_amd/pipeline.py b/sa-ssd_amd/pipeline.py
--- a/sa-ssd_amd/pipeline.py
+++ b/sa-ssd_amd/pipeline.py
@@ -47,7 +47,7 @@
                  iou_thr=0.1, cap_k=4096, cap_d=512, device=None, level_cap_factor=2, overlap=True, winograd=True,
                  fused_rulebooks=True, chain_bev=True, pyramid_persistent=False, spconv_cfg=None, wino4_cfg=None,
                  skip_inactive_tiles=True, rb_sync_levels=(0, 1, 2, 3), ps_tail=False, precision="fp32",
-                 sparse_precision="fp32", dense_entry=False):
+                 sparse_precision="fp32", dense_entry=False, ps_sampled=True):
         if precision not in ("fp32", "bf16"):
             raise ValueError("precision must be 'fp32' or 'bf16', got %r" % (precision,))
         if sparse_precision not in ("fp32", "bf16"):
@@ -109,7 +109,7 @@
         if self.bf16:
             self._dense_weights_bf16(sd, hw, w0, w1)
         else:
-            self._dense_weights_fp32(sd, hw, w0, w1, winograd, chain_bev, wino4_cfg, ps_tail)
+            self._dense_weights_fp32(sd, hw, w0, w1, winograd, chain_bev, wino4_cfg, ps_tail, ps_sampled)
 
         self.Atot = self.ncls * self.H * self.W * self.A
         if anchors is not None:
@@ -141,7 +141,10 @@
         self._dense = None
         self.act = [z(B, 256, H, W, dt=mdt) for _ in range(3)]
         self.head_out = z(B, self.head_c, H, W)
-        self.ps_t = [z(B, self.ps_parts, H, W, dt=mdt), z(B, self.ps_parts, H, W)]
+        self._ps_t = [None if self.ps_sampled else z(B, self.ps_parts, H, W, dt=mdt), z(B, self.ps_parts, H, W)]
+        self._ps_dense = None
+        self.ps_list = K.ps_pixel_list_buffer(B, H, W, dev) if self.ps_sampled else None
+        self.conv6 = None
         self.mask = z(B, self.Atot, dt=torch.uint8)
         self.df = dict(guided=z(B, self.capK, 7), labels=z(B, self.capK, dt=i32), scores=z(B, self.capK),
                        counts=z(B, dt=i32))
@@ -184,7 +187,7 @@
         self.prof = None
         self.prof_sparse_layers = False
 
-    def _dense_weights_fp32(self, sd, hw, w0, w1, winograd, chain_bev, wino4_cfg, ps_tail):
+    def _dense_weights_fp32(self, sd, hw, w0, w1, winograd, chain_bev, wino4_cfg, ps_tail, ps_sampled):
         D3, dev = self.D3, self.dev
         self.bev = []
         for i in range(8):
@@ -220,6 +223,8 @@
         self.ps_w0t = K.conv2d_wino4_pack_weight_narrow(w0) if self.ps_tail else None
         self.ps_narrow = K.conv1x1_narrow_supported(w1.shape[1], w1.shape[0])
         self.ps_w1 = K.conv1x1_narrow_pack_weight(w1) if self.ps_narrow else K.conv2d_pack_weight(w1)
+        self.ps_sampled = bool(ps_sampled and not self.ps_tail and self.ps_narrow and w0.shape[2] == 3 and
+                               self.ps_parts == 28 and K.ps_head_sampled_supported(w0.shape[1], self.ps_parts))
 
     def _dense_weights_bf16(self, sd, hw, w0, w1):
         H, W = self.H, self.W
@@ -230,7 +235,7 @@
                                  % (what, H, W))
         need(K.densify_bf16_supported(64, self.shapes[3]), "the dense map (64 x %d channels)" % self.D3)
         self.bev, self.chain, self.wino4_ws, self.ps_tail, self.ps_w0t = [], [False] * 8, None, False, None
-        self.head_narrow = self.ps_narrow = False
+        self.head_narrow = self.ps_narrow = self.ps_sampled = False
         self.bev_cin = [int(sd["neck.fcn.conv%d.weight" % i].shape[1]) for i in range(8)]
         self.bev16 = []
         for i in range(8):
@@ -257,6 +262,17 @@
         if self._dense is None:
             self._dense = torch.zeros(*self._dense_shape, dtype=self._dense_dt, device=self.dev)
         return self._dense
+
+    @property
+    def ps_t(self):
+        if not self.ps_sampled:
+            return self._ps_t
+        if self._ps_dense is None:
+            self._ps_dense = [torch.zeros(self.B, self.ps_parts, self.H, self.W, device=self.dev) for _ in range(2)]
+        if self.conv6 is not None:
+            K.conv2d_fwd(self.conv6, self.ps_w0, self.ps_parts, 3, self.ps_s0, self.ps_b0, True, self._ps_dense[0])
+            K.conv1x1_narrow_fwd(self._ps_dense[0], self.ps_w1, self.ps_parts, None, None, False, self._ps_dense[1])
+        return self._ps_dense
 
     @property
     def dense(self):
@@ -436,7 +452,7 @@
                 K.conv2d_fwd(x, wp, cout, ks, scale, shift, True, y)
             if i == 6 and self.ps_tail:
                 K.conv2d_wino4_chain_tail(self.bev[6][3:5] + (True,), y, self.ps_w0t, cout, self.ps_parts, self.cmax, self.B,
-                                          self.H, self.W, self.ps_s0, self.ps_b0, True, self.ps_t[0], self.wino4_ws,
+                                          self.H, self.W, self.ps_s0, self.ps_b0, True, self._ps_t[0], self.wino4_ws,
                                           cfg=self.wino4_cfg)
             self._seg("bev_conv%d" % i, e0)
             x = y
@@ -448,12 +464,15 @@
             K.conv1x1_narrow_fwd(x, self.head_w, self.head_c, None, self.head_b, False, self.head_out)
         else:
             K.conv2d_fwd(x, self.head_w, self.head_c, 1, None, self.head_b, False, self.head_out)
+        if self.ps_sampled:
+            self._seg("heads", e0)
+            return
         if not self.ps_tail:
-            K.conv2d_fwd(self.conv6, self.ps_w0, self.ps_parts, 3, self.ps_s0, self.ps_b0, True, self.ps_t[0])
+            K.conv2d_fwd(self.conv6, self.ps_w0, self.ps_parts, 3, self.ps_s0, self.ps_b0, True, self._ps_t[0])
         if self.ps_narrow:
-            K.conv1x1_narrow_fwd(self.ps_t[0], self.ps_w1, self.ps_parts, None, None, False, self.ps_t[1])
-        else:
-            K.conv2d_fwd(self.ps_t[0], self.ps_w1, self.ps_parts, 1, None, None, False, self.ps_t[1])
+            K.conv1x1_narrow_fwd(self._ps_t[0], self.ps_w1, self.ps_parts, None, None, False, self._ps_t[1])
+        else:
+            K.conv2d_fwd(self._ps_t[0], self.ps_w1, self.ps_parts, 1, None, None, False, self._ps_t[1])
         self._seg("heads", e0)
 
     def _bev_and_heads_bf16(self):
@@ -472,8 +491,8 @@
         self.x = x
         e0 = self._ev() if self.prof is not None else None
         K.conv1x1_bf16_infer_fwd(x, self.head_w, self.head_c, None, self.head_b, False, self.head_out, out_bf16=False)
-        K.conv2d_bf16_infer_fwd(self.conv6, self.ps_w0, self.ps_parts, self.ps_s0, self.ps_b0, True, self.ps_t[0])
-        K.conv1x1_bf16_infer_fwd(self.ps_t[0], self.ps_w1, self.ps_parts, None, None, False, self.ps_t[1], out_bf16=False)
+        K.conv2d_bf16_infer_fwd(self.conv6, self.ps_w0, self.ps_parts, self.ps_s0, self.ps_b0, True, self._ps_t[0])
+        K.conv1x1_bf16_infer_fwd(self._ps_t[0], self.ps_w1, self.ps_parts, None, None, False, self._ps_t[1], out_bf16=False)
         self._seg("heads", e0)
 
     def anchor_masks(self, masks=None):
@@ -494,7 +513,12 @@
         dirp = base[(self.n_box + self.n_cls) * HW:]
         K.decode_filter(box, cls, dirp, self.head_c * HW, self.B, self.ncls, self.A, self.H, self.W, self.anchors,
                         self.mask, self.rpn_thr, self.capK, self.df, self.status)
-        K.pswarp_sample(self.ps_t[1], self.df["guided"], self.df["counts"], self.capK, self.grid_offsets,
+        if self.ps_sampled:
+            K.ps_pixel_list(self.df["guided"], self.df["counts"], self.capK, self.B, self.H, self.W, self.grid_offsets,
+                            self.spatial_scale, out=self.ps_list)
+            K.ps_head_sampled(self.conv6, self.ps_w0, self.ps_s0, self.ps_b0, True, self.ps_w1, None, None, False,
+                              self.ps_list, self._ps_t[1])
+        K.pswarp_sample(self._ps_t[1], self.df["guided"], self.df["counts"], self.capK, self.grid_offsets,
                         self.spatial_scale, self.logits)
         K.rescore_nms(self.df["guided"], self.logits, self.df["labels"], self.df["counts"], self.score_thr,
                       self.iou_thr, self.capD, self.det, self.status)
```

New measurement: 1061 frames/s (median of 6 runs). +4.3%, better.
